# Nuralamsiddik16/Ultrafnd_git

Hardware: AMD Instinct MI355X
Metric: train-step samples/sec (FakeSV batch, seq128+224^2) (higher is better)
Workload: dtype bf16

## Files before the change

### include/ultrafnd_hip.h

```cpp
#ifndef ULTRAFND_HIP_H
#define ULTRAFND_HIP_H

#include <stddef.h>
#include <stdint.h>

#ifdef __cplusplus
extern "C" {
#endif

#define UFND_OK 0
#define UFND_ERR_INVALID 1
#define UFND_ERR_LAUNCH 2

#define UFND_ABI_VERSION 5

const char* ufnd_last_error(void);
int ufnd_abi_version(void);

typedef struct ufnd_step_state {
  uint64_t step;
  uint64_t seed;
  float lr;
  float weight_decay;
  float beta1, beta2, eps;
  float max_norm;
  float grad_scale;
  float loss;
  float grad_norm;
  float clip_coef;
  float bc1, bc2_sqrt;
  float reserved[3];
} ufnd_step_state;

typedef struct ufnd_dims {
  int hidden;
  int text_dim;
  int audio_dim;
  int visual_dim;
  int temporal_dim;
  int gnn_dim;
  int aux_dim;
  int trees;
  int depth;
  int classes;
  float fusion_dropout;
  float clf_dropout;
  float node_dropout;
} ufnd_dims;

typedef struct ufnd_fusion_params {
  float *text_w, *text_b;
  float *audio_w, *audio_b;
  float *visual_w, *visual_b;
  float *temporal_w, *temporal_b;
  float *gnn_w, *gnn_b;
  float *qkv_w, *qkv_b;
  float *ev0_w[3], *ev0_b[3];
  float *ev2_w[3], *ev2_b[3];
  float *fuse0_w, *fuse0_b;
  float *fuse3_w, *fuse3_b;
  float *cls_w, *cls_b;
} ufnd_fusion_params;

typedef struct ufnd_clf_params {
  float *pre0_w, *pre0_b;
  float *pre3_w, *pre3_b;
  float *gates, *thresh;
  float *leaf, *tau;
  float *bypass_w, *bypass_b;
  float *temperature;
} ufnd_clf_params;

size_t ufnd_fusion_workspace_floats(const ufnd_dims* d, int B);
size_t ufnd_clf_workspace_floats(const ufnd_dims* d, int B);

int ufnd_fusion_forward(const ufnd_dims* d, const ufnd_fusion_params* p, const float* text, const float* audio,
                        const float* visual, const float* temporal, const float* gnn, int B, int train,
                        float* workspace, float* fused, int ld_fused, float* logits, float* forensic,
                        const ufnd_step_state* state, void* stream);

int ufnd_fusion_backward(const ufnd_dims* d, const ufnd_fusion_params* p, const ufnd_fusion_params* g,
                         const float* text, const float* audio, const float* visual, const float* temporal,
                         const float* gnn, int B, int train, float* workspace, const float* d_fused,
                         int ld_dfused, const float* d_logits, const ufnd_step_state* state, void* stream,
                         void* side_stream, int join);

#define UFND_BWD_ALL 0
#define UFND_BWD_FUSE_MLP 1
#define UFND_BWD_REST 2
#define UFND_BWD_NO_LINEAR_GRADS 16
int ufnd_fusion_backward_phase(const ufnd_dims* d, const ufnd_fusion_params* p, const ufnd_fusion_params* g,
                               const float* text, const float* audio, const float* visual, const float* temporal,
                               const float* gnn, int B, int train, float* workspace, const float* d_fused,
                               int ld_dfused, const float* d_logits, const ufnd_step_state* state, void* stream,
                               void* side_stream, int join, int phase);

float* ufnd_clf_input_panel(const ufnd_dims* d, float* clf_workspace, int B, int* ld);
int ufnd_classifier_forward(const ufnd_dims* d, const ufnd_clf_params* p, const float* fused, int ld_fused,
                            const float* aux, int B, int train, float* workspace, float* logits, float* probs,
                            const ufnd_step_state* state, void* stream);
int ufnd_classifier_backward(const ufnd_dims* d, const ufnd_clf_params* p, const ufnd_clf_params* g, int B,
                             int train, float* workspace, const float* d_logits, float* d_fused, int ld_dfused,
                             const ufnd_step_state* state, void* stream, void* side_stream, int join);

int ufnd_classifier_backward_ex(const ufnd_dims* d, const ufnd_clf_params* p, const ufnd_clf_params* g, int B,
                                int train, float* workspace, const float* d_logits, float* d_fused, int ld_dfused,
                                const ufnd_step_state* state, void* stream, void* side_stream, int join, int flags);

size_t ufnd_head_factor_floats(const ufnd_dims* d, int B);
int ufnd_head_pack_factors(const ufnd_dims* d, const float* text, const float* audio, const float* visual, const float* temporal,
                           const float* gnn, int B, float* fusion_workspace, float* clf_workspace, float* pack, void* stream);
int ufnd_head_linear_grads_from_factors(const ufnd_dims* d, const ufnd_fusion_params* fusion_grads, const ufnd_clf_params* clf_grads,
                                        const float* packs, size_t rank_stride, int ranks, int B, void* stream);

typedef struct ufnd_head_io {
  const float *text, *audio, *visual, *temporal, *gnn, *aux;
  const int64_t* labels;
  float *fusion_workspace, *clf_workspace;
  float *logits, *probs, *forensic;
  float* d_logits;
} ufnd_head_io;
int ufnd_head_forward_loss(const ufnd_dims* d, const ufnd_fusion_params* fusion, const ufnd_clf_params* clf, const ufnd_head_io* io, int B,
                           int train, ufnd_step_state* state, void* stream);
int ufnd_head_backward(const ufnd_dims* d, const ufnd_fusion_params* fusion, const ufnd_fusion_params* fusion_grads, const ufnd_clf_params* clf,
                       const ufnd_clf_params* clf_grads, const ufnd_head_io* io, int B, int train, ufnd_step_state* state, void* stream,
                       void* side_stream, int join, int phase);

int ufnd_softmax_ce(const float* logits, const int64_t* labels, int B, float* loss_rows, float* d_logits,
                    ufnd_step_state* state, void* stream);

int ufnd_softmax_ce_weighted(const float* logits, const int64_t* labels, int B, float w0, float w1, float label_smoothing,
                             float* loss_rows, float* d_logits, ufnd_step_state* state, void* stream);

int ufnd_grad_norm(const float* grad, size_t n, float* partials, ufnd_step_state* state, void* stream);
int ufnd_adamw_step(float* param, const float* grad, float* exp_avg, float* exp_avg_sq, size_t n,
                    const ufnd_step_state* state, void* stream);
int ufnd_step_advance(ufnd_step_state* state, void* stream);
int ufnd_clip_adamw_step(float* param, const float* grad, float* exp_avg, float* exp_avg_sq, size_t n, float* partials,
                         ufnd_step_state* state, void* stream);

#define UFND_ACT_NONE 0
#define UFND_ACT_GELU 1
#define UFND_ACT_QUICK_GELU 2
#define UFND_ACT_GELU_BWD 3
#define UFND_ACT_QUICK_GELU_BWD 4

int ufnd_cast_bf16(const float* src, void* dst_bf16, size_t n, void* stream);

int ufnd_gemm_bf16(const void* A, const void* W, const float* bias, const float* residual, void* out_bf16,
                   float* out_f32, int M, int N, int K, int lda, int ldw, int ldr, int ldo, int ldf, int act,
                   void* stream);

#define UFND_GEMM_TILE_PERSISTENT 64
int ufnd_gemm_bf16_ex(const void* A, const void* W, const float* bias, const float* residual, void* out_bf16,
                      float* out_f32, int M, int N, int K, int lda, int ldw, int ldr, int ldo, int ldf, int act,
                      int tile_cfg, void* stream);

typedef struct ufnd_gemm_ln {
  const float* a_stats;
  const float* colsum;
  const float* r_stats;
  const float* r_gamma;
  const float* r_beta;
  float* out_stats;
  int a_parts, r_parts;
  float a_eps, r_eps;
  int width;
  int tile_cfg;
  const void* residual_bf16;
  int ldrb;
  float* guard;
} ufnd_gemm_ln;
#define UFND_FOLD_GUARD_SLOTS 1024
int ufnd_gemm_bf16_ln(const void* A, const void* W, const float* bias, const float* residual, void* out_bf16,
                      float* out_f32, int M, int N, int K, int lda, int ldw, int ldr, int ldo, int ldf, int act,
                      const ufnd_gemm_ln* ln, void* stream);
int ufnd_gemm_bf16_stat_parts(int M, int N, int K);

int ufnd_ln_fold_guard(const float* stats, int M, int parts, int width, float eps, float* guard, void* stream);
int ufnd_ln_fold_guard_multi(const float* stats, int M, int parts, int nbuf, size_t buf_stride, int width, float eps, float* guard,
                             void* stream);

int ufnd_gemm_bf16_tile_count(void);
int ufnd_gemm_bf16_tile_info(int tile_cfg, int* bm, int* bn, int* ln_aware);

int ufnd_layernorm(const float* x, int ldx, const float* gamma, const float* beta, void* out_bf16, float* out_f32,
                   int M, int H, float eps, void* stream);

int ufnd_attention_bf16(const void* qkv, const int32_t* key_mask, void* ctx, int B, int L, int heads,
                        void* stream);

int ufnd_qkv_attention_bf16(const void* X, const void* Wqkv, const float* bqkv, const int32_t* key_mask, void* ctx, int B, int L,
                            int heads, int ldx, int ldw, const ufnd_gemm_ln* ln, void* stream);

int ufnd_bert_embed_packed(const int64_t* ids, const int32_t* pos_ids, const float* word, const float* pos, const float* type0,
                           const float* gamma, const float* beta, void* x_bf16, float* x_f32, int T, int max_pos, int H,
                           int vocab, float eps, void* stream);
int ufnd_attention_bf16_varlen(const void* qkv, const int32_t* cu_seqlens, void* ctx, int B, int max_len, int heads, void* stream);
int ufnd_meanpool_l2_packed(const float* hidden, const int32_t* cu_seqlens, const int32_t* pos_ids, float* out, int B, int H,
                            void* stream);

int ufnd_text_pack(const int32_t* mask, int B, int L, int32_t* cu_seqlens, int32_t* row_src, void* stream);
int ufnd_bert_embed_live(const int64_t* ids, const int32_t* row_src, const int* m_live, const float* word, const float* pos,
                         const float* type0, const float* gamma, const float* beta, void* x_bf16, float* x_f32, int capacity, int L,
                         int H, int vocab, float eps, void* stream);
int ufnd_gemm_bf16_live(const void* A, const void* W, const float* bias, const float* residual, void* out_bf16, float* out_f32,
                        int M, int N, int K, int lda, int ldw, int ldr, int ldo, int ldf, int act, int tile_cfg, const int* m_live,
                        void* stream);
int ufnd_gemm_bf16_ln_live(const void* A, const void* W, const float* bias, const float* residual, void* out_bf16, float* out_f32,
                           int M, int N, int K, int lda, int ldw, int ldr, int ldo, int ldf, int act, const ufnd_gemm_ln* ln,
                           const int* m_live, void* stream);
int ufnd_qkv_attention_bf16_packed(const void* X, const void* Wqkv, const float* bqkv, const int32_t* key_mask, const int32_t* cu_seqlens,
                                   void* ctx, int B, int L, int heads, int ldx, int ldw, const ufnd_gemm_ln* ln, void* stream);
int ufnd_attention_bf16_varlen_masked(const void* qkv, const int32_t* cu_seqlens, const int32_t* key_mask, void* ctx, int B, int max_len,
                                      int heads, void* stream);
int ufnd_layernorm_live(const float* x, int ldx, const float* gamma, const float* beta, void* out_bf16, float* out_f32, int capacity,
                        int H, float eps, const int* m_live, void* stream);
int ufnd_masked_meanpool_l2_live(const float* hidden, const int32_t* mask, const int32_t* cu_seqlens, float* out, int B, int L, int H,
                                 void* stream);

int ufnd_bert_embed(const int64_t* ids, const float* word, const float* pos, const float* type0, const float* gamma,
                    const float* beta, void* x_bf16, float* x_f32, int B, int L, int H, int vocab, float eps,
                    void* stream);

int ufnd_masked_meanpool_l2(const float* hidden, const int32_t* mask, float* out, int B, int L, int H,
                            void* stream);

int ufnd_field_mean_l2(const float* parts, const int32_t* valid, float* out, int N, int M, int D, void* stream);

int ufnd_vit_patchify(const float* frames, void* patches_bf16, int N, int image, int patch, void* stream);

int ufnd_vit_assemble(const float* patch_emb, const float* cls, const float* pos, const float* gamma,
                      const float* beta, float* x_f32, void* x_bf16, float* stats, int N, int P, int H, float eps,
                      void* stream);

int ufnd_l2norm_frames(const float* e, float* out, int B, int F, int D, void* stream);

#define UFND_GATHER_MAX_ITEMS 8
typedef struct ufnd_gather_item {
  const void* src;
  void* dst;
  int row_bytes;
  int64_t src_rows;
} ufnd_gather_item;
int ufnd_gather_rows(const int64_t* idx, int B, const ufnd_gather_item* items, int n_items, void* stream);

int ufnd_temporal_weight_ld(int in_dim);
size_t ufnd_temporal_workspace_floats(int B, int in_dim, int hidden);
int ufnd_temporal_align(const float* text, const float* visual, const float* w0, const float* b0, const float* w3,
                        const float* b3, float* workspace, float* out, int B, int in_dim, int vis_dim, int hidden,
                        int out_dim, float dropout_p, const ufnd_step_state* state, void* stream);

typedef struct ufnd_tcn_layer {
  const float *w, *b;
  const float *gamma, *beta;
  float *running_mean, *running_var;
} ufnd_tcn_layer;
int ufnd_tcn_weight_ld(int in_ch, int kernel);
size_t ufnd_tcn_workspace_floats(int B, int T, int in_ch, int hid, int kernel);
int ufnd_tcn_forward(const float* text_seq, int text_dim, const float* vis_seq, int vis_dim, int B, int T,
                     const ufnd_tcn_layer* layers, int n_layers, int kernel, int hid, const float* head_w,
                     const float* head_b, int out_dim, int train, float dropout_p, float momentum, float eps,
                     const ufnd_step_state* state, float* workspace, float* out, void* stream);


int ufnd_ocr_adjacency(const int32_t* offsets, const int32_t* tokens, int N, double thresh, float* adj, int ld, void* stream);

typedef struct ufnd_gcn_params {
  const float* w1;
  const float* b1;
  const float* w2;
  const float* b2;
} ufnd_gcn_params;

size_t ufnd_gcn_workspace_floats(int N, int in_dim, int hid, int out_dim, int train);

int ufnd_gcn_forward(const float* x, const float* adj, int ld_adj, const ufnd_gcn_params* p, float* z, float* workspace, int N,
                     int in_dim, int hid, int out_dim, float dropout_p, const ufnd_step_state* state, void* stream);

int ufnd_gcn_pretrain_step(const float* x, const float* adj, int ld_adj, const ufnd_gcn_params* p, float* exp_avg,
                           float* exp_avg_sq, const float* head_w, const float* head_b, float* z, float* workspace, int N,
                           int in_dim, int hid, int out_dim, float dropout_p, float lr, float weight_decay, int step,
                           const ufnd_step_state* state, float* loss, void* stream);


int ufnd_ocr_adjacency_weighted(const int32_t* offsets, const int32_t* tokens, int N, double thresh, float* adj, int ld, void* stream);

int ufnd_node_features(const float* text, int ld_text, const float* audio, int ld_audio, const float* visual, int ld_visual,
                       const float* temporal, int ld_temporal, int n_text, int n_audio, int n_visual, int n_temporal, int B,
                       float* out, void* stream);

size_t ufnd_gnn_workspace_floats(int N, int in_dim, int hid, int out_dim);
int ufnd_gnn_forward(const float* x, const float* adj, int ld_adj, const ufnd_gcn_params* p, float* z, float* workspace, int N,
                     int in_dim, int hid, int out_dim, float dropout_p, const ufnd_step_state* state, void* stream);
int ufnd_gnn_backward(const float* x, const ufnd_gcn_params* p, float* g_w1, float* g_b1, float* g_w2, float* g_b2, const float* d_z,
                      float* workspace, int N, int in_dim, int hid, int out_dim, float dropout_p, const ufnd_step_state* state,
                      void* stream);
int ufnd_fusion_feature_grads(const ufnd_dims* d, const ufnd_fusion_params* p, float* workspace, int B, float* d_text, float* d_visual,
                              const ufnd_step_state* state, void* stream);

int ufnd_fusion_gnn_input_grad(const ufnd_dims* d, const ufnd_fusion_params* p, float* workspace, int B, float* d_gnn,
                               const ufnd_step_state* state, void* stream);

int ufnd_stream_create_cu_mask(const uint32_t* mask_words, int n_words, void** stream_out);
int ufnd_stream_destroy(void* stream);
int ufnd_device_cu_count(void);


int ufnd_gemm_bf16_dgrad(const void* dY, const void* Wt, const float* residual, const void* aux, void* out_bf16, float* out_f32,
                         int M, int N, int K, int lda, int ldw, int ldr, int ldaux, int ldo, int ldf, int act, void* stream);

size_t ufnd_gemm_bf16_wgrad_workspace_floats(int n_out, int k_in, int tokens);
int ufnd_gemm_bf16_wgrad(const void* dYt, const void* Xt, float* dW, int n_out, int k_in, int tokens, int lda, int ldb, int ldw,
                         float* workspace, int accumulate, void* stream);

typedef struct ufnd_partials_job {
  const float* part;
  int nblk, H;
  float *out0, *out1;
} ufnd_partials_job;
#define UFND_PARTIALS_DEFER 2

#define UFND_WGRAD_ALL 0
#define UFND_WGRAD_TRANSPOSE 1
#define UFND_WGRAD_PRODUCT 2
int ufnd_linear_wgrad(const void* dY, int lddy, const void* X, int ldx, int M, int N, int K, float* dW, float* db, void* dYt, void* Xt, int ldt,
                      float* slab_workspace, float* colsum_workspace, const ufnd_partials_job* extra, int part, void* stream);

typedef struct ufnd_refresh_item {
  const void* master;
  void* w;
  void* wt;
  int rows, cols, ld_master, ld_w, ld_wt, tile0;
} ufnd_refresh_item;
int ufnd_refresh_operands(const ufnd_refresh_item* items_device, int n_items, int total_tiles, void* stream);

size_t ufnd_transpose_colsum_workspace_floats(int rows_pad, int cols);
int ufnd_transpose_bf16(const void* src, int src_is_f32, int rows, int cols, int lds, void* dst, int ldd, int rows_pad, float* colsum,
                        float* colsum_ws, int colsum_accumulate, void* stream);

int ufnd_attention_bf16_lse(const void* qkv, const int32_t* key_mask, void* ctx, float* lse, int B, int L, int heads, void* stream);
size_t ufnd_attention_bwd_workspace_floats(int B, int L, int heads);
int ufnd_attention_bf16_bwd(const void* qkv, const void* ctx, const void* dctx, const float* lse, const int32_t* key_mask, void* dqkv,
                            float* workspace, int B, int L, int heads, void* stream);

size_t ufnd_layernorm_bwd_workspace_floats(int M, int H);
int ufnd_layernorm_bwd_blocks(int M);
int ufnd_row_partials_finish(const ufnd_partials_job* job, int accumulate, void* stream);
int ufnd_layernorm_bwd(const float* x, int ldx, const float* gamma, const float* dy, int lddy, const float* add, int ldadd, float* dx_f32,
                       void* dx_bf16, int lddx, float* dgamma, float* dbeta, float* workspace, int accumulate, int M, int H, float eps,
                       void* stream);

int ufnd_act_bf16(const void* x, void* out, size_t n, int act, void* stream);

int ufnd_masked_meanpool_l2_bwd(const float* hidden, const int32_t* mask, const float* dfeat, float* dhidden, int B, int L, int H, void* stream);
int ufnd_l2norm_frames_bwd(const float* e, const float* dfeat, float* de, int B, int F, int D, void* stream);
int ufnd_bert_embed_bwd(const int64_t* ids, const float* ds, float* dword, float* dpos, float* dtype, int B, int L, int H, int vocab,
                        int max_pos, int type_vocab, void* stream);
int ufnd_vit_assemble_bwd(const float* ds, float* dcls, float* dpos, void* dpe_bf16, int N, int P, int H, void* stream);

typedef struct ufnd_dropout {
  const ufnd_step_state* state;
  float p;
  uint32_t tag;
} ufnd_dropout;

#define UFND_LN_BWD_DROP_DXB 1
#define UFND_LN_BWD_DROP_DY 2

int ufnd_attention_bf16_lse_dropout(const void* qkv, const int32_t* key_mask, void* ctx, float* lse, int B, int L, int heads,
                                    const ufnd_dropout* drop, void* stream);
int ufnd_attention_bf16_bwd_dropout(const void* qkv, const void* ctx, const void* dctx, const float* lse, const int32_t* key_mask,
                                    void* dqkv, float* workspace, int B, int L, int heads, const ufnd_dropout* drop, void* stream);
int ufnd_dropout_residual_layernorm(const float* x, int ldx, const float* d, int ldd, const float* gamma, const float* beta, float* y,
                                    void* out_bf16, float* out_f32, int M, int H, float eps, const ufnd_dropout* drop, void* stream);
int ufnd_layernorm_dropout(const float* x, int ldx, const float* gamma, const float* beta, void* out_bf16, float* out_f32, int M, int H,
                           float eps, const ufnd_dropout* drop, void* stream);
int ufnd_layernorm_bwd_dropout(const float* x, int ldx, const float* gamma, const float* dy, int lddy, const float* add, int ldadd,
                               float* dx_f32, void* dx_bf16, int lddx, float* dgamma, float* dbeta, float* workspace, int accumulate,
                               int M, int H, float eps, const ufnd_dropout* drop, int where, void* stream);

#ifdef __cplusplus
}
#endif
#endif
```

### ultrafnd_git_amd/_lib.py

```python
from __future__ import annotations

import ctypes as C
from pathlib import Path
from typing import Optional

import torch

_PKG = Path(__file__).resolve().parent
LIB_PATH = _PKG / "libultrafnd_hip.so"


class UltrafndHipError(RuntimeError):
    pass


class StepState(C.Structure):
    _fields_ = [("step", C.c_uint64), ("seed", C.c_uint64), ("lr", C.c_float), ("weight_decay", C.c_float),
                ("beta1", C.c_float), ("beta2", C.c_float), ("eps", C.c_float), ("max_norm", C.c_float),
                ("grad_scale", C.c_float), ("loss", C.c_float), ("grad_norm", C.c_float), ("clip_coef", C.c_float),
                ("bc1", C.c_float), ("bc2_sqrt", C.c_float), ("reserved", C.c_float * 3)]


class Dims(C.Structure):
    _fields_ = [("hidden", C.c_int), ("text_dim", C.c_int), ("audio_dim", C.c_int), ("visual_dim", C.c_int),
                ("temporal_dim", C.c_int), ("gnn_dim", C.c_int), ("aux_dim", C.c_int), ("trees", C.c_int),
                ("depth", C.c_int), ("classes", C.c_int), ("fusion_dropout", C.c_float), ("clf_dropout", C.c_float),
                ("node_dropout", C.c_float)]


_FP = C.c_void_p


class FusionParams(C.Structure):
    _fields_ = [(n, _FP) for n in ("text_w", "text_b", "audio_w", "audio_b", "visual_w", "visual_b", "temporal_w",
                                   "temporal_b", "gnn_w", "gnn_b", "qkv_w", "qkv_b")] + \
               [("ev0_w", _FP * 3), ("ev0_b", _FP * 3), ("ev2_w", _FP * 3), ("ev2_b", _FP * 3)] + \
               [(n, _FP) for n in ("fuse0_w", "fuse0_b", "fuse3_w", "fuse3_b", "cls_w", "cls_b")]


class ClfParams(C.Structure):
    _fields_ = [(n, _FP) for n in ("pre0_w", "pre0_b", "pre3_w", "pre3_b", "gates", "thresh", "leaf", "tau",
                                   "bypass_w", "bypass_b", "temperature")]


class GcnParams(C.Structure):
    _fields_ = [(n, _FP) for n in ("w1", "b1", "w2", "b2")]


class GatherItem(C.Structure):
    _fields_ = [("src", _FP), ("dst", _FP), ("row_bytes", C.c_int), ("src_rows", C.c_int64)]


class TcnLayer(C.Structure):
    _fields_ = [(n, _FP) for n in ("w", "b", "gamma", "beta", "running_mean", "running_var")]


class HeadIO(C.Structure):
    _fields_ = [(n, C.c_void_p) for n in ("text", "audio", "visual", "temporal", "gnn", "aux", "labels", "fusion_workspace", "clf_workspace",
                                           "logits", "probs", "forensic", "d_logits")]


class PartialsJob(C.Structure):
    _fields_ = [("part", C.c_void_p), ("nblk", C.c_int), ("H", C.c_int), ("out0", C.c_void_p), ("out1", C.c_void_p)]


class RefreshItem(C.Structure):
    _fields_ = [("master", C.c_void_p), ("w", C.c_void_p), ("wt", C.c_void_p), ("rows", C.c_int), ("cols", C.c_int), ("ld_master", C.c_int),
                ("ld_w", C.c_int), ("ld_wt", C.c_int), ("tile0", C.c_int)]


class Dropout(C.Structure):
    _fields_ = [("state", C.c_void_p), ("p", C.c_float), ("tag", C.c_uint32)]


PARTIALS_DEFER = 2
LN_BWD_DROP_DXB, LN_BWD_DROP_DY = 1, 2
WGRAD_ALL, WGRAD_TRANSPOSE, WGRAD_PRODUCT = 0, 1, 2


class GemmLn(C.Structure):
    _fields_ = [("a_stats", _FP), ("colsum", _FP), ("r_stats", _FP), ("r_gamma", _FP), ("r_beta", _FP), ("out_stats", _FP),
                ("a_parts", C.c_int), ("r_parts", C.c_int), ("a_eps", C.c_float), ("r_eps", C.c_float), ("width", C.c_int),
                ("tile_cfg", C.c_int), ("residual_bf16", _FP), ("ldrb", C.c_int), ("guard", _FP)]

    def __init__(self, *a, **kw):
        super().__init__(*a, **kw)
        if "tile_cfg" not in kw:
            self.tile_cfg = -1


STEP_STATE_BYTES = C.sizeof(StepState)
BWD_ALL, BWD_FUSE_MLP, BWD_REST = 0, 1, 2
BWD_NO_LINEAR_GRADS = 16
ABI_VERSION = 5
FOLD_GUARD_SLOTS = 1024

_lib: Optional[C.CDLL] = None


def _declare(lib: C.CDLL) -> None:
    P, I, S = C.c_void_p, C.c_int, C.c_size_t
    lib.ufnd_last_error.restype = C.c_char_p
    lib.ufnd_abi_version.restype = I
    lib.ufnd_fusion_workspace_floats.restype = S
    lib.ufnd_fusion_workspace_floats.argtypes = [C.POINTER(Dims), I]
    lib.ufnd_clf_workspace_floats.restype = S
    lib.ufnd_clf_workspace_floats.argtypes = [C.POINTER(Dims), I]
    lib.ufnd_clf_input_panel.restype = P
    lib.ufnd_clf_input_panel.argtypes = [C.POINTER(Dims), P, I, C.POINTER(I)]
    lib.ufnd_fusion_forward.argtypes = [C.POINTER(Dims), C.POINTER(FusionParams), P, P, P, P, P, I, I, P, P, I, P, P, P, P]
    lib.ufnd_fusion_backward.argtypes = [C.POINTER(Dims), C.POINTER(FusionParams), C.POINTER(FusionParams),
                                         P, P, P, P, P, I, I, P, P, I, P, P, P, P, I]
    lib.ufnd_fusion_backward_phase.argtypes = [C.POINTER(Dims), C.POINTER(FusionParams), C.POINTER(FusionParams),
                                               P, P, P, P, P, I, I, P, P, I, P, P, P, P, I, I]
    lib.ufnd_fusion_backward_phase.restype = I
    lib.ufnd_classifier_forward.argtypes = [C.POINTER(Dims), C.POINTER(ClfParams), P, I, P, I, I, P, P, P, P, P]
    lib.ufnd_classifier_backward.argtypes = [C.POINTER(Dims), C.POINTER(ClfParams), C.POINTER(ClfParams), I, I, P, P, P,
                                             I, P, P, P, I]
    lib.ufnd_classifier_backward_ex.argtypes = [C.POINTER(Dims), C.POINTER(ClfParams), C.POINTER(ClfParams), I, I, P, P, P,
                                                I, P, P, P, I, I]
    lib.ufnd_classifier_backward_ex.restype = I
    lib.ufnd_head_factor_floats.argtypes = [C.POINTER(Dims), I]
    lib.ufnd_head_factor_floats.restype = S
    lib.ufnd_head_pack_factors.argtypes = [C.POINTER(Dims), P, P, P, P, P, I, P, P, P, P]
    lib.ufnd_head_pack_factors.restype = I
    lib.ufnd_head_linear_grads_from_factors.argtypes = [C.POINTER(Dims), C.POINTER(FusionParams), C.POINTER(ClfParams), P, S, I, I, P]
    lib.ufnd_head_linear_grads_from_factors.restype = I
    lib.ufnd_head_forward_loss.argtypes = [C.POINTER(Dims), C.POINTER(FusionParams), C.POINTER(ClfParams), C.POINTER(HeadIO), I, I, P, P]
    lib.ufnd_head_forward_loss.restype = I
    lib.ufnd_head_backward.argtypes = [C.POINTER(Dims), C.POINTER(FusionParams), C.POINTER(FusionParams), C.POINTER(ClfParams), C.POINTER(ClfParams),
                                       C.POINTER(HeadIO), I, I, P, P, P, I, I]
    lib.ufnd_head_backward.restype = I
    lib.ufnd_softmax_ce.argtypes = [P, P, I, P, P, P, P]
    lib.ufnd_softmax_ce_weighted.argtypes = [P, P, I, C.c_float, C.c_float, C.c_float, P, P, P, P]
    lib.ufnd_softmax_ce_weighted.restype = I
    lib.ufnd_grad_norm.argtypes = [P, S, P, P, P]
    lib.ufnd_adamw_step.argtypes = [P, P, P, P, S, P, P]
    lib.ufnd_step_advance.argtypes = [P, P]
    lib.ufnd_clip_adamw_step.argtypes = [P, P, P, P, S, P, P, P]
    lib.ufnd_clip_adamw_step.restype = I
    for name in ("ufnd_fusion_forward", "ufnd_fusion_backward", "ufnd_classifier_forward", "ufnd_classifier_backward",
                 "ufnd_softmax_ce", "ufnd_grad_norm", "ufnd_adamw_step", "ufnd_step_advance"):
        getattr(lib, name).restype = I
    _declare_encoders(lib)


def _declare_encoders(lib: C.CDLL) -> None:
    P, I, S, F = C.c_void_p, C.c_int, C.c_size_t, C.c_float
    sigs = {
        "ufnd_cast_bf16": [P, P, S, P],
        "ufnd_gemm_bf16": [P] * 6 + [I] * 9 + [P],
        "ufnd_gemm_bf16_ex": [P] * 6 + [I] * 10 + [P],
        "ufnd_layernorm": [P, I, P, P, P, P, I, I, F, P],
        "ufnd_attention_bf16": [P, P, P, I, I, I, P],
        "ufnd_qkv_attention_bf16": [P, P, P, P, P, I, I, I, I, I, C.POINTER(GemmLn), P],
        "ufnd_bert_embed": [P] * 8 + [I, I, I, I, F, P],
        "ufnd_masked_meanpool_l2": [P, P, P, I, I, I, P],
        "ufnd_bert_embed_packed": [P] * 9 + [I, I, I, I, F, P],
        "ufnd_attention_bf16_varlen": [P, P, P, I, I, I, P],
        "ufnd_meanpool_l2_packed": [P, P, P, P, I, I, P],
        "ufnd_text_pack": [P, I, I, P, P, P],
        "ufnd_bert_embed_live": [P] * 10 + [I, I, I, I, F, P],
        "ufnd_gemm_bf16_live": [P] * 6 + [I] * 10 + [P, P],
        "ufnd_gemm_bf16_ln_live": [P] * 6 + [I] * 9 + [C.POINTER(GemmLn), P, P],
        "ufnd_qkv_attention_bf16_packed": [P, P, P, P, P, P, I, I, I, I, I, C.POINTER(GemmLn), P],
        "ufnd_attention_bf16_varlen_masked": [P, P, P, P, I, I, I, P],
        "ufnd_layernorm_live": [P, I, P, P, P, P, I, I, F, P, P],
        "ufnd_masked_meanpool_l2_live": [P, P, P, P, I, I, I, P],
        "ufnd_vit_patchify": [P, P, I, I, I, P],
        "ufnd_vit_assemble": [P] * 8 + [I, I, I, F, P],
        "ufnd_gemm_bf16_ln": [P] * 6 + [I] * 9 + [C.POINTER(GemmLn), P],
        "ufnd_gemm_bf16_stat_parts": [I, I, I],
        "ufnd_ln_fold_guard": [P, I, I, I, F, P, P],
        "ufnd_ln_fold_guard_multi": [P, I, I, I, S, I, F, P, P],
        "ufnd_gemm_bf16_tile_count": [],
        "ufnd_gemm_bf16_tile_info": [I, C.POINTER(I), C.POINTER(I), C.POINTER(I)],
        "ufnd_stream_create_cu_mask": [C.POINTER(C.c_uint32), I, C.POINTER(P)],
        "ufnd_stream_destroy": [P],
        "ufnd_device_cu_count": [],
        "ufnd_l2norm_frames": [P, P, I, I, I, P],
        "ufnd_field_mean_l2": [P, P, P, I, I, I, P],
        "ufnd_temporal_align": [P] * 8 + [I] * 5 + [F, P, P],
    }
    sigs.update({
        "ufnd_gemm_bf16_dgrad": [P] * 6 + [I] * 10 + [P],
        "ufnd_gemm_bf16_wgrad": [P, P, P, I, I, I, I, I, I, P, I, P],
        "ufnd_transpose_bf16": [P, I, I, I, I, P, I, I, P, P, I, P],
        "ufnd_linear_wgrad": [P, I, P, I, I, I, I, P, P, P, P, I, P, P, C.POINTER(PartialsJob), I, P],
        "ufnd_refresh_operands": [P, I, I, P],
        "ufnd_layernorm_bwd_blocks": [I],
        "ufnd_row_partials_finish": [C.POINTER(PartialsJob), I, P],
        "ufnd_attention_bf16_lse": [P, P, P, P, I, I, I, P],
        "ufnd_attention_bf16_bwd": [P, P, P, P, P, P, P, I, I, I, P],
        "ufnd_layernorm_bwd": [P, I, P, P, I, P, I, P, P, I, P, P, P, I, I, I, F, P],
        "ufnd_masked_meanpool_l2_bwd": [P, P, P, P, I, I, I, P],
        "ufnd_l2norm_frames_bwd": [P, P, P, I, I, I, P],
        "ufnd_bert_embed_bwd": [P, P, P, P, P, I, I, I, I, I, I, P],
        "ufnd_vit_assemble_bwd": [P, P, P, P, I, I, I, P],
        "ufnd_act_bf16": [P, P, S, I, P],
        "ufnd_attention_bf16_lse_dropout": [P, P, P, P, I, I, I, C.POINTER(Dropout), P],
        "ufnd_attention_bf16_bwd_dropout": [P, P, P, P, P, P, P, I, I, I, C.POINTER(Dropout), P],
        "ufnd_dropout_residual_layernorm": [P, I, P, I, P, P, P, P, P, I, I, F, C.POINTER(Dropout), P],
        "ufnd_layernorm_dropout": [P, I, P, P, P, P, I, I, F, C.POINTER(Dropout), P],
        "ufnd_layernorm_bwd_dropout": [P, I, P, P, I, P, I, P, P, I, P, P, P, I, I, I, F, C.POINTER(Dropout), I, P],
    })
    for name, argtypes in sigs.items():
        fn = getattr(lib, name)
        fn.argtypes = argtypes
        fn.restype = I
    for name, argtypes in (("ufnd_gemm_bf16_wgrad_workspace_floats", [I, I, I]), ("ufnd_transpose_colsum_workspace_floats", [I, I]),
                           ("ufnd_attention_bwd_workspace_floats", [I, I, I]), ("ufnd_layernorm_bwd_workspace_floats", [I, I])):
        fn = getattr(lib, name)
        fn.argtypes = argtypes
        fn.restype = S
    D = C.c_double
    lib.ufnd_ocr_adjacency.argtypes = [P, P, I, D, P, I, P]
    lib.ufnd_ocr_adjacency.restype = I
    lib.ufnd_gcn_workspace_floats.argtypes = [I, I, I, I, I]
    lib.ufnd_gcn_workspace_floats.restype = S
    lib.ufnd_gcn_forward.argtypes = [P, P, I, C.POINTER(GcnParams), P, P, I, I, I, I, F, P, P]
    lib.ufnd_gcn_forward.restype = I
    lib.ufnd_gcn_pretrain_step.argtypes = [P, P, I, C.POINTER(GcnParams), P, P, P, P, P, P, I, I, I, I, F, F, F, I, P, P, P]
    lib.ufnd_gcn_pretrain_step.restype = I
    lib.ufnd_ocr_adjacency_weighted.argtypes = [P, P, I, D, P, I, P]
    lib.ufnd_ocr_adjacency_weighted.restype = I
    lib.ufnd_node_features.argtypes = [P, I, P, I, P, I, P, I, I, I, I, I, I, P, P]
    lib.ufnd_node_features.restype = I
    lib.ufnd_gnn_workspace_floats.argtypes = [I, I, I, I]
    lib.ufnd_gnn_workspace_floats.restype = S
    lib.ufnd_gnn_forward.argtypes = [P, P, I, C.POINTER(GcnParams), P, P, I, I, I, I, F, P, P]
    lib.ufnd_gnn_forward.restype = I
    lib.ufnd_gnn_backward.argtypes = [P, C.POINTER(GcnParams), P, P, P, P, P, P, I, I, I, I, F, P, P]
    lib.ufnd_gnn_backward.restype = I
    lib.ufnd_fusion_gnn_input_grad.argtypes = [C.POINTER(Dims), C.POINTER(FusionParams), P, I, P, P, P]
    lib.ufnd_fusion_gnn_input_grad.restype = I
    lib.ufnd_fusion_feature_grads.argtypes = [C.POINTER(Dims), C.POINTER(FusionParams), P, I, P, P, P, P]
    lib.ufnd_fusion_feature_grads.restype = I
    lib.ufnd_gather_rows.argtypes = [P, I, C.POINTER(GatherItem), I, P]
    lib.ufnd_gather_rows.restype = I
    lib.ufnd_tcn_weight_ld.argtypes = [I, I]
    lib.ufnd_tcn_weight_ld.restype = I
    lib.ufnd_tcn_workspace_floats.argtypes = [I, I, I, I, I]
    lib.ufnd_tcn_workspace_floats.restype = S
    lib.ufnd_tcn_forward.argtypes = [P, I, P, I, I, I, C.POINTER(TcnLayer), I, I, I, P, P, I, I, F, F, F, P, P, P, P]
    lib.ufnd_tcn_forward.restype = I
    lib.ufnd_temporal_weight_ld.argtypes = [I]
    lib.ufnd_temporal_weight_ld.restype = I
    lib.ufnd_temporal_workspace_floats.argtypes = [I, I, I]
    lib.ufnd_temporal_workspace_floats.restype = S


def lib() -> C.CDLL:
    global _lib
    if _lib is None:
        if not LIB_PATH.exists():
            raise UltrafndHipError(
                f"{LIB_PATH} is missing: run `python -m ultrafnd_git_amd.build` (hipcc, gfx950). "
                "This package has no CPU fallback.")
        l = C.CDLL(str(LIB_PATH))
        _declare(l)
        if l.ufnd_abi_version() != ABI_VERSION:
            raise UltrafndHipError("libultrafnd_hip.so ABI version mismatch; rebuild")
        _lib = l
    return _lib


def check(rc: int, what: str) -> None:
    if rc != 0:
        raise UltrafndHipError(f"{what} failed (code {rc}): {lib().ufnd_last_error().decode()}")


def ptr(t: Optional[torch.Tensor]) -> Optional[int]:
    return None if t is None else t.data_ptr()


def require_hip(*tensors: Optional[torch.Tensor]) -> torch.device:
    dev = None
    for t in tensors:
        if t is None:
            continue
        if t.device.type != "cuda":
            raise UltrafndHipError(
                f"tensor on {t.device}: the fusion hot path runs on a HIP device only (no CPU fallback); "
                "move the module and its inputs to 'cuda'")
        dev = dev or t.device
        if t.device != dev:
            raise UltrafndHipError("all tensors of one call must live on the same device")
    return dev


def stream_ptr(device: torch.device) -> int:
    return torch.cuda.current_stream(device).cuda_stream


def f32c(t: torch.Tensor) -> torch.Tensor:
    if t.dtype != torch.float32:
        t = t.float()
    return t if t.is_contiguous() else t.contiguous()
```

### ultrafnd_git_amd/csrc/encoders.hip

```cpp
#include "common.hpp"

namespace {

__device__ __forceinline__ f32x4 ld4(const float* p) { return *reinterpret_cast<const f32x4*>(p); }

template <int NI>
__device__ __forceinline__ void ln_row(f32x4 (&v)[NI], int H, float eps, const float* gamma, const float* beta, int lane) {
  float s = 0.0f;
#pragma unroll
  for (int i = 0; i < NI; ++i) s += v[i][0] + v[i][1] + v[i][2] + v[i][3];
  const float mean = wave_sum(s) / (float)H;
  float q = 0.0f;
#pragma unroll
  for (int i = 0; i < NI; ++i)
#pragma unroll
    for (int k = 0; k < 4; ++k) {
      const float d = v[i][k] - mean;
      q += d * d;
    }
  const float rstd = rsqrtf(wave_sum(q) / (float)H + eps);
#pragma unroll
  for (int i = 0; i < NI; ++i) {
    const int col = 4 * lane + 256 * i;
    const f32x4 gm = ld4(gamma + col), bt = ld4(beta + col);
#pragma unroll
    for (int k = 0; k < 4; ++k) v[i][k] = (v[i][k] - mean) * rstd * gm[k] + bt[k];
  }
}

template <int NI>
__device__ __forceinline__ void store_row(const f32x4 (&v)[NI], __bf16* ob, float* of, size_t row, int H, int lane) {
#pragma unroll
  for (int i = 0; i < NI; ++i) {
    const int col = 4 * lane + 256 * i;
    if (of) *reinterpret_cast<f32x4*>(of + row * H + col) = v[i];
    if (ob) {
      bf16x4 o = {(__bf16)v[i][0], (__bf16)v[i][1], (__bf16)v[i][2], (__bf16)v[i][3]};
      *reinterpret_cast<bf16x4*>(ob + row * H + col) = o;
    }
  }
}

template <int NI>
__device__ __forceinline__ void row_stats(const f32x4 (&v)[NI], float* stats, size_t row, int lane) {
  float s = 0.0f, q = 0.0f;
#pragma unroll
  for (int i = 0; i < NI; ++i)
#pragma unroll
    for (int k = 0; k < 4; ++k) { s += v[i][k]; q += v[i][k] * v[i][k]; }
  s = wave_sum(s);
  q = wave_sum(q);
  if (lane == 0) *reinterpret_cast<f32x4*>(stats + row * 4) = f32x4{s, q, 0.0f, 0.0f};
}

template <int NI>
__global__ __launch_bounds__(256) void layernorm_kernel(const float* x, int ldx, const float* gamma, const float* beta,
                                                        __bf16* ob, float* of, int M, int H, float eps, const int* m_live) {
  const int lane = threadIdx.x & 63;
  const int row = blockIdx.x * 4 + (threadIdx.x >> 6);
  if (row >= M || (m_live && row >= *m_live)) return;
  f32x4 v[NI];
#pragma unroll
  for (int i = 0; i < NI; ++i) v[i] = ld4(x + (size_t)row * ldx + 4 * lane + 256 * i);
  ln_row<NI>(v, H, eps, gamma, beta, lane);
  store_row<NI>(v, ob, of, row, H, lane);
}

template <int NI, bool RESID>
__global__ __launch_bounds__(256) void dropout_layernorm_kernel(const float* x, int ldx, const float* d, int ldd, const float* gamma,
                                                                const float* beta, float* y, __bf16* ob, float* of, int M, int H, float eps,
                                                                ufnd_dropout dr) {
  const int lane = threadIdx.x & 63;
  const int row = blockIdx.x * 4 + (threadIdx.x >> 6);
  if (row >= M) return;
  const uint64_t seed = dr.state->seed, step = dr.state->step;
  f32x4 v[NI], m[NI];
#pragma unroll
  for (int i = 0; i < NI; ++i) {
    const int col = 4 * lane + 256 * i;
    float m4[4];
    dropout_mul4_ctr(seed, step, dr.p, dr.tag, (uint32_t)(((size_t)row * H + col) >> 2), m4);
    m[i] = f32x4{m4[0], m4[1], m4[2], m4[3]};
    v[i] = ld4(x + (size_t)row * ldx + col);
    if constexpr (RESID) {
      v[i] += m[i] * ld4(d + (size_t)row * ldd + col);
      *reinterpret_cast<f32x4*>(y + (size_t)row * H + col) = v[i];
    }
  }
  ln_row<NI>(v, H, eps, gamma, beta, lane);
  if constexpr (!RESID) {
#pragma unroll
    for (int i = 0; i < NI; ++i) v[i] *= m[i];
  }
  store_row<NI>(v, ob, of, row, H, lane);
}

template <int NI>
__global__ __launch_bounds__(256) void bert_embed_kernel(const int64_t* ids, const float* word, const float* pos,
                                                         const float* type0, const float* gamma, const float* beta,
                                                         __bf16* ob, float* of, int M, int L, int H, int vocab,
                                                         float eps, const int32_t* pos_ids, const int32_t* row_src,
                                                         const int* m_live) {
  const int lane = threadIdx.x & 63;
  const int row = blockIdx.x * 4 + (threadIdx.x >> 6);
  if (row >= M || (m_live && row >= *m_live)) return;
  const int src = row_src ? row_src[row] : row;
  long long id = ids[src];
  id = id < 0 ? 0 : (id >= vocab ? vocab - 1 : id);
  int l = pos_ids ? pos_ids[row] : src % L;
  l = l < 0 ? 0 : (l >= L ? L - 1 : l);
  f32x4 v[NI];
#pragma unroll
  for (int i = 0; i < NI; ++i) {
    const int col = 4 * lane + 256 * i;
    v[i] = ld4(word + (size_t)id * H + col) + ld4(pos + (size_t)l * H + col) + ld4(type0 + col);
  }
  if (gamma) ln_row<NI>(v, H, eps, gamma, beta, lane);
  store_row<NI>(v, ob, of, row, H, lane);
}

template <bool PACKED>
__global__ __launch_bounds__(256) void meanpool_kernel(const float* hidden, const int32_t* mask, float* out, int L, int H, const int32_t* cu) {
  __shared__ f32x4 part[4][64];
  __shared__ float cnts[4];
  const int b = blockIdx.y, col = blockIdx.x * 256 + 4 * (threadIdx.x & 63), grp = threadIdx.x >> 6, lane = threadIdx.x & 63;
  f32x4 acc = {0.f, 0.f, 0.f, 0.f};
  float cnt = 0.0f;
  const size_t r0 = PACKED ? (size_t)cu[b] : (size_t)b * L;
  const int n = PACKED ? cu[b + 1] - cu[b] : L;
  for (int l0 = grp; l0 < n; l0 += 32) {
    int mk[8];
    f32x4 x[8];
#pragma unroll
    for (int u = 0; u < 8; ++u) {
      const int l = l0 + 4 * u;
      mk[u] = l < n ? mask[(size_t)b * L + l] : 0;
    }
#pragma unroll
    for (int u = 0; u < 8; ++u) {
      const int l = l0 + 4 * u < n ? l0 + 4 * u : n - 1;
      x[u] = ld4(hidden + (r0 + l) * H + col);
    }
#pragma unroll
    for (int u = 0; u < 8; ++u) {
      if (mk[u] != 0) {
        acc += x[u];
        cnt += 1.0f;
      }
    }
  }
  part[grp][lane] = acc;
  if (lane == 0) cnts[grp] = cnt;
  __syncthreads();
  if (grp == 0) {
    const f32x4 s = (part[0][lane] + part[1][lane]) + (part[2][lane] + part[3][lane]);
    const float denom = fmaxf((cnts[0] + cnts[1]) + (cnts[2] + cnts[3]), 1e-6f);
    *reinterpret_cast<f32x4*>(out + (size_t)b * H + col) = s / denom;
  }
}
__global__ __launch_bounds__(256) void meanpool_packed_kernel(const float* hidden, const int32_t* cu, const int32_t* pos_ids, float* out,
                                                              int H) {
  __shared__ f32x4 part[4][64];
  __shared__ float cnts[4];
  const int b = blockIdx.y, col = blockIdx.x * 256 + 4 * (threadIdx.x & 63), grp = threadIdx.x >> 6, lane = threadIdx.x & 63;
  const int r0 = cu[b], r1 = cu[b + 1];
  f32x4 acc = {0.f, 0.f, 0.f, 0.f};
  float cnt = 0.0f;
  for (int r = r0; r < r1; ++r) {
    if ((pos_ids[r] & 3) == grp) {
      acc += ld4(hidden + (size_t)r * H + col);
      cnt += 1.0f;
    }
  }
  part[grp][lane] = acc;
  if (lane == 0) cnts[grp] = cnt;
  __syncthreads();
  if (grp == 0) {
    const f32x4 s = (part[0][lane] + part[1][lane]) + (part[2][lane] + part[3][lane]);
    const float denom = fmaxf((cnts[0] + cnts[1]) + (cnts[2] + cnts[3]), 1e-6f);
    *reinterpret_cast<f32x4*>(out + (size_t)b * H + col) = s / denom;
  }
}
constexpr int PACK_THREADS = 1024, PACK_MAX_B = 16384;
__global__ __launch_bounds__(PACK_THREADS) void text_pack_kernel(const int32_t* mask, int B, int L, int32_t* cu, int32_t* row_src) {
  __shared__ int lens[PACK_MAX_B];
  __shared__ int wsum[PACK_THREADS / 64];
  __shared__ int total;
  const int tid = threadIdx.x, wave = tid >> 6, lane = tid & 63;
  for (int b = wave; b < B; b += PACK_THREADS / 64) {
    int last = 0;
    for (int l = lane; l < L; l += 64) last = mask[(size_t)b * L + l] != 0 ? l + 1 : last;
#pragma unroll
    for (int o = 32; o >= 1; o >>= 1) last = max(last, __shfl_xor(last, o, 64));
    if (lane == 0) lens[b] = last;
  }
  __syncthreads();
  const int per = (B + PACK_THREADS - 1) / PACK_THREADS, b0 = tid * per, b1 = min(b0 + per, B);
  int own = 0;
  for (int b = b0; b < b1; ++b) own += lens[b];
  int inc = own;
#pragma unroll
  for (int o = 1; o < 64; o <<= 1) {
    const int y = __shfl_up(inc, o, 64);
    if (lane >= o) inc += y;
  }
  if (lane == 63) wsum[wave] = inc;
  __syncthreads();
  int base = 0;
  for (int w = 0; w < wave; ++w) base += wsum[w];
  int run = base + inc - own;
  for (int b = b0; b < b1; ++b) {
    const int n = lens[b];
    lens[b] = run;
    cu[b] = run;
    run += n;
  }
  if (tid == PACK_THREADS - 1) {
    cu[B] = run;
    total = run;
  }
  __syncthreads();
  for (int b = wave; b < B; b += PACK_THREADS / 64) {
    const int r0 = lens[b], n = (b + 1 < B ? lens[b + 1] : total) - r0;
    for (int l = lane; l < n; l += 64) row_src[r0 + l] = b * L + l;
  }
}

__global__ __launch_bounds__(256) void l2norm_rows_kernel(float* x, int H) {
  __shared__ float sh[4];
  float* row = x + (size_t)blockIdx.x * H;
  float sq = 0.0f;
  for (int c = threadIdx.x; c < H; c += 256) sq += row[c] * row[c];
  sq = wave_sum(sq);
  if ((threadIdx.x & 63) == 0) sh[threadIdx.x >> 6] = sq;
  __syncthreads();
  const float nrm = sqrtf((sh[0] + sh[1]) + (sh[2] + sh[3])) + 1e-9f;
  for (int c = threadIdx.x; c < H; c += 256) row[c] = row[c] / nrm;
}

template <int PT, int GT>
__global__ __launch_bounds__(256) void patchify_kernel(const float* frames, __bf16* patches, int S_, int P_) {
  const int P = PT ? PT : P_, G = GT ? GT : S_ / P_, S = P * G;
  const int n = blockIdx.x / G, py = blockIdx.x - n * G;
  const int K = 3 * P * P, CPR = P / 8;
  const int chunks = 3 * P * G * CPR;
  const float* src = frames + ((size_t)n * 3 * S + (size_t)py * P) * S;
  __bf16* dst = patches + ((size_t)n * G * G + (size_t)py * G) * K;
  for (int q = threadIdx.x; q < chunks; q += 256) {
    const int x8 = q % (G * CPR), r = q / (G * CPR);
    const int ky = r % P, c = r / P;
    const int px = x8 / CPR, kx = (x8 - px * CPR) * 8;
    const float* sp = src + ((size_t)c * S + ky) * S + x8 * 8;
    const f32x4 v0 = ld4(sp), v1 = ld4(sp + 4);
    bf16x8 o = {(__bf16)v0[0], (__bf16)v0[1], (__bf16)v0[2], (__bf16)v0[3], (__bf16)v1[0], (__bf16)v1[1], (__bf16)v1[2], (__bf16)v1[3]};
    *reinterpret_cast<bf16x8*>(dst + (size_t)px * K + c * P * P + ky * P + kx) = o;
  }
}

template <int NI>
__global__ __launch_bounds__(256) void vit_assemble_kernel(const float* pe, const float* cls, const float* pos,
                                                           const float* gamma, const float* beta, float* of, __bf16* ob,
                                                           float* stats, int M, int P, int H, float eps) {
  const int lane = threadIdx.x & 63;
  const int row = blockIdx.x * 4 + (threadIdx.x >> 6);
  if (row >= M) return;
  const int n = row / (P + 1), t = row % (P + 1);
  f32x4 v[NI];
#pragma unroll
  for (int i = 0; i < NI; ++i) {
    const int col = 4 * lane + 256 * i;
    const f32x4 base = (t == 0) ? ld4(cls + col) : ld4(pe + ((size_t)n * P + (t - 1)) * H + col);
    v[i] = base + ld4(pos + (size_t)t * H + col);
  }
  if (gamma) ln_row<NI>(v, H, eps, gamma, beta, lane);
  store_row<NI>(v, ob, of, row, H, lane);
  if (stats) row_stats<NI>(v, stats, row, lane);
}

__global__ __launch_bounds__(256) void l2norm_frames_kernel(const float* e, float* out, int F, int D) {
  __shared__ float sh[4];
  const int b = blockIdx.x;
  float acc[4] = {0, 0, 0, 0};
  for (int f = 0; f < F; ++f) {
    const float* row = e + ((size_t)b * F + f) * D;
    float sq = 0.0f;
    for (int c = threadIdx.x; c < D; c += 256) sq += row[c] * row[c];
    sq = wave_sum(sq);
    __syncthreads();
    if ((threadIdx.x & 63) == 0) sh[threadIdx.x >> 6] = sq;
    __syncthreads();
    const float nrm = sqrtf((sh[0] + sh[1]) + (sh[2] + sh[3])) + 1e-9f;
    int n = 0;
    for (int c = threadIdx.x; c < D; c += 256, ++n) acc[n] += row[c] / nrm;
  }
  if (F == 1) {
    int n = 0;
    for (int c = threadIdx.x; c < D; c += 256, ++n) out[(size_t)b * D + c] = acc[n];
    return;
  }
  float sq = 0.0f;
  int n = 0;
  for (int c = threadIdx.x; c < D; c += 256, ++n) {
    acc[n] /= (float)F;
    sq += acc[n] * acc[n];
  }
  sq = wave_sum(sq);
  __syncthreads();
  if ((threadIdx.x & 63) == 0) sh[threadIdx.x >> 6] = sq;
  __syncthreads();
  const float nrm = sqrtf((sh[0] + sh[1]) + (sh[2] + sh[3])) + 1e-9f;
  n = 0;
  for (int c = threadIdx.x; c < D; c += 256, ++n) out[(size_t)b * D + c] = acc[n] / nrm;
}

__global__ __launch_bounds__(256) void field_mean_l2_kernel(const float* parts, const int32_t* valid, float* out, int Mx,
                                                            int D) {
  __shared__ float sh[4];
  const int n = blockIdx.x;
  float acc[4] = {0, 0, 0, 0};
  int cnt = 0;
  for (int m = 0; m < Mx; ++m) {
    if (valid[(size_t)n * Mx + m] == 0) continue;
    ++cnt;
    const float* row = parts + ((size_t)n * Mx + m) * D;
    int k = 0;
    for (int c = threadIdx.x; c < D; c += 256, ++k) acc[k] += row[c];
  }
  float sq = 0.0f;
  int k = 0;
  for (int c = threadIdx.x; c < D; c += 256, ++k) {
    acc[k] = cnt ? acc[k] / (float)cnt : 0.0f;
    sq += acc[k] * acc[k];
  }
  sq = wave_sum(sq);
  if ((threadIdx.x & 63) == 0) sh[threadIdx.x >> 6] = sq;
  __syncthreads();
  const float nrm = sqrtf((sh[0] + sh[1]) + (sh[2] + sh[3])) + 1e-9f;
  k = 0;
  for (int c = threadIdx.x; c < D; c += 256, ++k) out[(size_t)n * D + c] = cnt ? acc[k] / nrm : 0.0f;
}

#define NI_LAUNCH(H, KERNEL, GRID, STREAM, ...)                                                       \
  do {                                                                                                \
    if ((H) == 256) hipLaunchKernelGGL((KERNEL<1>), GRID, dim3(256), 0, STREAM, __VA_ARGS__);         \
    else if ((H) == 512) hipLaunchKernelGGL((KERNEL<2>), GRID, dim3(256), 0, STREAM, __VA_ARGS__);    \
    else if ((H) == 768) hipLaunchKernelGGL((KERNEL<3>), GRID, dim3(256), 0, STREAM, __VA_ARGS__);    \
    else hipLaunchKernelGGL((KERNEL<4>), GRID, dim3(256), 0, STREAM, __VA_ARGS__);                    \
  } while (0)

#define NI_LAUNCH_T(H, KERNEL, T, GRID, STREAM, ...)                                                       \
  do {                                                                                                     \
    if ((H) == 256) hipLaunchKernelGGL((KERNEL<1, T>), GRID, dim3(256), 0, STREAM, __VA_ARGS__);           \
    else if ((H) == 512) hipLaunchKernelGGL((KERNEL<2, T>), GRID, dim3(256), 0, STREAM, __VA_ARGS__);      \
    else if ((H) == 768) hipLaunchKernelGGL((KERNEL<3, T>), GRID, dim3(256), 0, STREAM, __VA_ARGS__);      \
    else hipLaunchKernelGGL((KERNEL<4, T>), GRID, dim3(256), 0, STREAM, __VA_ARGS__);                      \
  } while (0)

inline bool h_ok(int H) { return H == 256 || H == 512 || H == 768 || H == 1024; }

}

extern "C" int ufnd_layernorm(const float* x, int ldx, const float* gamma, const float* beta, void* out_bf16,
                              float* out_f32, int M, int H, float eps, void* stream_) {
  UFND_REQUIRE(x && gamma && beta && (out_bf16 || out_f32) && M >= 1, "layernorm: null argument");
  UFND_REQUIRE(h_ok(H), "layernorm: H=%d (supported 256/512/768/1024)", H);
  UFND_REQUIRE(ldx % 4 == 0 && ldx >= H && ufnd_aligned(x, 16) && ufnd_aligned(gamma, 16) && ufnd_aligned(beta, 16),
               "layernorm: alignment");
  NI_LAUNCH(H, layernorm_kernel, dim3(ufnd_cdiv(M, 4)), (hipStream_t)stream_, x, ldx, gamma, beta, (__bf16*)out_bf16,
            out_f32, M, H, eps, (const int*)nullptr);
  UFND_CHECK_LAUNCH();
  return UFND_OK;
}

extern "C" int ufnd_dropout_residual_layernorm(const float* x, int ldx, const float* d, int ldd, const float* gamma, const float* beta, float* y,
                                               void* out_bf16, float* out_f32, int M, int H, float eps, const ufnd_dropout* drop, void* stream_) {
  UFND_REQUIRE(x && d && gamma && beta && y && (out_bf16 || out_f32) && M >= 1 && drop && drop->state, "dropout_residual_layernorm: null argument");
  UFND_REQUIRE(drop->p > 0.0f && drop->p < 1.0f, "dropout_residual_layernorm: p=%g (0 < p < 1)", (double)drop->p);
  UFND_REQUIRE(h_ok(H), "dropout_residual_layernorm: H=%d (supported 256/512/768/1024)", H);
  UFND_REQUIRE(ldx % 4 == 0 && ldx >= H && ldd % 4 == 0 && ldd >= H && ufnd_aligned(x, 16) && ufnd_aligned(d, 16) && ufnd_aligned(y, 16) &&
                   ufnd_aligned(gamma, 16) && ufnd_aligned(beta, 16) && (!out_f32 || ufnd_aligned(out_f32, 16)) && (!out_bf16 || ufnd_aligned(out_bf16, 8)),
               "dropout_residual_layernorm: alignment");
  UFND_REQUIRE((long long)M * H / 4 <= (1ll << 32), "dropout_residual_layernorm: M=%d H=%d overflows the 32-bit dropout counter", M, H);
  NI_LAUNCH_T(H, dropout_layernorm_kernel, true, dim3(ufnd_cdiv(M, 4)), (hipStream_t)stream_, x, ldx, d, ldd, gamma, beta, y, (__bf16*)out_bf16,
            out_f32, M, H, eps, *drop);
  UFND_CHECK_LAUNCH();
  return UFND_OK;
}

extern "C" int ufnd_layernorm_dropout(const float* x, int ldx, const float* gamma, const float* beta, void* out_bf16, float* out_f32, int M, int H,
                                      float eps, const ufnd_dropout* drop, void* stream_) {
  UFND_REQUIRE(x && gamma && beta && (out_bf16 || out_f32) && M >= 1 && drop && drop->state, "layernorm_dropout: null argument");
  UFND_REQUIRE(drop->p > 0.0f && drop->p < 1.0f, "layernorm_dropout: p=%g (0 < p < 1)", (double)drop->p);
  UFND_REQUIRE(h_ok(H), "layernorm_dropout: H=%d (supported 256/512/768/1024)", H);
  UFND_REQUIRE(ldx % 4 == 0 && ldx >= H && ufnd_aligned(x, 16) && ufnd_aligned(gamma, 16) && ufnd_aligned(beta, 16) &&
                   (!out_f32 || ufnd_aligned(out_f32, 16)) && (!out_bf16 || ufnd_aligned(out_bf16, 8)), "layernorm_dropout: alignment");
  UFND_REQUIRE((long long)M * H / 4 <= (1ll << 32), "layernorm_dropout: M=%d H=%d overflows the 32-bit dropout counter", M, H);
  NI_LAUNCH_T(H, dropout_layernorm_kernel, false, dim3(ufnd_cdiv(M, 4)), (hipStream_t)stream_, x, ldx, (const float*)nullptr, 0, gamma, beta,
            (float*)nullptr, (__bf16*)out_bf16, out_f32, M, H, eps, *drop);
  UFND_CHECK_LAUNCH();
  return UFND_OK;
}

extern "C" int ufnd_bert_embed(const int64_t* ids, const float* word, const float* pos, const float* type0,
                               const float* gamma, const float* beta, void* x_bf16, float* x_f32, int B, int L, int H,
                               int vocab, float eps, void* stream_) {
  UFND_REQUIRE(ids && word && pos && type0 && ((gamma && beta) || (!gamma && !beta)) && (x_bf16 || x_f32), "bert_embed: null argument");
  UFND_REQUIRE(h_ok(H) && B >= 1 && L >= 1 && vocab >= 1, "bert_embed: B=%d L=%d H=%d vocab=%d", B, L, H, vocab);
  UFND_REQUIRE(ufnd_aligned(word, 16) && ufnd_aligned(pos, 16) && ufnd_aligned(type0, 16), "bert_embed: alignment");
  const int M = B * L;
  NI_LAUNCH(H, bert_embed_kernel, dim3(ufnd_cdiv(M, 4)), (hipStream_t)stream_, ids, word, pos, type0, gamma, beta,
            (__bf16*)x_bf16, x_f32, M, L, H, vocab, eps, (const int32_t*)nullptr, (const int32_t*)nullptr,
            (const int*)nullptr);
  UFND_CHECK_LAUNCH();
  return UFND_OK;
}

extern "C" int ufnd_bert_embed_packed(const int64_t* ids, const int32_t* pos_ids, const float* word, const float* pos,
                                      const float* type0, const float* gamma, const float* beta, void* x_bf16, float* x_f32,
                                      int T, int max_pos, int H, int vocab, float eps, void* stream_) {
  UFND_REQUIRE(ids && pos_ids && word && pos && type0 && gamma && beta && (x_bf16 || x_f32), "bert_embed_packed: null argument");
  UFND_REQUIRE(h_ok(H) && T >= 1 && max_pos >= 1 && vocab >= 1, "bert_embed_packed: T=%d H=%d vocab=%d", T, H, vocab);
  UFND_REQUIRE(ufnd_aligned(word, 16) && ufnd_aligned(pos, 16) && ufnd_aligned(type0, 16), "bert_embed_packed: alignment");
  NI_LAUNCH(H, bert_embed_kernel, dim3(ufnd_cdiv(T, 4)), (hipStream_t)stream_, ids, word, pos, type0, gamma, beta,
            (__bf16*)x_bf16, x_f32, T, max_pos, H, vocab, eps, pos_ids, (const int32_t*)nullptr, (const int*)nullptr);
  UFND_CHECK_LAUNCH();
  return UFND_OK;
}

extern "C" int ufnd_masked_meanpool_l2(const float* hidden, const int32_t* mask, float* out, int B, int L, int H,
                                       void* stream_) {
  UFND_REQUIRE(hidden && mask && out && B >= 1 && L >= 1, "meanpool: null argument");
  UFND_REQUIRE(H >= 256 && H % 256 == 0 && ufnd_aligned(hidden, 16) && ufnd_aligned(out, 16), "meanpool: H=%d (multiple of 256)", H);
  hipLaunchKernelGGL(meanpool_kernel<false>, dim3(H / 256, B), dim3(256), 0, (hipStream_t)stream_, hidden, mask, out, L, H,
                     (const int32_t*)nullptr);
  UFND_CHECK_LAUNCH();
  hipLaunchKernelGGL(l2norm_rows_kernel, dim3(B), dim3(256), 0, (hipStream_t)stream_, out, H);
  UFND_CHECK_LAUNCH();
  return UFND_OK;
}

extern "C" int ufnd_meanpool_l2_packed(const float* hidden, const int32_t* cu_seqlens, const int32_t* pos_ids, float* out, int B, int H,
                                       void* stream_) {
  UFND_REQUIRE(hidden && cu_seqlens && pos_ids && out && B >= 1, "meanpool_packed: null argument");
  UFND_REQUIRE(H >= 256 && H % 256 == 0 && ufnd_aligned(hidden, 16) && ufnd_aligned(out, 16), "meanpool_packed: H=%d (multiple of 256)", H);
  hipLaunchKernelGGL(meanpool_packed_kernel, dim3(H / 256, B), dim3(256), 0, (hipStream_t)stream_, hidden, cu_seqlens, pos_ids, out, H);
  UFND_CHECK_LAUNCH();
  hipLaunchKernelGGL(l2norm_rows_kernel, dim3(B), dim3(256), 0, (hipStream_t)stream_, out, H);
  UFND_CHECK_LAUNCH();
  return UFND_OK;
}

extern "C" int ufnd_text_pack(const int32_t* mask, int B, int L, int32_t* cu_seqlens, int32_t* row_src, void* stream_) {
  UFND_REQUIRE(mask && cu_seqlens && row_src, "text_pack: null argument");
  UFND_REQUIRE(B >= 1 && B <= PACK_MAX_B && L >= 1 && (long long)B * L < (1ll << 31), "text_pack: B=%d L=%d (B <= %d)", B, L, PACK_MAX_B);
  hipLaunchKernelGGL(text_pack_kernel, dim3(1), dim3(PACK_THREADS), 0, (hipStream_t)stream_, mask, B, L, cu_seqlens, row_src);
  UFND_CHECK_LAUNCH();
  return UFND_OK;
}

extern "C" int ufnd_bert_embed_live(const int64_t* ids, const int32_t* row_src, const int* m_live, const float* word, const float* pos,
                                    const float* type0, const float* gamma, const float* beta, void* x_bf16, float* x_f32, int capacity,
                                    int L, int H, int vocab, float eps, void* stream_) {
  UFND_REQUIRE(ids && row_src && m_live && word && pos && type0 && gamma && beta && (x_bf16 || x_f32), "bert_embed_live: null argument");
  UFND_REQUIRE(h_ok(H) && capacity >= 1 && L >= 1 && vocab >= 1, "bert_embed_live: capacity=%d L=%d H=%d vocab=%d", capacity, L, H, vocab);
  UFND_REQUIRE(ufnd_aligned(word, 16) && ufnd_aligned(pos, 16) && ufnd_aligned(type0, 16), "bert_embed_live: alignment");
  NI_LAUNCH(H, bert_embed_kernel, dim3(ufnd_cdiv(capacity, 4)), (hipStream_t)stream_, ids, word, pos, type0, gamma, beta,
            (__bf16*)x_bf16, x_f32, capacity, L, H, vocab, eps, (const int32_t*)nullptr, row_src, m_live);
  UFND_CHECK_LAUNCH();
  return UFND_OK;
}

extern "C" int ufnd_layernorm_live(const float* x, int ldx, const float* gamma, const float* beta, void* out_bf16, float* out_f32,
                                   int capacity, int H, float eps, const int* m_live, void* stream_) {
  UFND_REQUIRE(x && gamma && beta && (out_bf16 || out_f32) && m_live && capacity >= 1, "layernorm_live: null argument");
  UFND_REQUIRE(h_ok(H), "layernorm_live: H=%d (supported 256/512/768/1024)", H);
  UFND_REQUIRE(ldx % 4 == 0 && ldx >= H && ufnd_aligned(x, 16) && ufnd_aligned(gamma, 16) && ufnd_aligned(beta, 16),
               "layernorm_live: alignment");
  NI_LAUNCH(H, layernorm_kernel, dim3(ufnd_cdiv(capacity, 4)), (hipStream_t)stream_, x, ldx, gamma, beta, (__bf16*)out_bf16,
            out_f32, capacity, H, eps, m_live);
  UFND_CHECK_LAUNCH();
  return UFND_OK;
}

extern "C" int ufnd_masked_meanpool_l2_live(const float* hidden, const int32_t* mask, const int32_t* cu_seqlens, float* out, int B, int L,
                                            int H, void* stream_) {
  UFND_REQUIRE(hidden && mask && cu_seqlens && out && B >= 1 && L >= 1, "meanpool_live: null argument");
  UFND_REQUIRE(H >= 256 && H % 256 == 0 && ufnd_aligned(hidden, 16) && ufnd_aligned(out, 16), "meanpool_live: H=%d (multiple of 256)", H);
  hipLaunchKernelGGL(meanpool_kernel<true>, dim3(H / 256, B), dim3(256), 0, (hipStream_t)stream_, hidden, mask, out, L, H, cu_seqlens);
  UFND_CHECK_LAUNCH();
  hipLaunchKernelGGL(l2norm_rows_kernel, dim3(B), dim3(256), 0, (hipStream_t)stream_, out, H);
  UFND_CHECK_LAUNCH();
  return UFND_OK;
}

extern "C" int ufnd_vit_patchify(const float* frames, void* patches, int N, int image, int patch, void* stream_) {
  UFND_REQUIRE(frames && patches && N >= 1, "patchify: null argument");
  UFND_REQUIRE(patch % 8 == 0 && image % patch == 0 && ufnd_aligned(frames, 16) && ufnd_aligned(patches, 16),
               "patchify: image=%d patch=%d (patch a multiple of 8, 16-B aligned buffers)", image, patch);
  const int G = image / patch;
  if (patch == 32 && G == 7) hipLaunchKernelGGL((patchify_kernel<32, 7>), dim3(N * G), dim3(256), 0, (hipStream_t)stream_, frames, (__bf16*)patches, image, patch);
  else hipLaunchKernelGGL((patchify_kernel<0, 0>), dim3(N * G), dim3(256), 0, (hipStream_t)stream_, frames, (__bf16*)patches, image, patch);
  UFND_CHECK_LAUNCH();
  return UFND_OK;
}

extern "C" int ufnd_vit_assemble(const float* patch_emb, const float* cls, const float* pos, const float* gamma,
                                 const float* beta, float* x_f32, void* x_bf16, float* stats, int N, int P, int H, float eps,
                                 void* stream_) {
  UFND_REQUIRE(patch_emb && cls && pos && ((gamma && beta) || (!gamma && !beta)) && (x_f32 || x_bf16) && N >= 1 && P >= 1, "vit_assemble: null argument");
  UFND_REQUIRE(h_ok(H), "vit_assemble: H=%d", H);
  const int M = N * (P + 1);
  UFND_REQUIRE(!stats || ufnd_aligned(stats, 16), "vit_assemble: stats alignment");
  NI_LAUNCH(H, vit_assemble_kernel, dim3(ufnd_cdiv(M, 4)), (hipStream_t)stream_, patch_emb, cls, pos, gamma, beta, x_f32,
            (__bf16*)x_bf16, stats, M, P, H, eps);
  UFND_CHECK_LAUNCH();
  return UFND_OK;
}

extern "C" int ufnd_l2norm_frames(const float* e, float* out, int B, int F, int D, void* stream_) {
  UFND_REQUIRE(e && out && B >= 1 && F >= 1 && D >= 1 && D <= 1024, "l2norm_frames: B=%d F=%d D=%d", B, F, D);
  hipLaunchKernelGGL(l2norm_frames_kernel, dim3(B), dim3(256), 0, (hipStream_t)stream_, e, out, F, D);
  UFND_CHECK_LAUNCH();
  return UFND_OK;
}

extern "C" int ufnd_field_mean_l2(const float* parts, const int32_t* valid, float* out, int N, int Mx, int D, void* stream_) {
  UFND_REQUIRE(parts && valid && out && N >= 1 && Mx >= 1 && D >= 1 && D <= 1024, "field_mean_l2: N=%d M=%d D=%d", N, Mx, D);
  hipLaunchKernelGGL(field_mean_l2_kernel, dim3(N), dim3(256), 0, (hipStream_t)stream_, parts, valid, out, Mx, D);
  UFND_CHECK_LAUNCH();
  return UFND_OK;
}

namespace {
__global__ __launch_bounds__(256) void ln_fold_guard_kernel(const float* stats, int M, int parts, int nbuf, size_t buf_stride, float inv_h,
                                                            float eps, float* guard) {
  __shared__ float sh[4];
  float worst = 0.0f;
  const int nq = parts >> 1, sub = threadIdx.x & 3;
  const long long total = (long long)M * nbuf;
  const long long step = (long long)gridDim.x * 64;
  for (long long r = (long long)blockIdx.x * 64 + (threadIdx.x >> 2); r < total; r += 2 * step) {
    f32x4 v[2][3];
    bool live[2];
#pragma unroll
    for (int k = 0; k < 2; ++k) {
      const long long rk = r + k * step;
      live[k] = rk < total;
      const long long rc = live[k] ? rk : r;
      const int bi = (int)(rc / M), row = (int)(rc - (long long)bi * M);
      const f32x4* p = reinterpret_cast<const f32x4*>(stats + bi * buf_stride + (size_t)row * parts * 2);
#pragma unroll
      for (int u = 0; u < 3; ++u) {
        const int c = sub + 4 * u;
        v[k][u] = p[c < nq ? c : sub];
      }
    }
#pragma unroll
    for (int k = 0; k < 2; ++k) {
      float sm = 0.0f, sq = 0.0f;
#pragma unroll
      for (int u = 0; u < 3; ++u) {
        if (sub + 4 * u < nq) {
          sm += v[k][u][0] + v[k][u][2];
          sq += v[k][u][1] + v[k][u][3];
        }
      }
      sm += quad_xor1(sm); sq += quad_xor1(sq);
      sm += quad_xor2(sm); sq += quad_xor2(sq);
      const float mean = sm * inv_h;
      const float var = fmaxf(sq * inv_h - mean * mean, 0.0f);
      if (live[k]) {
        float ratio = fabsf(mean) * rsqrtf(var + eps);
        ratio = ratio == ratio ? ratio : INFINITY;
        worst = fmaxf(worst, ratio);
      }
    }
  }
  worst = wave_max(worst);
  if ((threadIdx.x & 63) == 0) sh[threadIdx.x >> 6] = worst;
  __syncthreads();
  if (threadIdx.x == 0)
    atomicMax(reinterpret_cast<int*>(guard), __float_as_int(fmaxf(fmaxf(sh[0], sh[1]), fmaxf(sh[2], sh[3]))));
}
}

extern "C" int ufnd_ln_fold_guard_multi(const float* stats, int M, int parts, int nbuf, size_t buf_stride, int width, float eps, float* guard,
                                        void* stream_) {
  UFND_REQUIRE(stats && guard && M >= 1 && parts >= 2 && parts <= 24 && parts % 2 == 0 && nbuf >= 1 && width >= 1 && ufnd_aligned(stats, 16) &&
               (nbuf == 1 || (buf_stride % 4 == 0 && buf_stride >= (size_t)M * parts * 2)),
               "ln_fold_guard: M=%d parts=%d (even) nbuf=%d stride=%zu", M, parts, nbuf, buf_stride);
  const long long rows = (long long)M * nbuf;
  const long long want = (rows + 63) / 64;
  const int blocks = (int)(want < 2048 ? want : 2048);
  hipLaunchKernelGGL(ln_fold_guard_kernel, dim3(blocks), dim3(256), 0, (hipStream_t)stream_, stats, M, parts, nbuf, buf_stride,
                     1.0f / (float)width, eps, guard);
  UFND_CHECK_LAUNCH();
  return UFND_OK;
}

extern "C" int ufnd_ln_fold_guard(const float* stats, int M, int parts, int width, float eps, float* guard, void* stream_) {
  return ufnd_ln_fold_guard_multi(stats, M, parts, 1, 0, width, eps, guard, stream_);
}
```

### ultrafnd_git_amd/csrc/gemm_bf16.hip

```cpp
#include "gemm_bf16_kernel.hpp"

#define UFND_GEMM_TILE_PP UFND_GEMM_TILE_PERSISTENT
int ufnd_pp_pick(const void* gemm_args);
int ufnd_pp_launch(void* gemm_args, void* stream);
int ufnd_pp_stat_parts(int N);

namespace {
__global__ __launch_bounds__(256) void cast_bf16_kernel(const float* src, __bf16* dst, size_t n) {
  for (size_t i = (blockIdx.x * (size_t)256 + threadIdx.x) * 4; i < n; i += (size_t)gridDim.x * 256 * 4) {
    if (i + 4 <= n) {
      const f32x4 v = *reinterpret_cast<const f32x4*>(src + i);
      bf16x4 o = {(__bf16)v[0], (__bf16)v[1], (__bf16)v[2], (__bf16)v[3]};
      *reinterpret_cast<bf16x4*>(dst + i) = o;
    } else {
      for (size_t j = i; j < n; ++j) dst[j] = (__bf16)src[j];
    }
  }
}

}

extern "C" int ufnd_gemm_bf16_live(const void* A, const void* W, const float* bias, const float* residual, void* out_bf16,
                                   float* out_f32, int M, int N, int K, int lda, int ldw, int ldr, int ldo, int ldf, int act,
                                   int tile_cfg, const int* m_live, void* stream_) {
  UFND_REQUIRE(A && W && (out_bf16 || out_f32), "gemm_bf16: null operand");
  UFND_REQUIRE(M >= 1 && N >= 64 && K >= 64 && N % 64 == 0 && K % 64 == 0, "gemm_bf16: M=%d N=%d K=%d (need N%%64==0, K%%64==0)", M, N, K);
  UFND_REQUIRE(lda % 8 == 0 && ldw % 8 == 0 && lda >= K && ldw >= K && ufnd_aligned(A, 16) && ufnd_aligned(W, 16),
               "gemm_bf16: A/W strides must be multiples of 8 and pointers 16-B aligned");
  UFND_REQUIRE(!residual || (ldr % 4 == 0 && ldr >= N && ufnd_aligned(residual, 16)), "gemm_bf16: residual alignment");
  UFND_REQUIRE(!out_f32 || (ldf % 4 == 0 && ldf >= N && ufnd_aligned(out_f32, 16)), "gemm_bf16: out_f32 alignment");
  UFND_REQUIRE(!out_bf16 || (ldo % 8 == 0 && ldo >= N && ufnd_aligned(out_bf16, 16)), "gemm_bf16: out_bf16 alignment");
  UFND_REQUIRE(!bias || ufnd_aligned(bias, 4), "gemm_bf16: bias alignment");
  UFND_REQUIRE(act >= 0 && act <= 2, "gemm_bf16: act=%d", act);
  GemmArgs a{(const __bf16*)A, (const __bf16*)W, bias, residual, (__bf16*)out_bf16, out_f32, M, N, K, lda, ldw, ldr, ldo, ldf, act, 0, 0, nullptr};
  a.m_live = m_live;
  if (tile_cfg == UFND_GEMM_TILE_PP || (tile_cfg < 0 && ufnd_pp_pick(&a))) return ufnd_pp_launch(&a, stream_);
  const int cfg = tile_cfg < 0 ? auto_cfg(M, N, K) : tile_cfg;
  UFND_REQUIRE(cfg < kNumTiles && kTiles[cfg].built, "gemm_bf16: tile config %d is not part of this library (ufnd_gemm_bf16_tile_info)", cfg);
  UFND_REQUIRE(N % kTiles[cfg].bn == 0, "gemm_bf16: tile config %d needs N %% %d == 0", cfg, kTiles[cfg].bn);
  int rc = launch_cfg(cfg, 0, a, (hipStream_t)stream_);
  if (rc != UFND_OK) return rc;
  UFND_CHECK_LAUNCH();
  return UFND_OK;
}

extern "C" int ufnd_gemm_bf16_ex(const void* A, const void* W, const float* bias, const float* residual, void* out_bf16,
                                 float* out_f32, int M, int N, int K, int lda, int ldw, int ldr, int ldo, int ldf, int act,
                                 int tile_cfg, void* stream_) {
  return ufnd_gemm_bf16_live(A, W, bias, residual, out_bf16, out_f32, M, N, K, lda, ldw, ldr, ldo, ldf, act, tile_cfg, nullptr, stream_);
}

extern "C" int ufnd_gemm_bf16_tile_info(int tile_cfg, int* bm, int* bn, int* ln_aware) {
  if (tile_cfg < 0 || tile_cfg >= kNumTiles || !kTiles[tile_cfg].built) return 0;
  if (bm) *bm = kTiles[tile_cfg].bm;
  if (bn) *bn = kTiles[tile_cfg].bn;
  if (ln_aware) *ln_aware = kTiles[tile_cfg].lnx;
  return 1;
}
extern "C" int ufnd_gemm_bf16_tile_count(void) { return kNumTiles; }

static int stat_parts_for(int cfg, int N) {
  const TileCfg& t = kTiles[cfg];
  const int tn = t.bn / t.wn;
  if (!t.built || !t.lnx || N % t.bn != 0 || tn % 32 != 0 || (N / 32) % 2 != 0 || N / 32 > 24) return 0;
  return N / 32;
}
extern "C" int ufnd_gemm_bf16_stat_parts(int M, int N, int K) {
  static const __bf16 probe[8] = {};
  GemmArgs a{};
  a.A = a.W = probe;
  a.out_bf16 = const_cast<__bf16*>(probe);
  a.residual_b = probe;
  a.out_stats = reinterpret_cast<float*>(const_cast<__bf16*>(probe));
  a.M = M; a.N = N; a.K = K; a.lda = a.ldw = K; a.ldo = a.ldrb = N;
  if (ufnd_pp_pick(&a)) return ufnd_pp_stat_parts(N);
  return stat_parts_for(auto_cfg(M, N, K), N);
}

extern "C" int ufnd_gemm_bf16_ln_live(const void* A, const void* W, const float* bias, const float* residual, void* out_bf16,
                                      float* out_f32, int M, int N, int K, int lda, int ldw, int ldr, int ldo, int ldf, int act,
                                      const ufnd_gemm_ln* ln, const int* m_live, void* stream_);
extern "C" int ufnd_gemm_bf16_ln(const void* A, const void* W, const float* bias, const float* residual, void* out_bf16,
                                 float* out_f32, int M, int N, int K, int lda, int ldw, int ldr, int ldo, int ldf, int act,
                                 const ufnd_gemm_ln* ln, void* stream_) {
  return ufnd_gemm_bf16_ln_live(A, W, bias, residual, out_bf16, out_f32, M, N, K, lda, ldw, ldr, ldo, ldf, act, ln, nullptr, stream_);
}

extern "C" int ufnd_gemm_bf16_ln_live(const void* A, const void* W, const float* bias, const float* residual, void* out_bf16,
                                      float* out_f32, int M, int N, int K, int lda, int ldw, int ldr, int ldo, int ldf, int act,
                                      const ufnd_gemm_ln* ln, const int* m_live, void* stream_) {
  UFND_REQUIRE(A && W && ln && (out_bf16 || out_f32), "gemm_bf16_ln: null operand");
  UFND_REQUIRE(M >= 1 && N >= 64 && K >= 64 && N % 64 == 0 && K % 64 == 0, "gemm_bf16_ln: M=%d N=%d K=%d (need N%%64==0, K%%64==0)", M, N, K);
  UFND_REQUIRE(lda % 8 == 0 && ldw % 8 == 0 && lda >= K && ldw >= K && ufnd_aligned(A, 16) && ufnd_aligned(W, 16),
               "gemm_bf16_ln: A/W strides must be multiples of 8 and pointers 16-B aligned");
  UFND_REQUIRE(!residual || (ldr % 4 == 0 && ldr >= N && ufnd_aligned(residual, 16)), "gemm_bf16_ln: residual alignment");
  UFND_REQUIRE(!out_f32 || (ldf % 4 == 0 && ldf >= N && ufnd_aligned(out_f32, 16)), "gemm_bf16_ln: out_f32 alignment");
  UFND_REQUIRE(!out_bf16 || (ldo % 8 == 0 && ldo >= N && ufnd_aligned(out_bf16, 16)), "gemm_bf16_ln: out_bf16 alignment");
  UFND_REQUIRE(!bias || ufnd_aligned(bias, 16), "gemm_bf16_ln: bias must be 16-B aligned");
  UFND_REQUIRE(act >= 0 && act <= 2, "gemm_bf16_ln: act=%d", act);
  UFND_REQUIRE(!(ln->a_stats && ln->r_stats), "gemm_bf16_ln: a_stats and r_stats are mutually exclusive");
  UFND_REQUIRE(!(residual && ln->residual_bf16), "gemm_bf16_ln: residual (fp32) and residual_bf16 are mutually exclusive");
  UFND_REQUIRE(!ln->residual_bf16 || (ln->ldrb % 8 == 0 && ln->ldrb >= N && ufnd_aligned(ln->residual_bf16, 16)), "gemm_bf16_ln: residual_bf16 alignment");
  UFND_REQUIRE(ln->a_stats || act == UFND_ACT_NONE, "gemm_bf16_ln: an activation is only fused together with a folded LayerNorm (a_stats)");
  UFND_REQUIRE(ln->width > 0, "gemm_bf16_ln: width (the LayerNorm dimension) must be positive");
  if (ln->a_stats) {
    UFND_REQUIRE(!residual && !ln->residual_bf16 && !ln->out_stats,
                 "gemm_bf16_ln: a folded LayerNorm (a_stats) takes no residual and writes no out_stats (that epilogue is compiled without them)");
    UFND_REQUIRE(ln->colsum && ufnd_aligned(ln->colsum, 16) && ufnd_aligned(ln->a_stats, 16), "gemm_bf16_ln: colsum / a_stats alignment");
    UFND_REQUIRE(ln->a_parts >= 2 && ln->a_parts <= 24 && ln->a_parts % 2 == 0, "gemm_bf16_ln: a_parts=%d (even, 2..24)", ln->a_parts);
  }
  if (ln->r_stats) {
    UFND_REQUIRE((residual || ln->residual_bf16) && ln->r_gamma && ln->r_beta && ufnd_aligned(ln->r_gamma, 16) && ufnd_aligned(ln->r_beta, 16) &&
                     ufnd_aligned(ln->r_stats, 16), "gemm_bf16_ln: r_stats needs residual, r_gamma, r_beta (16-B aligned)");
    UFND_REQUIRE(ln->r_parts >= 2 && ln->r_parts <= 24 && ln->r_parts % 2 == 0, "gemm_bf16_ln: r_parts=%d (even, 2..24)", ln->r_parts);
  }
  GemmArgs a{(const __bf16*)A, (const __bf16*)W, bias, residual, (__bf16*)out_bf16, out_f32, M, N, K, lda, ldw, ldr, ldo, ldf, act, 0, 0, nullptr};
  a.a_stats = ln->a_stats; a.colsum = ln->colsum; a.r_stats = ln->r_stats; a.r_gamma = ln->r_gamma; a.r_beta = ln->r_beta;
  a.out_stats = ln->out_stats; a.a_parts = ln->a_parts; a.r_parts = ln->r_parts; a.a_eps = ln->a_eps; a.r_eps = ln->r_eps;
  a.inv_h = 1.0f / (float)ln->width;
  a.residual_b = (const __bf16*)ln->residual_bf16;
  a.ldrb = ln->ldrb;
  a.guard = ln->a_stats ? ln->guard : nullptr;
  a.m_live = m_live;
  if (ln->tile_cfg == UFND_GEMM_TILE_PP || (ln->tile_cfg < 0 && ufnd_pp_pick(&a))) return ufnd_pp_launch(&a, stream_);
  const int cfg = ln->tile_cfg < 0 ? auto_cfg(M, N, K) : ln->tile_cfg;
  UFND_REQUIRE(cfg < kNumTiles && kTiles[cfg].built && kTiles[cfg].lnx && N % kTiles[cfg].bn == 0,
               "gemm_bf16_ln: no LayerNorm-aware kernel for M=%d N=%d K=%d (tile %d)", M, N, K, cfg);
  if (ln->out_stats) {
    UFND_REQUIRE(stat_parts_for(cfg, N) > 0 && ufnd_aligned(ln->out_stats, 16), "gemm_bf16_ln: out_stats unsupported for this shape / tile");
  }
  int rc = launch_cfg(cfg, 4, a, (hipStream_t)stream_);
  if (rc != UFND_OK) return rc;
  UFND_CHECK_LAUNCH();
  return UFND_OK;
}

extern "C" int ufnd_qkv_attention_bf16_packed(const void* X, const void* Wqkv, const float* bqkv, const int32_t* key_mask,
                                              const int32_t* cu_seqlens, void* ctx, int B, int L, int heads, int ldx, int ldw,
                                              const ufnd_gemm_ln* ln, void* stream_);
extern "C" int ufnd_qkv_attention_bf16(const void* X, const void* Wqkv, const float* bqkv, const int32_t* key_mask, void* ctx,
                                       int B, int L, int heads, int ldx, int ldw, const ufnd_gemm_ln* ln, void* stream_) {
  return ufnd_qkv_attention_bf16_packed(X, Wqkv, bqkv, key_mask, nullptr, ctx, B, L, heads, ldx, ldw, ln, stream_);
}

extern "C" int ufnd_qkv_attention_bf16_packed(const void* X, const void* Wqkv, const float* bqkv, const int32_t* key_mask,
                                              const int32_t* cu_seqlens, void* ctx, int B, int L, int heads, int ldx, int ldw,
                                              const ufnd_gemm_ln* ln, void* stream_) {
  UFND_REQUIRE(X && Wqkv && ctx, "qkv_attention: null operand");
  UFND_REQUIRE(L == 128 && heads >= 2 && heads % 2 == 0 && heads <= 64 && B >= 1 && B <= 16384,
               "qkv_attention: B=%d L=%d heads=%d (this kernel is built for 128-token samples and an even head count; "
               "use ufnd_gemm_bf16[_ln] + ufnd_attention_bf16 otherwise)", B, L, heads);
  const int H = heads * 64;
  UFND_REQUIRE(ldx % 8 == 0 && ldw % 8 == 0 && ldx >= H && ldw >= H && ufnd_aligned(X, 16) && ufnd_aligned(Wqkv, 16) && ufnd_aligned(ctx, 16),
               "qkv_attention: strides must be multiples of 8 and pointers 16-B aligned");
  UFND_REQUIRE(!bqkv || ufnd_aligned(bqkv, 16), "qkv_attention: bias alignment");
  GemmArgs a{(const __bf16*)X, (const __bf16*)Wqkv, bqkv, nullptr, nullptr, nullptr, B * L, 3 * H, H, ldx, ldw, 0, 0, 0, UFND_ACT_NONE, 0, 0, nullptr};
  if (ln && ln->a_stats) {
    UFND_REQUIRE(ln->colsum && ufnd_aligned(ln->colsum, 16) && ufnd_aligned(ln->a_stats, 16), "qkv_attention: colsum / a_stats alignment");
    UFND_REQUIRE(ln->a_parts >= 2 && ln->a_parts <= 24 && ln->a_parts % 2 == 0 && ln->width > 0, "qkv_attention: a_parts=%d width=%d", ln->a_parts, ln->width);
    a.a_stats = ln->a_stats; a.colsum = ln->colsum; a.a_parts = ln->a_parts; a.a_eps = ln->a_eps;
    a.inv_h = 1.0f / (float)ln->width;
    a.guard = ln->guard;
  }
  a.att_mask = key_mask;
  a.att_cu = cu_seqlens;
  a.m_live = cu_seqlens ? cu_seqlens + B : nullptr;
  a.att_ctx = (__bf16*)ctx;
  a.att_h = H;
  a.att_scale_log2e = 0.125f * 1.44269504088896340736f;
  a.m_tiles = B;
  a.n_tiles = heads / 2;
  a.xcd_cols = (a.n_tiles % 2 == 0 && a.m_tiles >= 4) ? 2 : 1;
  hipLaunchKernelGGL((gemm_bf16_kernel<128, 384, 2, 4, 3, 2, 16, 0, 0, 1, 1>), dim3(a.m_tiles * a.n_tiles), dim3(512), 0, (hipStream_t)stream_, a);
  UFND_CHECK_LAUNCH();
  return UFND_OK;
}

extern "C" int ufnd_gemm_bf16(const void* A, const void* W, const float* bias, const float* residual, void* out_bf16,
                              float* out_f32, int M, int N, int K, int lda, int ldw, int ldr, int ldo, int ldf, int act,
                              void* stream_) {
  return ufnd_gemm_bf16_ex(A, W, bias, residual, out_bf16, out_f32, M, N, K, lda, ldw, ldr, ldo, ldf, act, -1, stream_);
}

extern "C" int ufnd_cast_bf16(const float* src, void* dst, size_t n, void* stream_) {
  UFND_REQUIRE(src && dst && n > 0, "cast_bf16: null argument");
  UFND_REQUIRE(ufnd_aligned(src, 16) && ufnd_aligned(dst, 8), "cast_bf16: alignment");
  size_t want = (n / 4 + 255) / 256;
  const int blocks = (int)(want < 1 ? 1 : (want > 4096 ? 4096 : want));
  hipLaunchKernelGGL(cast_bf16_kernel, dim3(blocks), dim3(256), 0, (hipStream_t)stream_, src, (__bf16*)dst, n);
  UFND_CHECK_LAUNCH();
  return UFND_OK;
}
```

### ultrafnd_git_amd/csrc/gemm_bf16_kernel.hpp

```cpp
#pragma once
#ifndef UFND_GEMM_OUT_NT
#define UFND_GEMM_OUT_NT 0
#endif

#include <type_traits>

#include "common.hpp"
#include "attn_softmax.hpp"

#pragma clang fp contract(off)

#ifndef UFND_GEMM_ILV
#define UFND_GEMM_ILV 1
#endif

namespace {

constexpr int BK = 64;

struct GemmArgs {
  const __bf16* A;
  const __bf16* W;
  const float* bias;
  const float* residual;
  __bf16* out_bf16;
  float* out_f32;
  int M, N, K, lda, ldw, ldr, ldo, ldf, act;
  int m_tiles, n_tiles;
  unsigned long long* stamps;
  const float* a_stats;
  const float* colsum;
  const float* r_stats;
  const float* r_gamma;
  const float* r_beta;
  float* out_stats;
  int a_parts, r_parts;
  float a_eps, r_eps, inv_h;
  const int32_t* att_mask;
  __bf16* att_ctx;
  int att_h;
  int xcd_cols;
  float att_scale_log2e;
  const __bf16* residual_b;
  int ldrb;
  int ksplit;
  size_t slab_stride;
  const __bf16* aux;
  int ldaux;
  float* guard;
  int pp_rows;
  const int* m_live;
  const int32_t* att_cu;
};

__device__ __forceinline__ void dma16(const void* gsrc, void* lds_dst) {
  __builtin_amdgcn_global_load_lds((const void __attribute__((address_space(1)))*)gsrc,
                                   (void __attribute__((address_space(3)))*)lds_dst, 16, 0, 0);
}

__device__ __forceinline__ float opaque_f(float x) {
  asm volatile("" : "+v"(x));
  return x;
}
__device__ __forceinline__ f32x2 opaque_f2(f32x2 x) {
  asm volatile("" : "+v"(x));
  return x;
}

__device__ __forceinline__ bf16x8 lds_frag(const char* tile, int row, int chunk) {
  return *reinterpret_cast<const bf16x8*>(tile + row * 128 + ((chunk ^ ((row >> 1) & 7)) << 4));
}

template <int N>
__device__ __forceinline__ void wait_vmcnt() {
  static_assert(N >= 0 && N <= 63, "vmcnt range");
  asm volatile("s_waitcnt vmcnt(%0)" ::"n"(N) : "memory");
}

template <int V> struct IntC { static constexpr int value = V; };

constexpr int gemm_waves_per_simd(int BM, int BN, int WM, int WN, int STA, int STB, int MI, int LNX, int ATT) {
  const int ring = (STA * BM + STB * BN) * 128, cbytes = WM * WN * MI * (BN / WN + 4) * 4;
  const int smem = (ring > cbytes ? ring : cbytes) + (LNX ? BM * 8 + 64 : 0);
  return (!ATT && smem <= 80 * 1024 ? 2 : 1) * WM * WN / 4;
}
template <int BM, int BN, int WM, int WN, int STA, int STB, int MI, int ABL = 0, int DBG = 0, int LNX = 0, int ATT = 0, int BWD = 0>
__global__ __launch_bounds__(WM * WN * 64) __attribute__((amdgpu_waves_per_eu(gemm_waves_per_simd(BM, BN, WM, WN, STA, STB, MI, LNX, ATT))))
void gemm_bf16_kernel(const GemmArgs a) {
  static_assert(!BWD || (!LNX && !ATT && !ABL && !DBG), "backward forms are plain kernels");
  static_assert(MI == 16 || MI == 32, "MFMA shape");
  static_assert(!ATT || (BM == 128 && BN == 384 && MI == 16 && WM * WN == 8 && LNX == 1), "fused attention tile");
  using acc_t = typename std::conditional<MI == 16, f32x4, f32x16>::type;
  constexpr int AR = MI * MI / 64;
  constexpr int KQ = MI == 16 ? 1 : 2;
  constexpr int NW = WM * WN;
  constexpr int TM = BM / WM, TN = BN / WN;
  constexpr int MT = TM / MI, NT = TN / MI;
  constexpr int ASLOT = BM * 128, BSLOT = BN * 128;
  constexpr int DA = STA - 1, DB = STB - 1;
  constexpr int APIECES = BM / 8, BPIECES = BN / 8;
  constexpr int PWA = APIECES / NW, PWB = (BPIECES + NW - 1) / NW;
  constexpr int WAITN = PWA * (DA - 1 > 0 ? DA - 1 : 0) + PWB * (DB - 1 > 0 ? DB - 1 : 0);
  constexpr int CP = TN + 4;
  constexpr int CBYTES = NW * MI * CP * 4;
  constexpr int RING = STA * ASLOT + STB * BSLOT;
  constexpr int ATT_OFF = (CBYTES + 1023) & ~1023;
  constexpr int ATT_END = ATT ? ATT_OFF + 6 * 16384 + 512 : 0;
  constexpr int STAT_OFF0 = (RING > CBYTES) ? RING : CBYTES;
  constexpr int STAT_OFF = STAT_OFF0 > ATT_END ? STAT_OFF0 : ATT_END;
  constexpr int SMEM = STAT_OFF + (LNX ? BM * 8 + 64 : 0);
  static_assert(SMEM <= 160 * 1024, "LDS budget");
  static_assert(APIECES % NW == 0 && TM % MI == 0 && TN % MI == 0, "tile split");
  static_assert(STB >= 2 && (STA == STB || STA == STB + 1), "ring depths");
  static_assert(WAITN <= 63, "vmcnt range");
  __shared__ __attribute__((aligned(16))) char smem[SMEM];

  unsigned long long stamp[10];
  if constexpr (DBG) {
    stamp[0] = __builtin_amdgcn_s_memtime();
    stamp[1] = __builtin_amdgcn_s_memrealtime();
  }

  int mlive = a.M, m_tiles = a.m_tiles;
  if constexpr (!BWD && !ATT) {
    if (a.m_live) {
      const int v = __builtin_amdgcn_readfirstlane(*a.m_live);
      mlive = v < a.M ? (v > 0 ? v : 0) : a.M;
      m_tiles = (mlive + BM - 1) / BM;
      if ((int)blockIdx.x >= m_tiles * a.n_tiles) return;
    }
  }
  const int nblk = m_tiles * a.n_tiles;
  int bid, kslice = 0;
  {
    const int ngrid = BWD ? nblk * (a.ksplit > 1 ? a.ksplit : 1) : nblk;
    const int q = ngrid >> 3, r = ngrid & 7, xcd = blockIdx.x & 7, idx = blockIdx.x >> 3;
    bid = (xcd < r ? xcd * (q + 1) : r * (q + 1) + (xcd - r) * q) + idx;
    if constexpr (BWD) {
      kslice = bid / nblk;
      bid -= kslice * nblk;
    }
  }
  int tm = bid / a.n_tiles, tn = bid % a.n_tiles;
  if (a.xcd_cols == 2) {
    const int nh = a.n_tiles >> 1, per_half = m_tiles * nh;
    const int half = bid / per_half, rem = bid - half * per_half;
    tm = rem / nh;
    tn = half * nh + (rem - tm * nh);
  }
  const int m0 = tm * BM, n0 = tn * BN;
  int arow0 = m0, alen = BM;
  if constexpr (ATT) {
    if (a.att_cu) {
      mlive = __builtin_amdgcn_readfirstlane(*a.m_live);
      arow0 = __builtin_amdgcn_readfirstlane(a.att_cu[tm]);
      alen = __builtin_amdgcn_readfirstlane(a.att_cu[tm + 1]) - arow0;
      if (alen <= 0) return;
    }
  } else {
    alen = mlive - m0;
  }
  const int wave = __builtin_amdgcn_readfirstlane(threadIdx.x >> 6), lane = threadIdx.x & 63;
  const int wm = wave / WN, wn = wave % WN, fr = lane & (MI - 1), g = lane / MI;

  acc_t acc[MT][NT];
#pragma unroll
  for (int i = 0; i < MT; ++i)
#pragma unroll
    for (int j = 0; j < NT; ++j)
#pragma unroll
      for (int r = 0; r < AR; ++r) acc[i][j][r] = 0.f;

  int nk = a.K / BK, kbase = 0;
  if constexpr (BWD) {
    if (a.ksplit > 1) {
      const int per = (nk + a.ksplit - 1) / a.ksplit;
      kbase = kslice * per * BK;
      nk = nk - kslice * per < per ? nk - kslice * per : per;
    }
  }
  const int prow = lane >> 3, ppos = lane & 7;
  auto issueA = [&](int t) {
    char* buf = smem + (t % STA) * ASLOT;
    const int k0 = kbase + t * BK;
#pragma unroll
    for (int ii = 0; ii < PWA; ++ii) {
      const int p = wave + NW * ii;
      const int r = 8 * p + prow;
      const int c = ppos ^ ((r >> 1) & 7);
      int gr = arow0 + r;
      gr = gr < mlive ? gr : mlive - 1;
      dma16(a.A + (size_t)gr * a.lda + k0 + c * 8, buf + p * 1024);
    }
  };
  auto issueB = [&](int t) {
    char* buf = smem + STA * ASLOT + (t % STB) * BSLOT;
    const int k0 = kbase + t * BK;
#pragma unroll
    for (int ii = 0; ii < PWB; ++ii) {
      int p = wave + NW * ii;
      if constexpr (BPIECES % NW != 0) p = p < BPIECES ? p : p - BPIECES;
      const int r = 8 * p + prow;
      const int c = ppos ^ ((r >> 1) & 7);
      int gr = n0 + r;
      gr = gr < a.N ? gr : a.N - 1;
      if constexpr (ATT) gr = (r >> 7) * a.att_h + tn * 128 + (r & 127);
      dma16(a.W + (size_t)gr * a.ldw + k0 + c * 8, buf + p * 1024);
    }
  };
  constexpr int TPR = NW * 64 / BM;
  static_assert(!LNX || TPR == 2 || TPR == 4, "threads per tile row");
  constexpr int GPT = 4 / (TPR < 4 ? TPR : 4);
  f32x4 sv[GPT][3];
  f32x2* st_lds = reinterpret_cast<f32x2*>(smem + STAT_OFF);
  const float* sp = nullptr;
  if constexpr (LNX) {
    sp = a.a_stats ? a.a_stats : a.r_stats;
    if (sp) {
      const int parts = a.a_stats ? a.a_parts : a.r_parts;
      int row = arow0 + (int)threadIdx.x / TPR;
      row = row < mlive ? row : mlive - 1;
      const f32x4* base = reinterpret_cast<const f32x4*>(sp + (size_t)row * parts * 2);
      const int nq = parts >> 1, sub = threadIdx.x % TPR;
#pragma unroll
      for (int gi = 0; gi < GPT; ++gi)
#pragma unroll
        for (int u = 0; u < 3; ++u) {
          const int q = (sub + gi * TPR) + 4 * u;
          asm volatile("global_load_dwordx4 %0, %1, off" : "=v"(sv[gi][u]) : "v"(base + (q < nq ? q : 0)) : "memory");
        }
    }
  }
  int att_mk = 1;
  if constexpr (ATT) {
    if (a.att_mask && threadIdx.x < BM) att_mk = a.att_mask[m0 + threadIdx.x];
  }
#pragma unroll
  for (int s = 0; s < STA; ++s) {
    if (s < STB && s < nk) issueB(s);
    if (s < nk) issueA(s);
  }

  if constexpr (LNX) {
    if (sp) {
      constexpr int NPRO = STA * PWA + STB * PWB;
      static_assert(NPRO <= 63, "vmcnt range");
      if (STA <= nk) {
        if constexpr (GPT == 1)
          asm volatile("s_waitcnt vmcnt(%3)" : "+v"(sv[0][0]), "+v"(sv[0][1]), "+v"(sv[0][2]) : "n"(NPRO) : "memory");
        else
          asm volatile("s_waitcnt vmcnt(%6)" : "+v"(sv[0][0]), "+v"(sv[0][1]), "+v"(sv[0][2]), "+v"(sv[GPT - 1][0]), "+v"(sv[GPT - 1][1]),
                       "+v"(sv[GPT - 1][2]) : "n"(NPRO) : "memory");
      } else {
        if constexpr (GPT == 1)
          asm volatile("s_waitcnt vmcnt(0)" : "+v"(sv[0][0]), "+v"(sv[0][1]), "+v"(sv[0][2]) : : "memory");
        else
          asm volatile("s_waitcnt vmcnt(0)" : "+v"(sv[0][0]), "+v"(sv[0][1]), "+v"(sv[0][2]), "+v"(sv[GPT - 1][0]), "+v"(sv[GPT - 1][1]),
                       "+v"(sv[GPT - 1][2]) : : "memory");
      }
      const int nq_ = (a.a_stats ? a.a_parts : a.r_parts) >> 1, sub_ = threadIdx.x % TPR;
      float gs[GPT], gq[GPT];
#pragma unroll
      for (int gi = 0; gi < GPT; ++gi) {
#pragma unroll
        for (int u = 0; u < 3; ++u) {
          if ((sub_ + gi * TPR) + 4 * u >= nq_) sv[gi][u] = f32x4{0.f, 0.f, 0.f, 0.f};
        }
        gs[gi] = sv[gi][0][0] + sv[gi][0][2];
        gq[gi] = sv[gi][0][1] + sv[gi][0][3];
#pragma unroll
        for (int u = 1; u < 3; ++u) { gs[gi] += sv[gi][u][0] + sv[gi][u][2]; gq[gi] += sv[gi][u][1] + sv[gi][u][3]; }
      }
      float sm, sq;
      if constexpr (TPR == 4) {
        sm = gs[0] + quad_xor1(gs[0]);
        sq = gq[0] + quad_xor1(gq[0]);
        sm += quad_xor2(sm);
        sq += quad_xor2(sq);
      } else {
        const float s01 = gs[0] + quad_xor1(gs[0]), s23 = gs[1] + quad_xor1(gs[1]);
        const float q01 = gq[0] + quad_xor1(gq[0]), q23 = gq[1] + quad_xor1(gq[1]);
        sm = s01 + s23;
        sq = q01 + q23;
      }
      const float mean = __fmul_rn(sm, a.inv_h);
      const float var = fmaxf(__fmaf_rn(-mean, mean, __fmul_rn(sq, a.inv_h)), 0.f);
      const float rstd = __builtin_amdgcn_rsqf(__fadd_rn(var, a.a_stats ? a.a_eps : a.r_eps));
      if (threadIdx.x % TPR == 0) st_lds[threadIdx.x / TPR] = f32x2{mean, rstd};
      if (a.guard && a.a_stats) {
        float ratio = __fmul_rn(fabsf(mean), rstd);
        ratio = ratio == ratio ? ratio : INFINITY;
        const float worst = wave_max(threadIdx.x % TPR == 0 && (int)threadIdx.x / TPR < alen ? ratio : 0.0f);
        if (lane == 0) reinterpret_cast<float*>(smem + STAT_OFF + BM * 8)[wave] = worst;
      }
      asm volatile("s_waitcnt lgkmcnt(0)" ::: "memory");
    }
  }

  bf16x8 af0[KQ][MT], bf0[KQ][NT], af1[KQ][MT], bf1[KQ][NT];
  auto read_half = [&](int t, auto kk_, bf16x8 (&af)[KQ][MT], bf16x8 (&bfr)[KQ][NT]) {
    constexpr int kk = decltype(kk_)::value;
    const char* At = smem + (t % STA) * ASLOT;
    const char* Bt = smem + STA * ASLOT + (t % STB) * BSLOT;
#pragma unroll
    for (int q = 0; q < KQ; ++q) {
      const int chunk = MI == 16 ? g + 4 * kk : g + 2 * q + 4 * kk;
#pragma unroll
      for (int i = 0; i < MT; ++i) af[q][i] = lds_frag(At, wm * TM + i * MI + fr, chunk);
#pragma unroll
      for (int j = 0; j < NT; ++j) bfr[q][j] = lds_frag(Bt, wn * TN + j * MI + fr, chunk);
    }
  };
  auto mma_half = [&](const bf16x8 (&af)[KQ][MT], const bf16x8 (&bfr)[KQ][NT]) {
#pragma unroll
    for (int q = 0; q < KQ; ++q)
#pragma unroll
      for (int i = 0; i < MT; ++i)
#pragma unroll
        for (int j = 0; j < NT; ++j) {
          if constexpr (MI == 16) acc[i][j] = __builtin_amdgcn_mfma_f32_16x16x32_bf16(af[q][i], bfr[q][j], acc[i][j], 0, 0, 0);
          else acc[i][j] = __builtin_amdgcn_mfma_f32_32x32x16_bf16(af[q][i], bfr[q][j], acc[i][j], 0, 0, 0);
        }
  };
  constexpr int NMF = KQ * MT * NT, NRD = KQ * (MT + NT);
  constexpr bool ILV = UFND_GEMM_ILV != 0;
  auto body = [&](int t, auto ia_, auto ib_, auto next_) {
    constexpr bool IA = decltype(ia_)::value != 0, IB = decltype(ib_)::value != 0, NEXT = decltype(next_)::value != 0;
    if constexpr (ABL != 1) {
      read_half(t, IntC<1>{}, af1, bf1);
      mma_half(af0, bf0);
      if constexpr (ILV) {
#pragma unroll
        for (int q = 0; q < (NRD < NMF ? NRD : NMF - 1); ++q) {
          __builtin_amdgcn_sched_group_barrier(0x008, 1, 0);
          __builtin_amdgcn_sched_group_barrier(0x100, 1, 0);
        }
        __builtin_amdgcn_sched_group_barrier(0x100, NRD - (NRD < NMF ? NRD : NMF - 1), 0);
        __builtin_amdgcn_sched_group_barrier(0x008, NMF - (NRD < NMF ? NRD : NMF - 1), 0);
      } else {
        __builtin_amdgcn_sched_group_barrier(0x008, 1, 0);
        __builtin_amdgcn_sched_group_barrier(0x100, NRD, 0);
        __builtin_amdgcn_sched_group_barrier(0x008, NMF - 1, 0);
      }
    }
    if constexpr (NEXT) {
      __builtin_amdgcn_sched_barrier(0);
      if (t + STA - 1 < nk) wait_vmcnt<WAITN>();
      else wait_vmcnt<0>();
      asm volatile("s_waitcnt lgkmcnt(0)" ::: "memory");
      __builtin_amdgcn_s_barrier();
      __builtin_amdgcn_sched_barrier(0);
      if constexpr (ABL != 1) read_half(t + 1, IntC<0>{}, af0, bf0);
      if constexpr (ABL != 2) {
        if constexpr (IB) issueB(t + STB);
        if constexpr (IA) issueA(t + STA);
      }
    }
    if constexpr (ABL != 1) {
      mma_half(af1, bf1);
      constexpr int PW = (ABL == 2 || !NEXT) ? 0 : (IA ? PWA : 0) + (IB ? PWB : 0);
      constexpr int GRP = (NMF - 1) / (PW + 1) > 0 ? (NMF - 1) / (PW + 1) : 1;
      if constexpr (ILV && NEXT && NRD + PW < NMF) {
#pragma unroll
        for (int q = 0; q < NRD; ++q) {
          __builtin_amdgcn_sched_group_barrier(0x008, 1, 0);
          __builtin_amdgcn_sched_group_barrier(0x100, 1, 0);
        }
        constexpr int REST = NMF - NRD, G2 = REST / (PW + 1) > 0 ? REST / (PW + 1) : 1;
#pragma unroll
        for (int q = 0; q < PW; ++q) {
          __builtin_amdgcn_sched_group_barrier(0x008, G2, 0);
          __builtin_amdgcn_sched_group_barrier(0x020, 1, 0);
        }
        __builtin_amdgcn_sched_group_barrier(0x008, REST - G2 * PW > 0 ? REST - G2 * PW : 0, 0);
      } else {
        __builtin_amdgcn_sched_group_barrier(0x008, 1, 0);
        if constexpr (NEXT) __builtin_amdgcn_sched_group_barrier(0x100, NRD, 0);
#pragma unroll
        for (int q = 0; q < PW; ++q) {
          __builtin_amdgcn_sched_group_barrier(0x008, GRP, 0);
          __builtin_amdgcn_sched_group_barrier(0x020, 1, 0);
        }
        __builtin_amdgcn_sched_group_barrier(0x008, NMF - 1 - GRP * PW > 0 ? NMF - 1 - GRP * PW : 0, 0);
      }
    }
  };

  if (STA <= nk) wait_vmcnt<PWA * (STA - 1) + PWB * (STB - 1)>();
  else wait_vmcnt<0>();
  __builtin_amdgcn_sched_barrier(0);
  __builtin_amdgcn_s_barrier();
  __builtin_amdgcn_sched_barrier(0);
  if constexpr (DBG) {
    stamp[2] = __builtin_amdgcn_s_memtime();
    stamp[3] = __builtin_amdgcn_s_memrealtime();
  }
  if constexpr (ABL != 1) read_half(0, IntC<0>{}, af0, bf0);
  int t = 0;
  for (; t + STA < nk; ++t) body(t, IntC<1>{}, IntC<1>{}, IntC<1>{});
  for (; t + STB < nk; ++t) body(t, IntC<0>{}, IntC<1>{}, IntC<1>{});
  for (; t + 1 < nk; ++t) body(t, IntC<0>{}, IntC<0>{}, IntC<1>{});
  body(t, IntC<0>{}, IntC<0>{}, IntC<0>{});
  __builtin_amdgcn_sched_barrier(0);
  __builtin_amdgcn_s_barrier();
  __builtin_amdgcn_sched_barrier(0);
  if constexpr (DBG) {
    stamp[4] = __builtin_amdgcn_s_memtime();
    stamp[5] = __builtin_amdgcn_s_memrealtime();
  }

  float bj[NT], csj[NT];
#pragma unroll
  for (int j = 0; j < NT; ++j) { bj[j] = 0.f; csj[j] = 0.f; }
  auto gcol = [&](int c) { return ATT ? (c >> 7) * a.att_h + tn * 128 + (c & 127) : n0 + c; };
  if (a.bias) {
#pragma unroll
    for (int j = 0; j < NT; ++j) bj[j] = a.bias[gcol(wn * TN + j * MI + fr)];
  }
  bool fold = false, rln = false;
  if constexpr (LNX) {
    fold = a.a_stats != nullptr;
    rln = a.r_stats != nullptr;
    if (fold) {
#pragma unroll
      for (int j = 0; j < NT; ++j) csj[j] = a.colsum[gcol(wn * TN + j * MI + fr)];
    }
  }
  float* cst = reinterpret_cast<float*>(smem) + wave * MI * CP;
  float* const outf = (BWD && a.out_f32) ? a.out_f32 + (size_t)kslice * a.slab_stride : a.out_f32;
  constexpr int CPR = TN / 8;
  constexpr int CHUNKS = MI * CPR;
  constexpr int NIT = (CHUNKS + 63) / 64;
  constexpr bool FIXCOL = (64 % CPR) == 0;
  auto ld8 = [&](const float* ptr, float (&o)[8]) {
    const f32x4 x0 = *reinterpret_cast<const f32x4*>(ptr), x1 = *reinterpret_cast<const f32x4*>(ptr + 4);
#pragma unroll
    for (int q = 0; q < 4; ++q) { o[q] = x0[q]; o[4 + q] = x1[q]; }
  };
  float g8[8], b8[8];
  if constexpr (LNX && FIXCOL) {
    if (rln) {
      const int col = n0 + wn * TN + (lane % CPR) * 8;
      ld8(a.r_gamma + col, g8);
      ld8(a.r_beta + col, b8);
    }
  }
  auto epilogue = [&](auto act_, auto mode_) {
    constexpr int ACT = decltype(act_)::value;
    constexpr bool FOLD = LNX && decltype(mode_)::value == 1, RLN = LNX && decltype(mode_)::value == 2;
    constexpr bool RES = !FOLD;
#pragma unroll
    for (int i = 0; i < MT; ++i) {
      float rr8[RES ? NIT : 1][8];
      if constexpr (RES) if (a.residual && !(BWD && a.aux)) {
#pragma unroll
        for (int it = 0; it < NIT; ++it) {
          const int id = lane + 64 * it;
          if (id < CHUNKS) {
            int row = m0 + wm * TM + i * MI + id / CPR;
            row = row < a.M ? row : a.M - 1;
            ld8(a.residual + (size_t)row * a.ldr + n0 + wn * TN + (id % CPR) * 8, rr8[it]);
          }
        }
      }
      if constexpr (BWD) {
        if (a.aux) {
#pragma unroll
          for (int it = 0; it < NIT; ++it) {
            const int id = lane + 64 * it;
            if (id < CHUNKS) {
              int row = m0 + wm * TM + i * MI + id / CPR;
              row = row < a.M ? row : a.M - 1;
              const bf16x8 xb = *reinterpret_cast<const bf16x8*>(a.aux + (size_t)row * a.ldaux + n0 + wn * TN + (id % CPR) * 8);
#pragma unroll
              for (int q = 0; q < 8; ++q) rr8[it][q] = (float)xb[q];
            }
          }
        }
      }
      if constexpr (LNX && RES) {
        if (a.residual_b) {
#pragma unroll
          for (int it = 0; it < NIT; ++it) {
            const int id = lane + 64 * it;
            if (id < CHUNKS) {
              int row = m0 + wm * TM + i * MI + id / CPR;
              row = row < a.M ? row : a.M - 1;
              const bf16x8 rb = *reinterpret_cast<const bf16x8*>(a.residual_b + (size_t)row * a.ldrb + n0 + wn * TN + (id % CPR) * 8);
#pragma unroll
              for (int q = 0; q < 8; ++q) rr8[it][q] = (float)rb[q];
            }
          }
        }
      }
#pragma unroll
      for (int r = 0; r < AR; r += 2) {
        const int prow_ = MI == 16 ? 4 * g + r : 8 * (r >> 2) + 4 * g + (r & 3);
        f32x2 mean2 = {0.f, 0.f}, rstd2 = {1.f, 1.f};
        if constexpr (FOLD) {
          const f32x2 a0 = st_lds[wm * TM + i * MI + prow_], a1 = st_lds[wm * TM + i * MI + prow_ + 1];
          mean2 = f32x2{a0[0], a1[0]};
          rstd2 = f32x2{a0[1], a1[1]};
        }
#pragma unroll
        for (int j = 0; j < NT; ++j) {
          f32x2 v = {acc[i][j][r], acc[i][j][r + 1]};
          if constexpr (FOLD) v = opaque_f2(rstd2 * __builtin_elementwise_fma(-mean2, f32x2{csj[j], csj[j]}, v));
          v = v + f32x2{bj[j], bj[j]};
          if constexpr (ACT == UFND_ACT_GELU) v = gelu_fast_f2(v);
          else if constexpr (ACT == UFND_ACT_QUICK_GELU) v = quick_gelu_fast_f2(v);
          cst[prow_ * CP + j * MI + fr] = v.x;
          cst[(prow_ + 1) * CP + j * MI + fr] = v.y;
        }
      }
      asm volatile("s_waitcnt lgkmcnt(0)" ::: "memory");
#pragma unroll
      for (int it = 0; it < NIT; ++it) {
        const int id = lane + 64 * it;
        if (id >= CHUNKS) break;
        const int rr = id / CPR, cl = (id % CPR) * 8;
        const int row = m0 + wm * TM + i * MI + rr;
        const int col = n0 + wn * TN + cl;
        const bool live = row < mlive;
        const f32x4 v0 = *reinterpret_cast<const f32x4*>(cst + rr * CP + cl);
        const f32x4 v1 = *reinterpret_cast<const f32x4*>(cst + rr * CP + cl + 4);
        float v[8] = {v0[0], v0[1], v0[2], v0[3], v1[0], v1[1], v1[2], v1[3]};
        if constexpr (BWD) {
          if (a.aux) {
            if (a.act == UFND_ACT_GELU_BWD) {
#pragma unroll
              for (int q = 0; q < 8; ++q) v[q] = v[q] * gelu_grad_f(rr8[it][q]);
            } else {
#pragma unroll
              for (int q = 0; q < 8; ++q) v[q] = v[q] * quick_gelu_grad_f(rr8[it][q]);
            }
          }
        }
        if constexpr (RES) if ((a.residual && !(BWD && a.aux)) || (LNX && a.residual_b)) {
          if constexpr (RLN) {
            const f32x2 ms = st_lds[wm * TM + i * MI + rr];
            if constexpr (!FIXCOL) {
              ld8(a.r_gamma + col, g8);
              ld8(a.r_beta + col, b8);
            }
#pragma unroll
            for (int q = 0; q < 8; ++q) rr8[it][q] = __fmaf_rn(__fmul_rn(__fsub_rn(rr8[it][q], ms[0]), ms[1]), g8[q], b8[q]);
          }
#pragma unroll
          for (int q = 0; q < 8; ++q) v[q] = __fadd_rn(v[q], rr8[it][q]);
        }
        if constexpr (LNX && RES) {
          if (a.out_stats) {
            if constexpr (CPR % 4 == 0) {
              float sm = 0.f, sq = 0.f;
#pragma unroll
              for (int q = 0; q < 8; ++q) { sm = __fadd_rn(sm, v[q]); sq = __fmaf_rn(v[q], v[q], sq); }
              sm += quad_xor1(sm);
              sq += quad_xor1(sq);
              sm += quad_xor2(sm);
              sq += quad_xor2(sq);
              if (live && (id & 3) == 0)
                *reinterpret_cast<f32x2*>(a.out_stats + ((size_t)row * (a.N >> 5) + (col >> 5)) * 2) = f32x2{sm, sq};
            }
          }
        }
        if constexpr (ATT) {
          const int ct = wn * TN + cl;
          const int trow = wm * TM + i * MI + rr, img = ct >> 6, ch = (ct & 63) >> 3;
          bf16x8 o;
#pragma unroll
          for (int q = 0; q < 8; ++q) o[q] = (__bf16)v[q];
          const int sw = img >= 4 ? (ch ^ (((trow >> 1) & 3) << 1)) : (ch ^ ((trow >> 1) & 7));
          *reinterpret_cast<bf16x8*>(smem + ATT_OFF + img * 16384 + trow * 128 + (sw << 4)) = o;
          continue;
        }
        if (!live) continue;
        if (a.out_f32) {
          float* op = outf + (size_t)row * a.ldf + col;
          *reinterpret_cast<f32x4*>(op) = f32x4{v[0], v[1], v[2], v[3]};
          *reinterpret_cast<f32x4*>(op + 4) = f32x4{v[4], v[5], v[6], v[7]};
        }
        if (a.out_bf16) {
          bf16x8 o;
#pragma unroll
          for (int q = 0; q < 8; ++q) o[q] = (__bf16)v[q];
          if constexpr (UFND_GEMM_OUT_NT && !BWD) __builtin_nontemporal_store(o, reinterpret_cast<bf16x8*>(a.out_bf16 + (size_t)row * a.ldo + col));
          else *reinterpret_cast<bf16x8*>(a.out_bf16 + (size_t)row * a.ldo + col) = o;
        }
      }
      asm volatile("s_waitcnt lgkmcnt(0)" ::: "memory");
    }
  };
  if constexpr (LNX) {
    if (fold) {
      if (a.act == UFND_ACT_GELU) epilogue(IntC<UFND_ACT_GELU>{}, IntC<1>{});
      else if (a.act == UFND_ACT_QUICK_GELU) epilogue(IntC<UFND_ACT_QUICK_GELU>{}, IntC<1>{});
      else epilogue(IntC<UFND_ACT_NONE>{}, IntC<1>{});
    } else if (rln) {
      epilogue(IntC<UFND_ACT_NONE>{}, IntC<2>{});
    } else {
      epilogue(IntC<UFND_ACT_NONE>{}, IntC<0>{});
    }
  } else {
    if (a.act == UFND_ACT_GELU) epilogue(IntC<UFND_ACT_GELU>{}, IntC<0>{});
    else if (a.act == UFND_ACT_QUICK_GELU) epilogue(IntC<UFND_ACT_QUICK_GELU>{}, IntC<0>{});
    else epilogue(IntC<UFND_ACT_NONE>{}, IntC<0>{});
  }
  if constexpr (ATT && DBG) {
    stamp[8] = __builtin_amdgcn_s_memtime();
    stamp[9] = __builtin_amdgcn_s_memrealtime();
  }
  if constexpr (ATT) {
    constexpr float NEG_MASK = -3.0e38f;
    float* kbias = reinterpret_cast<float*>(smem + ATT_OFF + 6 * 16384);
    if (threadIdx.x < BM) kbias[threadIdx.x] = att_mk != 0 ? 0.0f : NEG_MASK;
    __syncthreads();
    const int hh = wave >> 2, wq = wave & 3, g4 = lane >> 4, f16 = lane & 15;
    const char* qimg = smem + ATT_OFF + hh * 16384;
    const char* kimg = smem + ATT_OFF + (2 + hh) * 16384;
    const char* vimg = smem + ATT_OFF + (4 + hh) * 16384;
    bf16x8 qf[2][2];
#pragma unroll
    for (int qt = 0; qt < 2; ++qt) {
      const int q = wq * 32 + qt * 16 + f16;
      qf[qt][0] = lds_frag(qimg, q, g4);
      qf[qt][1] = lds_frag(qimg, q, g4 + 4);
    }
    f32x4 o[4][2];
#pragma unroll
    for (int dt = 0; dt < 4; ++dt)
#pragma unroll
      for (int qt = 0; qt < 2; ++qt) o[dt][qt] = f32x4{0.f, 0.f, 0.f, 0.f};
    float m_run[2] = {-INFINITY, -INFINITY}, l_run[2] = {0.f, 0.f};
    constexpr int KB = 64, KT = KB / 16;
    if (wq * 32 < alen) {
#pragma unroll
    for (int kb0 = 0; kb0 < BM; kb0 += KB) {
      const char* ks = kimg + kb0 * 128;
      const char* vs = vimg + kb0 * 128;
      if (masked_block_is_noop(kbias + kb0, lane, m_run)) continue;
      f32x4 sc[KT][2];
#pragma unroll
      for (int kt = 0; kt < KT; ++kt)
#pragma unroll
        for (int qt = 0; qt < 2; ++qt) sc[kt][qt] = f32x4{0.f, 0.f, 0.f, 0.f};
#pragma unroll
      for (int kk = 0; kk < 2; ++kk)
#pragma unroll
        for (int kt = 0; kt < KT; ++kt) {
          const bf16x8 kf = lds_frag(ks, kt * 16 + f16, g4 + 4 * kk);
#pragma unroll
          for (int qt = 0; qt < 2; ++qt) sc[kt][qt] = __builtin_amdgcn_mfma_f32_16x16x32_bf16(kf, qf[qt][kk], sc[kt][qt], 0, 0, 0);
        }
      const bool any_masked = __any(kbias[kb0 + lane] != 0.0f);
      bf16x8 pf[KT / 2][2];
#pragma unroll
      for (int qt = 0; qt < 2; ++qt) {
        const float alpha = online_softmax_block<KT>(sc, qt, kbias + kb0, any_masked, g4, a.att_scale_log2e, m_run[qt], l_run[qt], pf);
        if (!__all(alpha == 1.0f)) {
#pragma unroll
          for (int dt = 0; dt < 4; ++dt) o[dt][qt] *= alpha;
        }
      }
#pragma unroll
      for (int ksd = 0; ksd < KT / 2; ++ksd) {
#pragma unroll
        for (int dt = 0; dt < 4; ++dt) {
          const int qq = f16 >> 2, pp = f16 & 3;
          const int key0 = 32 * ksd + 4 * g4 + qq;
          const int ch = 2 * dt + (pp >> 1);
          const int off0 = key0 * 128 + ((ch ^ (((key0 >> 1) & 3) << 1)) << 4) + 8 * (pp & 1);
          const int key1 = key0 + 16;
          const int off1 = key1 * 128 + ((ch ^ (((key1 >> 1) & 3) << 1)) << 4) + 8 * (pp & 1);
          const s16x4 t0 = __builtin_amdgcn_ds_read_tr16_b64_v4i16((s16x4 __attribute__((address_space(3)))*)(vs + off0));
          const s16x4 t1 = __builtin_amdgcn_ds_read_tr16_b64_v4i16((s16x4 __attribute__((address_space(3)))*)(vs + off1));
          union { s16x4 s2[2]; bf16x8 v; } u;
          u.s2[0] = t0;
          u.s2[1] = t1;
#pragma unroll
          for (int qt = 0; qt < 2; ++qt) o[dt][qt] = __builtin_amdgcn_mfma_f32_16x16x32_bf16(u.v, pf[ksd][qt], o[dt][qt], 0, 0, 0);
        }
      }
    }
    }
#pragma unroll
    for (int qt = 0; qt < 2; ++qt) {
      float l = l_run[qt];
      l += __shfl_xor(l, 16, 64);
      l += __shfl_xor(l, 32, 64);
      const float inv = 1.0f / l;
      const int q = wq * 32 + qt * 16 + f16;
      if (q >= alen) continue;
      __bf16* dst = a.att_ctx + (size_t)(arow0 + q) * a.att_h + (tn * 2 + hh) * 64 + 4 * g4;
#pragma unroll
      for (int dt = 0; dt < 4; ++dt) {
        bf16x4 ov = {(__bf16)(o[dt][qt][0] * inv), (__bf16)(o[dt][qt][1] * inv), (__bf16)(o[dt][qt][2] * inv), (__bf16)(o[dt][qt][3] * inv)};
        *reinterpret_cast<bf16x4*>(dst + dt * 16) = ov;
      }
    }
  }
  if constexpr (LNX) {
    if (a.guard && a.a_stats && threadIdx.x == 0) {
      const float* gw = reinterpret_cast<const float*>(smem + STAT_OFF + BM * 8);
      float worst = gw[0];
#pragma unroll
      for (int w = 1; w < NW; ++w) worst = fmaxf(worst, gw[w]);
      atomicMax(reinterpret_cast<int*>(a.guard + (blockIdx.x & 1023)), __float_as_int(worst));
    }
  }
  if constexpr (DBG) {
    asm volatile("s_waitcnt vmcnt(0)" ::: "memory");
    stamp[6] = __builtin_amdgcn_s_memtime();
    stamp[7] = __builtin_amdgcn_s_memrealtime();
    if (threadIdx.x == 0) {
      constexpr int NS = ATT ? 10 : 8;
#pragma unroll
      for (int i = 0; i < NS; ++i) a.stamps[(size_t)blockIdx.x * NS + i] = stamp[i];
    }
  }
}

}

#define UFND_GEMM_TILES(X)                                                                             \
  X(0, 128, 128, 2, 2, 3, 3, 16, 0, 0)                                                              \
  X(1, 128, 64, 2, 2, 3, 3, 16, 0, 0)                                                 \
  X(2, 256, 128, 4, 2, 3, 3, 16, 1, 1)                                                              \
  X(3, 128, 128, 2, 2, 2, 2, 16, 1, 0)                                                \
  X(4, 128, 64, 2, 2, 4, 4, 16, 0, 0)                                                               \
  X(5, 256, 64, 4, 2, 3, 3, 16, 0, 0)                                                               \
  X(6, 128, 288, 2, 2, 3, 3, 16, 0, 0)                                   \
  X(7, 128, 96, 2, 2, 3, 3, 16, 0, 0)                                     \
  X(8, 256, 192, 4, 2, 2, 2, 16, 1, 1)                                  \
  X(9, 128, 384, 2, 2, 2, 2, 16, 0, 0)                                                              \
  X(10, 128, 192, 2, 2, 3, 3, 16, 0, 0)                                                             \
  X(11, 128, 96, 2, 2, 4, 4, 16, 0, 0)                                                              \
  X(12, 64, 96, 1, 2, 4, 4, 16, 0, 0)                     \
  X(13, 64, 192, 1, 2, 3, 3, 16, 0, 0)                                                              \
  X(14, 128, 256, 2, 2, 2, 2, 16, 0, 0)                                                             \
  X(15, 256, 256, 4, 2, 2, 2, 16, 1, 1)                                                             \
  X(16, 128, 128, 4, 2, 3, 3, 16, 1, 1)                                  \
  X(17, 128, 192, 4, 2, 3, 3, 16, 1, 1)                                  \
  X(18, 256, 64, 4, 2, 4, 4, 16, 0, 0)                                                              \
  X(19, 64, 64, 1, 2, 4, 4, 16, 0, 0)                                                 \
  X(20, 128, 64, 4, 2, 4, 4, 16, 1, 1)                                   \
  X(21, 256, 192, 2, 4, 2, 2, 16, 0, 0)                                          \
  X(22, 256, 192, 4, 2, 3, 2, 16, 1, 1)                                 \
  X(23, 256, 256, 4, 2, 3, 2, 16, 0, 0)                                                             \
  X(24, 128, 192, 4, 2, 4, 4, 16, 0, 0)                                                             \
  X(25, 128, 256, 4, 2, 3, 3, 16, 0, 0)                                 \
  X(26, 256, 192, 4, 2, 2, 2, 32, 0, 0)   \
  X(27, 128, 128, 4, 2, 3, 3, 32, 0, 0)                                                                    \
  X(28, 256, 144, 8, 1, 2, 2, 16, 1, 1)   \
  X(29, 128, 128, 4, 2, 2, 2, 16, 1, 0)

#ifdef UFND_DIAG
#define UFND_TILE_BUILT(PROD_) 1
#else
#define UFND_TILE_BUILT(PROD_) (PROD_)
#endif

struct TileCfg { int bm, bn, threads, wn, lnx, built; };
static const TileCfg kTiles[] = {
#define X(id, BM_, BN_, WM_, WN_, SA_, SB_, MI_, LN_, PROD_) {BM_, BN_, WM_ * WN_ * 64, WN_, LN_, UFND_TILE_BUILT(PROD_)},
    UFND_GEMM_TILES(X)
#undef X
};
constexpr int kNumTiles = sizeof(kTiles) / sizeof(kTiles[0]);

static int xcd_cols_for(int M, int N, int K, int m_tiles, int n_tiles) {
#ifdef UFND_DIAG
  static const int forced = [] { const char* e = getenv("UFND_GEMM_XCD_COLS"); return e ? atoi(e) : 0; }();
  if (forced == 1) return 1;
  if (forced == 2) return (n_tiles % 2 == 0) ? 2 : 1;
#endif
  (void)K;
  return (4LL * N > (long long)M && n_tiles % 2 == 0 && m_tiles >= 4) ? 2 : 1;
}

static int launch_cfg(int cfg, int mode, GemmArgs& a, hipStream_t stream) {
  if (cfg < 0 || cfg >= kNumTiles || !kTiles[cfg].built) {
    ufnd_set_error("gemm_bf16: tile config %d is not part of this library", cfg);
    return UFND_ERR_INVALID;
  }
  const TileCfg& t = kTiles[cfg];
  a.m_tiles = ufnd_cdiv(a.M, t.bm);
  a.n_tiles = a.N / t.bn;
  a.xcd_cols = xcd_cols_for(a.M, a.N, a.K, a.m_tiles, a.n_tiles);
  const dim3 grid(a.m_tiles * a.n_tiles * (mode == 6 && a.ksplit > 1 ? a.ksplit : 1)), block(t.threads);
#ifdef UFND_GEMM_ONLY_BWD
#define X(id, BM_, BN_, WM_, WN_, SA_, SB_, MI_, LN_, PROD_)                                                                      \
  case id:                                                                                                                        \
    if constexpr (id == 15 || id == 16 || id == 17 || id == 20 || id == 22) {                                                     \
      hipLaunchKernelGGL((gemm_bf16_kernel<BM_, BN_, WM_, WN_, SA_, SB_, MI_, 0, 0, 0, 0, 1>), grid, block, 0, stream, a);        \
    } else {                                                                                                                      \
      ufnd_set_error("gemm_bf16 backward: tile %d has no backward kernel", id);                                                   \
      return UFND_ERR_INVALID;                                                                                                    \
    }                                                                                                                             \
    break;
  (void)mode;
  switch (cfg) {
    UFND_GEMM_TILES(X)
    default: ufnd_set_error("gemm_bf16: unknown tile config %d", cfg); return UFND_ERR_INVALID;
  }
#undef X
  return UFND_OK;
#else
#ifdef UFND_DIAG
#define UFND_DIAG_LAUNCH(BM_, BN_, WM_, WN_, SA_, SB_, MI_)                                                                             \
  else if (mode == 5) hipLaunchKernelGGL((gemm_bf16_kernel<BM_, BN_, WM_, WN_, SA_, SB_, MI_, 0, 1, 1>), grid, block, 0, stream, a);   \
  else if (mode == 1) hipLaunchKernelGGL((gemm_bf16_kernel<BM_, BN_, WM_, WN_, SA_, SB_, MI_, 1, 0>), grid, block, 0, stream, a);      \
  else if (mode == 2) hipLaunchKernelGGL((gemm_bf16_kernel<BM_, BN_, WM_, WN_, SA_, SB_, MI_, 2, 0>), grid, block, 0, stream, a);      \
  else if (mode == 3) hipLaunchKernelGGL((gemm_bf16_kernel<BM_, BN_, WM_, WN_, SA_, SB_, MI_, 0, 1>), grid, block, 0, stream, a);
#else
#define UFND_DIAG_LAUNCH(BM_, BN_, WM_, WN_, SA_, SB_, MI_)
#endif
#define X(id, BM_, BN_, WM_, WN_, SA_, SB_, MI_, LN_, PROD_)                                                        \
  case id:                                                                                                          \
    if constexpr (UFND_TILE_BUILT(PROD_) != 0) {                                                                    \
      if (mode == 0) {                                                                                              \
        hipLaunchKernelGGL((gemm_bf16_kernel<BM_, BN_, WM_, WN_, SA_, SB_, MI_, 0, 0>), grid, block, 0, stream, a); \
      } else if constexpr (LN_ != 0) {    \
        if (mode == 4) hipLaunchKernelGGL((gemm_bf16_kernel<BM_, BN_, WM_, WN_, SA_, SB_, MI_, 0, 0, 1>), grid, block, 0, stream, a); \
        UFND_DIAG_LAUNCH(BM_, BN_, WM_, WN_, SA_, SB_, MI_)                                                         \
        else {                                                                                                      \
          ufnd_set_error("gemm_bf16: tile %d has no kernel for mode %d in this library", id, mode);                 \
          return UFND_ERR_INVALID;                                                                                  \
        }                                                                                                           \
      } else {                                                                                                      \
        ufnd_set_error("gemm_bf16: tile %d has no diagnostics / LayerNorm-aware build", id);                        \
        return UFND_ERR_INVALID;                                                                                    \
      }                                                                                                             \
    }                                                                                                               \
    break;
  switch (cfg) {
    UFND_GEMM_TILES(X)
    default: ufnd_set_error("gemm_bf16: unknown tile config %d", cfg); return UFND_ERR_INVALID;
  }
#undef X
#undef UFND_DIAG_LAUNCH
  return UFND_OK;
#endif
}

static int auto_cfg(int M, int N, int K) {
#ifdef UFND_DIAG
  static const int forced = [] { const char* e = getenv("UFND_GEMM_FORCE_CFG"); return e ? atoi(e) : -1; }();
  if (forced >= 0 && forced < kNumTiles && N % kTiles[forced].bn == 0) return forced;
#endif
  auto tiles = [&](int cfg) { return (long long)ufnd_cdiv(M, kTiles[cfg].bm) * (N / kTiles[cfg].bn); };
  if (N % 256 == 0 && N >= 3072 && tiles(15) >= 512) return 15;
  if (N % 256 == 0 && N >= 2048 && tiles(15) >= 190 && tiles(15) <= 256) return 15;
  if (N % 192 == 0 && tiles(22) >= 160) return 22;
  if (N >= 2048) {
    if (N % 192 == 0 && N >= 3072) return 17;
    if (N % 128 == 0) return 16;
  }
  if (N < 2048 && N % 192 == 0 && tiles(17) >= 150 && tiles(17) <= 256) return 17;
  if (N % 128 == 0 && tiles(16) >= 150) return 16;
  return 20;
}
```

### ultrafnd_git_amd/encoders.py

```python
from __future__ import annotations

from collections import OrderedDict
from typing import Dict, Optional, Tuple

import torch
import torch.nn as nn

from . import _lib as L

ACT_NONE, ACT_GELU, ACT_QUICK_GELU = 0, 1, 2


def _bf16(t: torch.Tensor) -> torch.Tensor:
    t = t.contiguous()
    out = torch.empty(t.shape, dtype=torch.bfloat16, device=t.device)
    L.check(L.lib().ufnd_cast_bf16(t.data_ptr(), out.data_ptr(), t.numel(), L.stream_ptr(t.device)), "ufnd_cast_bf16")
    return out


def dropout_prob(name: str, p) -> float:
    p = float(p)
    if not 0.0 <= p < 1.0:
        raise ValueError(f"{name}={p!r}: a dropout probability in [0, 1)")
    return p


class _EncoderBase(nn.Module):

    FOLD_GUARD_MAX = 4.0

    def __init__(self):
        super().__init__()
        self.tiles = {}
        self._guard: Optional[torch.Tensor] = None
        self._w: "OrderedDict[str, torch.Tensor]" = OrderedDict()
        self._packed: Optional[dict] = None
        self._bufs: Dict[Tuple, dict] = {}
        self.weights_version = 0

    def state_dict(self, *args, **kwargs):
        return OrderedDict((k, v.detach().clone()) for k, v in self._w.items())

    def load_state_dict(self, sd, strict: bool = True):
        missing = [k for k in self._w if k not in sd]
        unexpected = [k for k in sd if k not in self._w]
        if strict and missing:
            raise RuntimeError(f"missing keys: {missing[:5]}{'...' if len(missing) > 5 else ''}")
        for k in self._w:
            if k in sd:
                if tuple(sd[k].shape) != tuple(self._w[k].shape):
                    raise RuntimeError(f"shape mismatch for {k}: {tuple(sd[k].shape)} vs {tuple(self._w[k].shape)}")
                self._w[k].copy_(sd[k].to(self._w[k].device, torch.float32))
        self._packed = None
        self.weights_version += 1
        return missing, unexpected

    def _apply(self, fn, recurse=True):
        super()._apply(fn, recurse)
        for k in self._w:
            self._w[k] = fn(self._w[k]).float()
        self._packed = None
        self._bufs.clear()
        self.weights_version += 1
        return self

    @property
    def device(self) -> torch.device:
        return next(iter(self._w.values())).device

    def _require_hip(self):
        if self.device.type != "cuda":
            raise L.UltrafndHipError(f"{type(self).__name__} runs on a HIP device only: call .to('cuda') (no CPU fallback)")

    tiles: Dict[str, int] = {}

    _m_live: Optional[int] = None

    def _gemm(self, A, W, bias, out_bf16=None, out_f32=None, residual=None, act=ACT_NONE, M=None, which=None):
        M = A.shape[0] if M is None else M
        N, K = W.shape
        L.check(L.lib().ufnd_gemm_bf16_live(A.data_ptr(), W.data_ptr(), L.ptr(bias), L.ptr(residual), L.ptr(out_bf16),
                                            L.ptr(out_f32), M, N, K, A.stride(0), W.stride(0),
                                            residual.stride(0) if residual is not None else 0,
                                            out_bf16.stride(0) if out_bf16 is not None else 0,
                                            out_f32.stride(0) if out_f32 is not None else 0, act, self.tiles.get(which, -1),
                                            self._m_live, L.stream_ptr(A.device)), "ufnd_gemm_bf16_live")

    def _gemm_ln(self, A, W, bias, out_bf16=None, out_f32=None, residual=None, act=ACT_NONE, a_stats=None, colsum=None,
                 r_stats=None, r_gamma=None, r_beta=None, out_stats=None, eps=1e-5, which=None, residual_bf16=None):
        M = A.shape[0]
        N, K = W.shape
        ln = L.GemmLn()
        ln.a_stats, ln.colsum = L.ptr(a_stats), L.ptr(colsum)
        ln.r_stats, ln.r_gamma, ln.r_beta = L.ptr(r_stats), L.ptr(r_gamma), L.ptr(r_beta)
        ln.out_stats = L.ptr(out_stats)
        ln.a_parts = a_stats.shape[1] if a_stats is not None else 0
        ln.r_parts = r_stats.shape[1] if r_stats is not None else 0
        ln.a_eps = ln.r_eps = eps
        ln.width = self.hidden
        ln.tile_cfg = self.tiles.get(which, -1)
        if residual_bf16 is not None:
            ln.residual_bf16, ln.ldrb = residual_bf16.data_ptr(), residual_bf16.stride(0)
        if a_stats is not None:
            ln.guard = self._guard_buf(A.device).data_ptr()
        import ctypes
        L.check(L.lib().ufnd_gemm_bf16_ln_live(A.data_ptr(), W.data_ptr(), L.ptr(bias), L.ptr(residual), L.ptr(out_bf16),
                                               L.ptr(out_f32), M, N, K, A.stride(0), W.stride(0),
                                               residual.stride(0) if residual is not None else 0,
                                               out_bf16.stride(0) if out_bf16 is not None else 0,
                                               out_f32.stride(0) if out_f32 is not None else 0, act, ctypes.byref(ln),
                                               self._m_live, L.stream_ptr(A.device)), "ufnd_gemm_bf16_ln_live")

    def _guard_buf(self, dev) -> torch.Tensor:
        if self._guard is None or self._guard.device != dev:
            self._guard = torch.zeros(L.FOLD_GUARD_SLOTS, dtype=torch.float32, device=dev)
        return self._guard

    def fold_ratio(self) -> float:
        return 0.0 if self._guard is None else float(self._guard.max().cpu())

    def check_fold(self, reset: bool = True, ratio: Optional[float] = None) -> bool:
        r = self.fold_ratio() if ratio is None else float(ratio)
        if reset and self._guard is not None:
            self._guard.zero_()
        if self.fold_ln and r > self.FOLD_GUARD_MAX:
            import warnings
            warnings.warn(f"{type(self).__name__}: a residual-stream row with |mean|/std = {r:.1f} (> {self.FOLD_GUARD_MAX}) went through a "
                          "folded LayerNorm; switching to materialised LayerNorms (fold_ln=False)")
            self.fold_ln = False
            self._bufs.clear()
            return True
        return False

    @staticmethod
    def _fold(W, b, gamma, beta):
        Wp = _bf16(W * gamma[None, :])
        return Wp, Wp.float().sum(1).contiguous(), (b + (W * beta[None, :]).sum(1)).contiguous()

    def _ln(self, x, ldx, gamma, beta, out_bf16, out_f32, M, H, eps):
        if self._m_live is not None:
            L.check(L.lib().ufnd_layernorm_live(x.data_ptr(), ldx, gamma.data_ptr(), beta.data_ptr(), L.ptr(out_bf16),
                                                L.ptr(out_f32), M, H, eps, self._m_live, L.stream_ptr(x.device)), "ufnd_layernorm_live")
            return
        L.check(L.lib().ufnd_layernorm(x.data_ptr(), ldx, gamma.data_ptr(), beta.data_ptr(), L.ptr(out_bf16),
                                       L.ptr(out_f32), M, H, eps, L.stream_ptr(x.device)), "ufnd_layernorm")

    def _qkv_attn(self, A, W, bias, mask_i32, ctx, B, Lq, heads, a_stats=None, colsum=None, eps=1e-5, cu=None):
        import ctypes
        ln = None
        if a_stats is not None:
            ln = L.GemmLn()
            ln.a_stats, ln.colsum, ln.a_parts, ln.a_eps, ln.r_eps, ln.width = a_stats.data_ptr(), colsum.data_ptr(), a_stats.shape[1], eps, eps, self.hidden
            ln.guard = self._guard_buf(A.device).data_ptr()
        L.check(L.lib().ufnd_qkv_attention_bf16_packed(A.data_ptr(), W.data_ptr(), L.ptr(bias), L.ptr(mask_i32), L.ptr(cu), ctx.data_ptr(),
                                                       B, Lq, heads, A.stride(0), W.stride(0), ctypes.byref(ln) if ln is not None else None,
                                                       L.stream_ptr(A.device)), "ufnd_qkv_attention_bf16_packed")

    def _attn(self, qkv, mask_i32, ctx, B, Lq, heads):
        L.check(L.lib().ufnd_attention_bf16(qkv.data_ptr(), L.ptr(mask_i32), ctx.data_ptr(), B, Lq, heads,
                                            L.stream_ptr(qkv.device)), "ufnd_attention_bf16")


class BertTextEncoder(_EncoderBase):
    def __init__(self, layers: int = 12, hidden: int = 768, heads: int = 12, intermediate: int = 3072,
                 vocab_size: int = 30522, max_position: int = 512, type_vocab: int = 2, eps: float = 1e-12,
                 fold_ln: bool = True, residual_dtype: str = "bf16", hidden_dropout_prob: float = 0.0,
                 attention_probs_dropout_prob: float = 0.0):
        super().__init__()
        self.fold_ln = fold_ln
        self.hidden_dropout_prob = dropout_prob("hidden_dropout_prob", hidden_dropout_prob)
        self.attention_probs_dropout_prob = dropout_prob("attention_probs_dropout_prob", attention_probs_dropout_prob)
        if residual_dtype not in ("fp32", "bf16"):
            raise ValueError(f"residual_dtype={residual_dtype!r}: 'fp32' or 'bf16'")
        self.residual_dtype = residual_dtype
        self.fuse_qkv_attention = True
        if hidden != heads * 64:
            raise ValueError("head_dim must be 64 (hidden == heads * 64)")
        self.layers, self.hidden, self.heads, self.inter, self.vocab, self.eps = layers, hidden, heads, intermediate, vocab_size, eps
        self.max_position = max_position
        w = self._w
        g = torch.Generator().manual_seed(0)

        def init(shape, std=0.02):
            return torch.randn(shape, generator=g) * std
        w["embeddings.word_embeddings.weight"] = init((vocab_size, hidden))
        w["embeddings.position_embeddings.weight"] = init((max_position, hidden))
        w["embeddings.token_type_embeddings.weight"] = init((type_vocab, hidden))
        w["embeddings.LayerNorm.weight"] = torch.ones(hidden)
        w["embeddings.LayerNorm.bias"] = torch.zeros(hidden)
        for i in range(layers):
            P = f"encoder.layer.{i}."
            for n in ("query", "key", "value"):
                w[P + f"attention.self.{n}.weight"] = init((hidden, hidden))
                w[P + f"attention.self.{n}.bias"] = torch.zeros(hidden)
            w[P + "attention.output.dense.weight"] = init((hidden, hidden))
            w[P + "attention.output.dense.bias"] = torch.zeros(hidden)
            w[P + "attention.output.LayerNorm.weight"] = torch.ones(hidden)
            w[P + "attention.output.LayerNorm.bias"] = torch.zeros(hidden)
            w[P + "intermediate.dense.weight"] = init((intermediate, hidden))
            w[P + "intermediate.dense.bias"] = torch.zeros(intermediate)
            w[P + "output.dense.weight"] = init((hidden, intermediate))
            w[P + "output.dense.bias"] = torch.zeros(hidden)
            w[P + "output.LayerNorm.weight"] = torch.ones(hidden)
            w[P + "output.LayerNorm.bias"] = torch.zeros(hidden)

    def _pack(self):
        if self._packed is None:
            w, layers = self._w, []
            for i in range(self.layers):
                P = f"encoder.layer.{i}."
                layers.append({
                    "wqkv": _bf16(torch.cat([w[P + f"attention.self.{n}.weight"] for n in ("query", "key", "value")], 0)),
                    "bqkv": torch.cat([w[P + f"attention.self.{n}.bias"] for n in ("query", "key", "value")], 0).contiguous(),
                    "wo": _bf16(w[P + "attention.output.dense.weight"]), "bo": w[P + "attention.output.dense.bias"],
                    "g1": w[P + "attention.output.LayerNorm.weight"], "b1": w[P + "attention.output.LayerNorm.bias"],
                    "w1": _bf16(w[P + "intermediate.dense.weight"]), "bi": w[P + "intermediate.dense.bias"],
                    "w2": _bf16(w[P + "output.dense.weight"]), "b2": w[P + "output.dense.bias"],
                    "g2": w[P + "output.LayerNorm.weight"], "b2n": w[P + "output.LayerNorm.bias"]})
                ly = layers[-1]
                ly["w1f"], ly["cs1"], ly["bif"] = self._fold(w[P + "intermediate.dense.weight"], ly["bi"], ly["g1"], ly["b1"])
                if i > 0:
                    prev = layers[-2]
                    wq = torch.cat([w[P + f"attention.self.{n}.weight"] for n in ("query", "key", "value")], 0)
                    ly["wqkvf"], ly["csqkv"], ly["bqkvf"] = self._fold(wq, ly["bqkv"], prev["g2"], prev["b2n"])
            self._packed = {"layers": layers}
        return self._packed

    def _workbufs(self, B: int, Lq: int) -> dict:
        key = (B, Lq)
        if key not in self._bufs:
            dev, M, H = self.device, B * Lq, self.hidden
            bf, f32 = dict(dtype=torch.bfloat16, device=dev), dict(dtype=torch.float32, device=dev)
            self._bufs[key] = {"xb": torch.empty(M, H, **bf), "xf": torch.empty(M, H, **f32), "y": torch.empty(M, H, **f32),
                               "x1b": torch.empty(M, H, **bf), "x1f": torch.empty(M, H, **f32),
                               "qkv": torch.empty(M, 3 * H, **bf), "ctx": torch.empty(M, H, **bf),
                               "h": torch.empty(M, self.inter, **bf), "feat": torch.empty(B, H, **f32),
                               "cu": torch.zeros(B + 1, dtype=torch.int32, device=dev), "row_src": torch.zeros(M, dtype=torch.int32, device=dev)}
            p1 = L.lib().ufnd_gemm_bf16_stat_parts(M, H, H)
            p2 = L.lib().ufnd_gemm_bf16_stat_parts(M, H, self.inter)
            if self.fold_ln and p1 > 0 and p1 == p2 and p1 % 2 == 0:
                self._bufs[key].update({"y2": torch.empty(M, H, **f32), "y1b": torch.empty(M, H, **bf), "y2b": torch.empty(M, H, **bf),
                                        "st": torch.zeros(2 * self.layers, M, p1, 2, **f32)})
                self._guard_buf(dev)
        return self._bufs[key]

    @torch.no_grad()
    def last_hidden_state(self, input_ids: torch.Tensor, attention_mask: torch.Tensor, n_layers: Optional[int] = None) -> torch.Tensor:
        self._require_hip()
        dev = self.device
        B, Lq = input_ids.shape
        if Lq > self.max_position:
            raise RuntimeError(f"sequence length {Lq} exceeds max_position_embeddings {self.max_position}")
        ids = input_ids.to(dev, torch.int64).contiguous()
        mask = attention_mask.to(dev, torch.int32).contiguous()
        self._mask_i32 = mask
        p, b, w = self._pack(), self._workbufs(B, Lq), self._w
        M, H = B * Lq, self.hidden
        L.check(L.lib().ufnd_bert_embed(ids.data_ptr(), w["embeddings.word_embeddings.weight"].data_ptr(),
                                        w["embeddings.position_embeddings.weight"].data_ptr(),
                                        w["embeddings.token_type_embeddings.weight"].data_ptr(),
                                        w["embeddings.LayerNorm.weight"].data_ptr(), w["embeddings.LayerNorm.bias"].data_ptr(),
                                        b["xb"].data_ptr(), None if ("st" in b and self.residual_dtype == "bf16") else b["xf"].data_ptr(),
                                        B, Lq, H, self.vocab, self.eps, L.stream_ptr(dev)), "ufnd_bert_embed")
        fused = (B, Lq, mask) if (self.fuse_qkv_attention and Lq == 128 and self.heads % 2 == 0) else None
        if n_layers is not None:
            p = {"layers": p["layers"][:max(1, int(n_layers))]}
        self._layers(p, b, M, lambda qkv, ctx: self._attn(qkv, mask, ctx, B, Lq, self.heads), fused)
        return b["xf"].view(B, Lq, H)

    def _layers(self, p, b, M, attn, fused=None) -> None:
        H = self.hidden
        v = {k: (x[:M] if torch.is_tensor(x) and x.dim() >= 2 and x.shape[0] >= M and k not in ("feat", "st") else x) for k, x in b.items()}
        cu = fused[3] if fused is not None and len(fused) > 3 else None
        if "st" in b:
            return self._layers_folded(p, v, M, attn, fused)
        for ly in p["layers"]:
            if fused is not None:
                self._qkv_attn(v["xb"], ly["wqkv"], ly["bqkv"], fused[2], v["ctx"], fused[0], fused[1], self.heads, cu=cu)
            else:
                self._gemm(v["xb"], ly["wqkv"], ly["bqkv"], out_bf16=v["qkv"], which="qkv")
                attn(v["qkv"], v["ctx"])
            self._gemm(v["ctx"], ly["wo"], ly["bo"], out_f32=v["y"], residual=v["xf"], which="out")
            self._ln(v["y"], H, ly["g1"], ly["b1"], v["x1b"], v["x1f"], M, H, self.eps)
            self._gemm(v["x1b"], ly["w1"], ly["bi"], out_bf16=v["h"], act=ACT_GELU, which="ffn1")
            self._gemm(v["h"], ly["w2"], ly["b2"], out_f32=v["y"], residual=v["x1f"], which="ffn2")
            self._ln(v["y"], H, ly["g2"], ly["b2n"], v["xb"], v["xf"], M, H, self.eps)

    def _layers_folded(self, p, b, M, attn, fused=None) -> None:
        H, eps = self.hidden, self.eps
        y1, y2 = b["y"], b["y2"]
        st = b["st"]
        cu = fused[3] if fused is not None and len(fused) > 3 else None
        prev = None
        for i, ly in enumerate(p["layers"]):
            st1, st2 = st[2 * i][:M], st[2 * i + 1][:M]
            stp = st[2 * i - 1][:M] if i > 0 else None
            if fused is not None:
                if prev is None:
                    self._qkv_attn(b["xb"], ly["wqkv"], ly["bqkv"], fused[2], b["ctx"], fused[0], fused[1], self.heads, cu=cu)
                else:
                    self._qkv_attn(b["y2b"], ly["wqkvf"], ly["bqkvf"], fused[2], b["ctx"], fused[0], fused[1], self.heads,
                                   a_stats=stp, colsum=ly["csqkv"], eps=eps, cu=cu)
            elif prev is None:
                self._gemm(b["xb"], ly["wqkv"], ly["bqkv"], out_bf16=b["qkv"], which="qkv")
            else:
                self._gemm_ln(b["y2b"], ly["wqkvf"], ly["bqkvf"], out_bf16=b["qkv"], a_stats=stp, colsum=ly["csqkv"], eps=eps, which="qkv")
            if fused is None:
                attn(b["qkv"], b["ctx"])
            rb = self.residual_dtype == "bf16"
            last = i == len(p["layers"]) - 1
            if prev is None:
                self._gemm_ln(b["ctx"], ly["wo"], ly["bo"], out_f32=None if rb else y1, out_bf16=b["y1b"], residual=None if rb else b["xf"],
                              residual_bf16=b["xb"] if rb else None, out_stats=st1, eps=eps, which="out")
            else:
                self._gemm_ln(b["ctx"], ly["wo"], ly["bo"], out_f32=None if rb else y1, out_bf16=b["y1b"], residual=None if rb else y2,
                              residual_bf16=b["y2b"] if rb else None, r_stats=stp, r_gamma=prev["g2"], r_beta=prev["b2n"], out_stats=st1,
                              eps=eps, which="out")
            self._gemm_ln(b["y1b"], ly["w1f"], ly["bif"], out_bf16=b["h"], act=ACT_GELU, a_stats=st1, colsum=ly["cs1"], eps=eps, which="ffn1")
            self._gemm_ln(b["h"], ly["w2"], ly["b2"], out_f32=y2 if (last or not rb) else None, out_bf16=b["y2b"], residual=None if rb else y1,
                          residual_bf16=b["y1b"] if rb else None, r_stats=st1, r_gamma=ly["g1"], r_beta=ly["b1"], out_stats=st2, eps=eps,
                          which="ffn2")
            prev = ly
        self._ln(y2, H, prev["g2"], prev["b2n"], None, b["xf"], M, H, eps)

    @torch.no_grad()
    def forward(self, input_ids: torch.Tensor, attention_mask: torch.Tensor, unpad: bool = True, strict: bool = False) -> torch.Tensor:
        if strict:
            rd, self.residual_dtype = self.residual_dtype, "fp32"
            try:
                if self.fold_ln:
                    out = self.forward(input_ids, attention_mask, unpad=unpad)
                    if not self.check_fold():
                        return out
                return self.forward(input_ids, attention_mask, unpad=unpad)
            finally:
                self.residual_dtype = rd
        if unpad:
            return self._forward_live(input_ids, attention_mask)
        hid = self.last_hidden_state(input_ids, attention_mask)
        B, Lq, H = hid.shape
        feat = self._workbufs(B, Lq)["feat"]
        L.check(L.lib().ufnd_masked_meanpool_l2(hid.data_ptr(), self._mask_i32.data_ptr(), feat.data_ptr(), B, Lq, H,
                                                L.stream_ptr(self.device)), "ufnd_masked_meanpool_l2")
        return feat

    def _forward_live(self, input_ids: torch.Tensor, attention_mask: torch.Tensor) -> torch.Tensor:
        self._require_hip()
        dev = self.device
        B, Lq = input_ids.shape
        if Lq > self.max_position:
            raise RuntimeError(f"sequence length {Lq} exceeds max_position_embeddings {self.max_position}")
        ids = input_ids.to(dev, torch.int64).contiguous()
        mask = attention_mask.to(dev, torch.int32).contiguous()
        p, b, w = self._pack(), self._workbufs(B, Lq), self._w
        M, H, s = B * Lq, self.hidden, L.stream_ptr(dev)
        cu, feat = b["cu"], b["feat"]
        live = cu.data_ptr() + 4 * B
        L.check(L.lib().ufnd_text_pack(mask.data_ptr(), B, Lq, cu.data_ptr(), b["row_src"].data_ptr(), s), "ufnd_text_pack")
        L.check(L.lib().ufnd_bert_embed_live(ids.data_ptr(), b["row_src"].data_ptr(), live, w["embeddings.word_embeddings.weight"].data_ptr(),
                                             w["embeddings.position_embeddings.weight"].data_ptr(),
                                             w["embeddings.token_type_embeddings.weight"].data_ptr(),
                                             w["embeddings.LayerNorm.weight"].data_ptr(), w["embeddings.LayerNorm.bias"].data_ptr(),
                                             b["xb"].data_ptr(), None if ("st" in b and self.residual_dtype == "bf16") else b["xf"].data_ptr(),
                                             M, Lq, H, self.vocab, self.eps, s), "ufnd_bert_embed_live")
        fused = (B, Lq, mask, cu) if (self.fuse_qkv_attention and Lq == 128 and self.heads % 2 == 0) else None

        def attn(qkv, ctx):
            L.check(L.lib().ufnd_attention_bf16_varlen_masked(qkv.data_ptr(), cu.data_ptr(), mask.data_ptr(), ctx.data_ptr(), B, Lq,
                                                              self.heads, s), "ufnd_attention_bf16_varlen_masked")
        self._m_live = live
        try:
            self._layers(p, b, M, attn, fused)
        finally:
            self._m_live = None
        L.check(L.lib().ufnd_masked_meanpool_l2_live(b["xf"].data_ptr(), mask.data_ptr(), cu.data_ptr(), feat.data_ptr(), B, Lq, H, s),
                "ufnd_masked_meanpool_l2_live")
        return feat

    encode_batch = forward

    @torch.no_grad()
    def encode_fields(self, input_ids: torch.Tensor, attention_mask: torch.Tensor, part_valid: torch.Tensor,
                      chunk: int = 1024, unpad: bool = True) -> torch.Tensor:
        self._require_hip()
        dev = self.device
        N, Mx, Lq = input_ids.shape
        valid = part_valid.to(dev, torch.int32).contiguous()
        ids = input_ids.to(dev, torch.int64).reshape(N * Mx, Lq)
        mask = attention_mask.to(dev, torch.int32).reshape(N * Mx, Lq)
        rows = torch.nonzero(valid.reshape(-1), as_tuple=False).flatten()
        parts = torch.zeros(N * Mx, self.hidden, dtype=torch.float32, device=dev)
        for s0 in range(0, rows.numel(), chunk):
            r = rows[s0:s0 + chunk]
            parts[r] = self.forward(ids[r], mask[r], unpad=unpad, strict=True)
        out = torch.empty(N, self.hidden, dtype=torch.float32, device=dev)
        L.check(L.lib().ufnd_field_mean_l2(parts.data_ptr(), valid.data_ptr(), out.data_ptr(), N, Mx, self.hidden,
                                           L.stream_ptr(dev)), "ufnd_field_mean_l2")
        return out


class ClipVisualEncoder(_EncoderBase):
    def __init__(self, layers: int = 12, hidden: int = 768, heads: int = 12, intermediate: int = 3072, patch: int = 32,
                 image: int = 224, projection_dim: int = 512, eps: float = 1e-5, fold_ln: bool = True, residual_dtype: str = "bf16",
                 attention_dropout: float = 0.0):
        super().__init__()
        self.fold_ln = fold_ln
        self.attention_dropout = dropout_prob("attention_dropout", attention_dropout)
        if residual_dtype not in ("fp32", "bf16"):
            raise ValueError(f"residual_dtype={residual_dtype!r}: 'fp32' or 'bf16'")
        self.residual_dtype = residual_dtype
        if hidden != heads * 64:
            raise ValueError("head_dim must be 64 (hidden == heads * 64)")
        self.layers, self.hidden, self.heads, self.inter = layers, hidden, heads, intermediate
        self.patch, self.image, self.proj, self.eps = patch, image, projection_dim, eps
        self.n_patches = (image // patch) ** 2
        w, V = self._w, "vision_model."
        g = torch.Generator().manual_seed(0)

        def init(shape, std=0.02):
            return torch.randn(shape, generator=g) * std
        w[V + "embeddings.class_embedding"] = init((hidden,))
        w[V + "embeddings.patch_embedding.weight"] = init((hidden, 3, patch, patch))
        w[V + "embeddings.position_embedding.weight"] = init((self.n_patches + 1, hidden))
        w[V + "pre_layrnorm.weight"], w[V + "pre_layrnorm.bias"] = torch.ones(hidden), torch.zeros(hidden)
        for i in range(layers):
            P = V + f"encoder.layers.{i}."
            for n in ("k_proj", "v_proj", "q_proj", "out_proj"):
                w[P + f"self_attn.{n}.weight"] = init((hidden, hidden))
                w[P + f"self_attn.{n}.bias"] = torch.zeros(hidden)
            w[P + "layer_norm1.weight"], w[P + "layer_norm1.bias"] = torch.ones(hidden), torch.zeros(hidden)
            w[P + "mlp.fc1.weight"], w[P + "mlp.fc1.bias"] = init((intermediate, hidden)), torch.zeros(intermediate)
            w[P + "mlp.fc2.weight"], w[P + "mlp.fc2.bias"] = init((hidden, intermediate)), torch.zeros(hidden)
            w[P + "layer_norm2.weight"], w[P + "layer_norm2.bias"] = torch.ones(hidden), torch.zeros(hidden)
        w[V + "post_layernorm.weight"], w[V + "post_layernorm.bias"] = torch.ones(hidden), torch.zeros(hidden)
        w["visual_projection.weight"] = init((projection_dim, hidden))

    def _pack(self):
        if self._packed is None:
            w, V, layers = self._w, "vision_model.", []
            for i in range(self.layers):
                P = V + f"encoder.layers.{i}."
                layers.append({
                    "wqkv": _bf16(torch.cat([w[P + f"self_attn.{n}.weight"] for n in ("q_proj", "k_proj", "v_proj")], 0)),
                    "bqkv": torch.cat([w[P + f"self_attn.{n}.bias"] for n in ("q_proj", "k_proj", "v_proj")], 0).contiguous(),
                    "wo": _bf16(w[P + "self_attn.out_proj.weight"]), "bo": w[P + "self_attn.out_proj.bias"],
                    "g1": w[P + "layer_norm1.weight"], "b1": w[P + "layer_norm1.bias"],
                    "w1": _bf16(w[P + "mlp.fc1.weight"]), "bi": w[P + "mlp.fc1.bias"],
                    "w2": _bf16(w[P + "mlp.fc2.weight"]), "b2": w[P + "mlp.fc2.bias"],
                    "g2": w[P + "layer_norm2.weight"], "b2n": w[P + "layer_norm2.bias"]})
                ly = layers[-1]
                wq = torch.cat([w[P + f"self_attn.{n}.weight"] for n in ("q_proj", "k_proj", "v_proj")], 0)
                ly["wqkvf"], ly["csqkv"], ly["bqkvf"] = self._fold(wq, ly["bqkv"], ly["g1"], ly["b1"])
                ly["w1f"], ly["cs1"], ly["bif"] = self._fold(w[P + "mlp.fc1.weight"], ly["bi"], ly["g2"], ly["b2n"])
            self._packed = {"layers": layers,
                            "wpatch": _bf16(w[V + "embeddings.patch_embedding.weight"].reshape(self.hidden, -1)),
                            "wproj": _bf16(w["visual_projection.weight"])}
        return self._packed

    def _workbufs(self, B: int, Fr: int) -> dict:
        key = (B, Fr)
        if key not in self._bufs:
            dev, H, N = self.device, self.hidden, B * Fr
            T = self.n_patches + 1
            M = N * T
            bf, f32 = dict(dtype=torch.bfloat16, device=dev), dict(dtype=torch.float32, device=dev)
            self._bufs[key] = {"patches": torch.empty(N * self.n_patches, 3 * self.patch ** 2, **bf),
                               "pe": torch.empty(N * self.n_patches, H, **f32), "xf": torch.empty(M, H, **f32),
                               "hb": torch.empty(M, H, **bf), "qkv": torch.empty(M, 3 * H, **bf),
                               "ctx": torch.empty(M, H, **bf), "m": torch.empty(M, self.inter, **bf),
                               "pooled": torch.empty(N, H, **bf), "e": torch.empty(N, self.proj, **f32),
                               "feat": torch.empty(B, self.proj, **f32)}
            p1 = L.lib().ufnd_gemm_bf16_stat_parts(M, H, H)
            p2 = L.lib().ufnd_gemm_bf16_stat_parts(M, H, self.inter)
            if self.fold_ln and p1 > 0 and p1 == p2 and p1 % 2 == 0:
                self._bufs[key].update({"st0": torch.zeros(M, 2, 2, **f32), "st": torch.zeros(2 * self.layers, M, p1, 2, **f32)})
                self._guard_buf(dev)
        return self._bufs[key]

    @torch.no_grad()
    def image_embeds(self, frames: torch.Tensor) -> torch.Tensor:
        return self._run(frames[:, None])[0]

    @torch.no_grad()
    def hidden_state(self, frames: torch.Tensor, n_layers: Optional[int] = None) -> torch.Tensor:
        if frames.dim() == 4:
            frames = frames[:, None]
        _, b = self._run(frames, n_layers)
        N = frames.shape[0] * frames.shape[1]
        return b["xf"].view(N, self.n_patches + 1, self.hidden)

    def _run(self, frames5: torch.Tensor, n_layers: Optional[int] = None):
        self._require_hip()
        dev = self.device
        B, Fr = frames5.shape[:2]
        if tuple(frames5.shape[2:]) != (3, self.image, self.image):
            raise RuntimeError(f"frames: expected (B,F,3,{self.image},{self.image}), got {tuple(frames5.shape)}")
        fr = L.f32c(frames5.to(dev)).view(B * Fr, 3, self.image, self.image)
        p, b, w, V = self._pack(), self._workbufs(B, Fr), self._w, "vision_model."
        if n_layers is not None:
            p = dict(p, layers=p["layers"][:max(1, int(n_layers))])
        N, H, T = B * Fr, self.hidden, self.n_patches + 1
        M = N * T
        s = L.stream_ptr(dev)
        L.check(L.lib().ufnd_vit_patchify(fr.data_ptr(), b["patches"].data_ptr(), N, self.image, self.patch, s), "ufnd_vit_patchify")
        self._gemm(b["patches"], p["wpatch"], None, out_f32=b["pe"])
        L.check(L.lib().ufnd_vit_assemble(b["pe"].data_ptr(), w[V + "embeddings.class_embedding"].data_ptr(),
                                          w[V + "embeddings.position_embedding.weight"].data_ptr(),
                                          w[V + "pre_layrnorm.weight"].data_ptr(), w[V + "pre_layrnorm.bias"].data_ptr(),
                                          None if ("st0" in b and self.residual_dtype == "bf16") else b["xf"].data_ptr(),
                                          L.ptr(b["hb"]) if "st0" in b else None, L.ptr(b.get("st0")),
                                          N, self.n_patches, H, self.eps, s), "ufnd_vit_assemble")
        if "st0" in b:
            eps, stA, st = self.eps, b["st0"], b["st"]
            for i, ly in enumerate(p["layers"]):
                st1, st2 = st[2 * i], st[2 * i + 1]
                self._gemm_ln(b["hb"], ly["wqkvf"], ly["bqkvf"], out_bf16=b["qkv"], a_stats=stA, colsum=ly["csqkv"], eps=eps, which="qkv")
                self._attn(b["qkv"], None, b["ctx"], N, T, self.heads)
                rb = self.residual_dtype == "bf16"
                last = i == len(p["layers"]) - 1
                self._gemm_ln(b["ctx"], ly["wo"], ly["bo"], out_f32=None if rb else b["xf"], out_bf16=b["hb"], residual=None if rb else b["xf"],
                              residual_bf16=b["hb"] if rb else None, out_stats=st1, eps=eps, which="out")
                self._gemm_ln(b["hb"], ly["w1f"], ly["bif"], out_bf16=b["m"], act=ACT_QUICK_GELU, a_stats=st1, colsum=ly["cs1"], eps=eps, which="ffn1")
                self._gemm_ln(b["m"], ly["w2"], ly["b2"], out_f32=b["xf"] if (last or not rb) else None, out_bf16=b["hb"],
                              residual=None if rb else b["xf"], residual_bf16=b["hb"] if rb else None, out_stats=st2, eps=eps, which="ffn2")
                stA = st2
            self._ln(b["xf"], T * H, w[V + "post_layernorm.weight"], w[V + "post_layernorm.bias"], b["pooled"], None, N, H, self.eps)
            self._gemm(b["pooled"], p["wproj"], None, out_f32=b["e"])
            return b["e"], b
        for ly in p["layers"]:
            self._ln(b["xf"], H, ly["g1"], ly["b1"], b["hb"], None, M, H, self.eps)
            self._gemm(b["hb"], ly["wqkv"], ly["bqkv"], out_bf16=b["qkv"], which="qkv")
            self._attn(b["qkv"], None, b["ctx"], N, T, self.heads)
            self._gemm(b["ctx"], ly["wo"], ly["bo"], out_f32=b["xf"], residual=b["xf"], which="out")
            self._ln(b["xf"], H, ly["g2"], ly["b2n"], b["hb"], None, M, H, self.eps)
            self._gemm(b["hb"], ly["w1"], ly["bi"], out_bf16=b["m"], act=ACT_QUICK_GELU, which="ffn1")
            self._gemm(b["m"], ly["w2"], ly["b2"], out_f32=b["xf"], residual=b["xf"], which="ffn2")
        self._ln(b["xf"], T * H, w[V + "post_layernorm.weight"], w[V + "post_layernorm.bias"], b["pooled"], None, N, H, self.eps)
        self._gemm(b["pooled"], p["wproj"], None, out_f32=b["e"])
        return b["e"], b

    @torch.no_grad()
    def forward(self, frames: torch.Tensor, strict: bool = False) -> torch.Tensor:
        if frames.dim() == 4:
            frames = frames[:, None]
        if strict:
            rd, self.residual_dtype = self.residual_dtype, "fp32"
            try:
                if self.fold_ln:
                    out = self.forward(frames)
                    if not self.check_fold():
                        return out
                return self.forward(frames)
            finally:
                self.residual_dtype = rd
        B, Fr = frames.shape[:2]
        e, b = self._run(frames)
        L.check(L.lib().ufnd_l2norm_frames(e.data_ptr(), b["feat"].data_ptr(), B, Fr, self.proj, L.stream_ptr(self.device)),
                "ufnd_l2norm_frames")
        return b["feat"]
```

Before: 27670.

## Bin-pack short text sequences into 128-row attention tiles for fused QKV-attention

Extends the text pack kernel to group live sequences into 32-row slots and bin-pack them, e.g. 3+1 or 2+2 or 1+1+1+1, into 128-row tiles. The fused QKV+attention GEMM then launches only nbins tiles and gathers rows per slot, replacing the one-tile-per-sample scheme. The goal is to cut wasted MMA and attention work on padded rows of short sequences. In exchange it adds index and masking complexity, slot-level row gathers, and a packing step in the single-block pack kernel.

```diff
diff --git a/include/ultrafnd_hip.h b/include/ultrafnd_hip.h
--- a/include/ultrafnd_hip.h
+++ b/include/ultrafnd_hip.h
@@ -201,6 +201,8 @@
                             void* stream);
 
 int ufnd_text_pack(const int32_t* mask, int B, int L, int32_t* cu_seqlens, int32_t* row_src, void* stream);
+int ufnd_text_pack_bins(const int32_t* mask, int B, int L, int32_t* cu_seqlens, int32_t* row_src, int32_t* bins, int32_t* nbins,
+                        void* stream);
 int ufnd_bert_embed_live(const int64_t* ids, const int32_t* row_src, const int* m_live, const float* word, const float* pos,
                          const float* type0, const float* gamma, const float* beta, void* x_bf16, float* x_f32, int capacity, int L,
                          int H, int vocab, float eps, void* stream);
@@ -212,6 +214,9 @@
                            const int* m_live, void* stream);
 int ufnd_qkv_attention_bf16_packed(const void* X, const void* Wqkv, const float* bqkv, const int32_t* key_mask, const int32_t* cu_seqlens,
                                    void* ctx, int B, int L, int heads, int ldx, int ldw, const ufnd_gemm_ln* ln, void* stream);
+int ufnd_qkv_attention_bf16_bins(const void* X, const void* Wqkv, const float* bqkv, const int32_t* key_mask, const int32_t* cu_seqlens,
+                                 const int32_t* bins, const int32_t* nbins, void* ctx, int B, int L, int heads, int ldx, int ldw,
+                                 const ufnd_gemm_ln* ln, void* stream);
 int ufnd_attention_bf16_varlen_masked(const void* qkv, const int32_t* cu_seqlens, const int32_t* key_mask, void* ctx, int B, int max_len,
                                       int heads, void* stream);
 int ufnd_layernorm_live(const float* x, int ldx, const float* gamma, const float* beta, void* out_bf16, float* out_f32, int capacity,
diff --git a/ultrafnd_git_amd/_lib.py b/ultrafnd_git_amd/_lib.py
--- a/ultrafnd_git_amd/_lib.py
+++ b/ultrafnd_git_amd/_lib.py
@@ -160,10 +160,12 @@
         "ufnd_attention_bf16_varlen": [P, P, P, I, I, I, P],
         "ufnd_meanpool_l2_packed": [P, P, P, P, I, I, P],
         "ufnd_text_pack": [P, I, I, P, P, P],
+        "ufnd_text_pack_bins": [P, I, I, P, P, P, P, P],
         "ufnd_bert_embed_live": [P] * 10 + [I, I, I, I, F, P],
         "ufnd_gemm_bf16_live": [P] * 6 + [I] * 10 + [P, P],
         "ufnd_gemm_bf16_ln_live": [P] * 6 + [I] * 9 + [C.POINTER(GemmLn), P, P],
         "ufnd_qkv_attention_bf16_packed": [P, P, P, P, P, P, I, I, I, I, I, C.POINTER(GemmLn), P],
+        "ufnd_qkv_attention_bf16_bins": [P] * 8 + [I, I, I, I, I, C.POINTER(GemmLn), P],
         "ufnd_attention_bf16_varlen_masked": [P, P, P, P, I, I, I, P],
         "ufnd_layernorm_live": [P, I, P, P, P, P, I, I, F, P, P],
         "ufnd_masked_meanpool_l2_live": [P, P, P, P, I, I, I, P],
diff --git a/ultrafnd_git_amd/csrc/encoders.hip b/ultrafnd_git_amd/csrc/encoders.hip
--- a/ultrafnd_git_amd/csrc/encoders.hip
+++ b/ultrafnd_git_amd/csrc/encoders.hip
@@ -182,9 +182,11 @@
   }
 }
 constexpr int PACK_THREADS = 1024, PACK_MAX_B = 16384;
-__global__ __launch_bounds__(PACK_THREADS) void text_pack_kernel(const int32_t* mask, int B, int L, int32_t* cu, int32_t* row_src) {
+__global__ __launch_bounds__(PACK_THREADS) void text_pack_kernel(const int32_t* mask, int B, int L, int32_t* cu, int32_t* row_src,
+                                                                 int32_t* bins, int32_t* nbins) {
   __shared__ int lens[PACK_MAX_B];
   __shared__ int wsum[PACK_THREADS / 64];
+  __shared__ long long csum[PACK_THREADS / 64];
   __shared__ int total;
   const int tid = threadIdx.x, wave = tid >> 6, lane = tid & 63;
   for (int b = wave; b < B; b += PACK_THREADS / 64) {
@@ -224,6 +226,68 @@
     const int r0 = lens[b], n = (b + 1 < B ? lens[b + 1] : total) - r0;
     for (int l = lane; l < n; l += 64) row_src[r0 + l] = b * L + l;
   }
+  if (!bins) return;
+  auto nrows = [&](int b) { return (b + 1 < B ? lens[b + 1] : total) - lens[b]; };
+  long long cown = 0;
+  for (int b = b0; b < b1; ++b) {
+    const int c = (nrows(b) + 31) >> 5;
+    if (c > 0) cown += 1ll << (16 * (c - 1));
+  }
+  long long cinc = cown;
+#pragma unroll
+  for (int o = 1; o < 64; o <<= 1) {
+    const long long y = __shfl_up(cinc, o, 64);
+    if (lane >= o) cinc += y;
+  }
+  if (lane == 63) csum[wave] = cinc;
+  __syncthreads();
+  long long cbase = 0, call = 0;
+  for (int w = 0; w < PACK_THREADS / 64; ++w) {
+    if (w < wave) cbase += csum[w];
+    call += csum[w];
+  }
+  auto field = [](long long v, int c) { return (int)((v >> (16 * (c - 1))) & 0xffff); };
+  const int n1 = field(call, 1), n2 = field(call, 2), n3 = field(call, 3), n4 = field(call, 4);
+  const int p = min(n1, n3), r1 = n1 - p, h = n2 >> 1, t = n2 & 1, u = t ? min(2, r1) : 0;
+  const bool odd_full = t && u == 2;
+  const int f1 = (r1 - u) >> 2, rem1 = (r1 - u) & 3;
+  const int b31 = n4, b22 = b31 + p, b211 = b22 + h, b1111 = b211 + (odd_full ? 1 : 0);
+  const int bp3 = b1111 + f1, bp2 = bp3 + (n3 - p), bp1 = bp2 + ((t && !odd_full) ? 1 : 0), nb = bp1 + (rem1 ? 1 : 0);
+  const int bodd = odd_full ? b211 : bp2;
+  long long rank = cbase + cinc - cown;
+  for (int b = b0; b < b1; ++b) {
+    const int n = nrows(b), c = (n + 31) >> 5;
+    if (c == 0) continue;
+    const int k = field(rank, c);
+    rank += 1ll << (16 * (c - 1));
+    int bin, s0;
+    if (c == 4) {
+      bin = k, s0 = 0;
+    } else if (c == 3) {
+      bin = k < p ? b31 + k : bp3 + (k - p), s0 = 0;
+    } else if (c == 2) {
+      bin = k < 2 * h ? b22 + (k >> 1) : bodd, s0 = k < 2 * h ? 2 * (k & 1) : 0;
+    } else if (k < p) {
+      bin = b31 + k, s0 = 3;
+    } else if (k - p < u) {
+      bin = bodd, s0 = 2 + (k - p);
+    } else {
+      const int k1 = k - p - u;
+      bin = (k1 >> 2) < f1 ? b1111 + (k1 >> 2) : bp1, s0 = k1 & 3;
+    }
+    for (int s = 0; s < c; ++s) {
+      bins[(size_t)bin * 8 + 2 * (s0 + s)] = lens[b] + 32 * s;
+      bins[(size_t)bin * 8 + 2 * (s0 + s) + 1] = (b << 10) | (s << 8) | n;
+    }
+  }
+  for (int i = bp3 + tid; i < nb; i += PACK_THREADS) {
+    const int used = i < bp2 ? 3 : (i < bp1 ? 2 + u : rem1);
+    for (int j = used; j < 4; ++j) {
+      bins[(size_t)i * 8 + 2 * j] = 0;
+      bins[(size_t)i * 8 + 2 * j + 1] = -1;
+    }
+  }
+  if (tid == 0) *nbins = nb;
 }
 
 __global__ __launch_bounds__(256) void l2norm_rows_kernel(float* x, int H) {
@@ -453,7 +517,17 @@
 extern "C" int ufnd_text_pack(const int32_t* mask, int B, int L, int32_t* cu_seqlens, int32_t* row_src, void* stream_) {
   UFND_REQUIRE(mask && cu_seqlens && row_src, "text_pack: null argument");
   UFND_REQUIRE(B >= 1 && B <= PACK_MAX_B && L >= 1 && (long long)B * L < (1ll << 31), "text_pack: B=%d L=%d (B <= %d)", B, L, PACK_MAX_B);
-  hipLaunchKernelGGL(text_pack_kernel, dim3(1), dim3(PACK_THREADS), 0, (hipStream_t)stream_, mask, B, L, cu_seqlens, row_src);
+  hipLaunchKernelGGL(text_pack_kernel, dim3(1), dim3(PACK_THREADS), 0, (hipStream_t)stream_, mask, B, L, cu_seqlens, row_src,
+                     (int32_t*)nullptr, (int32_t*)nullptr);
+  UFND_CHECK_LAUNCH();
+  return UFND_OK;
+}
+
+extern "C" int ufnd_text_pack_bins(const int32_t* mask, int B, int L, int32_t* cu_seqlens, int32_t* row_src, int32_t* bins,
+                                   int32_t* nbins, void* stream_) {
+  UFND_REQUIRE(mask && cu_seqlens && row_src && bins && nbins, "text_pack_bins: null argument");
+  UFND_REQUIRE(B >= 1 && B <= PACK_MAX_B && L >= 1 && L <= 128, "text_pack_bins: B=%d L=%d (B <= %d, L <= 128)", B, L, PACK_MAX_B);
+  hipLaunchKernelGGL(text_pack_kernel, dim3(1), dim3(PACK_THREADS), 0, (hipStream_t)stream_, mask, B, L, cu_seqlens, row_src, bins, nbins);
   UFND_CHECK_LAUNCH();
   return UFND_OK;
 }
diff --git a/ultrafnd_git_amd/csrc/gemm_bf16.hip b/ultrafnd_git_amd/csrc/gemm_bf16.hip
--- a/ultrafnd_git_amd/csrc/gemm_bf16.hip
+++ b/ultrafnd_git_amd/csrc/gemm_bf16.hip
@@ -143,10 +143,20 @@
   return ufnd_qkv_attention_bf16_packed(X, Wqkv, bqkv, key_mask, nullptr, ctx, B, L, heads, ldx, ldw, ln, stream_);
 }
 
+extern "C" int ufnd_qkv_attention_bf16_bins(const void* X, const void* Wqkv, const float* bqkv, const int32_t* key_mask,
+                                            const int32_t* cu_seqlens, const int32_t* bins, const int32_t* nbins, void* ctx, int B,
+                                            int L, int heads, int ldx, int ldw, const ufnd_gemm_ln* ln, void* stream_);
 extern "C" int ufnd_qkv_attention_bf16_packed(const void* X, const void* Wqkv, const float* bqkv, const int32_t* key_mask,
                                               const int32_t* cu_seqlens, void* ctx, int B, int L, int heads, int ldx, int ldw,
                                               const ufnd_gemm_ln* ln, void* stream_) {
+  return ufnd_qkv_attention_bf16_bins(X, Wqkv, bqkv, key_mask, cu_seqlens, nullptr, nullptr, ctx, B, L, heads, ldx, ldw, ln, stream_);
+}
+
+extern "C" int ufnd_qkv_attention_bf16_bins(const void* X, const void* Wqkv, const float* bqkv, const int32_t* key_mask,
+                                            const int32_t* cu_seqlens, const int32_t* bins, const int32_t* nbins, void* ctx, int B,
+                                            int L, int heads, int ldx, int ldw, const ufnd_gemm_ln* ln, void* stream_) {
   UFND_REQUIRE(X && Wqkv && ctx, "qkv_attention: null operand");
+  UFND_REQUIRE(!bins == !nbins && (!bins || cu_seqlens), "qkv_attention: slot bins need cu_seqlens, bins and nbins");
   UFND_REQUIRE(L == 128 && heads >= 2 && heads % 2 == 0 && heads <= 64 && B >= 1 && B <= 16384,
                "qkv_attention: B=%d L=%d heads=%d (this kernel is built for 128-token samples and an even head count; "
                "use ufnd_gemm_bf16[_ln] + ufnd_attention_bf16 otherwise)", B, L, heads);
@@ -164,6 +174,8 @@
   }
   a.att_mask = key_mask;
   a.att_cu = cu_seqlens;
+  a.att_bins = bins;
+  a.att_nbins = nbins;
   a.m_live = cu_seqlens ? cu_seqlens + B : nullptr;
   a.att_ctx = (__bf16*)ctx;
   a.att_h = H;
diff --git a/ultrafnd_git_amd/csrc/gemm_bf16_kernel.hpp b/ultrafnd_git_amd/csrc/gemm_bf16_kernel.hpp
--- a/ultrafnd_git_amd/csrc/gemm_bf16_kernel.hpp
+++ b/ultrafnd_git_amd/csrc/gemm_bf16_kernel.hpp
@@ -51,6 +51,8 @@
   int pp_rows;
   const int* m_live;
   const int32_t* att_cu;
+  const int32_t* att_bins;
+  const int* att_nbins;
 };
 
 __device__ __forceinline__ void dma16(const void* gsrc, void* lds_dst) {
@@ -105,7 +107,7 @@
   constexpr int CBYTES = NW * MI * CP * 4;
   constexpr int RING = STA * ASLOT + STB * BSLOT;
   constexpr int ATT_OFF = (CBYTES + 1023) & ~1023;
-  constexpr int ATT_END = ATT ? ATT_OFF + 6 * 16384 + 512 : 0;
+  constexpr int ATT_END = ATT ? ATT_OFF + 6 * 16384 + 2048 : 0;
   constexpr int STAT_OFF0 = (RING > CBYTES) ? RING : CBYTES;
   constexpr int STAT_OFF = STAT_OFF0 > ATT_END ? STAT_OFF0 : ATT_END;
   constexpr int SMEM = STAT_OFF + (LNX ? BM * 8 + 64 : 0);
@@ -127,6 +129,13 @@
       const int v = __builtin_amdgcn_readfirstlane(*a.m_live);
       mlive = v < a.M ? (v > 0 ? v : 0) : a.M;
       m_tiles = (mlive + BM - 1) / BM;
+      if ((int)blockIdx.x >= m_tiles * a.n_tiles) return;
+    }
+  }
+  if constexpr (ATT) {
+    if (a.att_bins) {
+      const int v = __builtin_amdgcn_readfirstlane(*a.att_nbins);
+      m_tiles = v < a.m_tiles ? (v > 0 ? v : 0) : a.m_tiles;
       if ((int)blockIdx.x >= m_tiles * a.n_tiles) return;
     }
   }
@@ -150,8 +159,21 @@
   }
   const int m0 = tm * BM, n0 = tn * BN;
   int arow0 = m0, alen = BM;
+  int srow[4] = {0, 0, 0, 0}, scnt[4] = {0, 0, 0, 0}, smeta[4] = {-1, -1, -1, -1};
+  const bool slots = ATT && a.att_bins != nullptr;
   if constexpr (ATT) {
-    if (a.att_cu) {
+    if (slots) {
+      const int32_t* bd = a.att_bins + (size_t)tm * 8;
+#pragma unroll
+      for (int j = 0; j < 4; ++j) {
+        srow[j] = __builtin_amdgcn_readfirstlane(bd[2 * j]);
+        smeta[j] = __builtin_amdgcn_readfirstlane(bd[2 * j + 1]);
+        const int n = smeta[j] & 255, rest = n - 32 * ((smeta[j] >> 8) & 3);
+        scnt[j] = smeta[j] < 0 ? 0 : (rest < 32 ? rest : 32);
+      }
+#pragma unroll
+      for (int j = 1; j < 4; ++j) srow[j] = scnt[j] > 0 ? srow[j] : srow[0];
+    } else if (a.att_cu) {
       mlive = __builtin_amdgcn_readfirstlane(*a.m_live);
       arow0 = __builtin_amdgcn_readfirstlane(a.att_cu[tm]);
       alen = __builtin_amdgcn_readfirstlane(a.att_cu[tm + 1]) - arow0;
@@ -160,6 +182,23 @@
   } else {
     alen = mlive - m0;
   }
+  auto tile_row = [&](int tr) {
+    if (slots) {
+      const int j = tr >> 5, q = tr & 31;
+      const int r0 = j == 0 ? srow[0] : j == 1 ? srow[1] : j == 2 ? srow[2] : srow[3];
+      const int c = j == 0 ? scnt[0] : j == 1 ? scnt[1] : j == 2 ? scnt[2] : scnt[3];
+      return r0 + (q < c ? q : (c > 0 ? c - 1 : 0));
+    }
+    const int gr = arow0 + tr;
+    return gr < mlive ? gr : mlive - 1;
+  };
+  auto tile_row_live = [&](int tr) {
+    if (slots) {
+      const int j = tr >> 5;
+      return (tr & 31) < (j == 0 ? scnt[0] : j == 1 ? scnt[1] : j == 2 ? scnt[2] : scnt[3]);
+    }
+    return tr < alen;
+  };
   const int wave = __builtin_amdgcn_readfirstlane(threadIdx.x >> 6), lane = threadIdx.x & 63;
   const int wm = wave / WN, wn = wave % WN, fr = lane & (MI - 1), g = lane / MI;
 
@@ -180,9 +219,14 @@
     }
   }
   const int prow = lane >> 3, ppos = lane & 7;
-  auto issueA = [&](int t) {
+  int arow_att[ATT ? PWA : 1];
+  if constexpr (ATT) {
+#pragma unroll
+    for (int ii = 0; ii < PWA; ++ii) arow_att[ii] = tile_row(8 * (wave + NW * ii) + prow);
+  }
+  auto issueA = [&](int t, int kt) {
     char* buf = smem + (t % STA) * ASLOT;
-    const int k0 = kbase + t * BK;
+    const int k0 = kbase + kt * BK;
 #pragma unroll
     for (int ii = 0; ii < PWA; ++ii) {
       const int p = wave + NW * ii;
@@ -190,12 +234,13 @@
       const int c = ppos ^ ((r >> 1) & 7);
       int gr = arow0 + r;
       gr = gr < mlive ? gr : mlive - 1;
+      if constexpr (ATT) gr = arow_att[ii];
       dma16(a.A + (size_t)gr * a.lda + k0 + c * 8, buf + p * 1024);
     }
   };
-  auto issueB = [&](int t) {
+  auto issueB = [&](int t, int kt) {
     char* buf = smem + STA * ASLOT + (t % STB) * BSLOT;
-    const int k0 = kbase + t * BK;
+    const int k0 = kbase + kt * BK;
 #pragma unroll
     for (int ii = 0; ii < PWB; ++ii) {
       int p = wave + NW * ii;
@@ -220,6 +265,7 @@
       const int parts = a.a_stats ? a.a_parts : a.r_parts;
       int row = arow0 + (int)threadIdx.x / TPR;
       row = row < mlive ? row : mlive - 1;
+      if constexpr (ATT) row = tile_row((int)threadIdx.x / TPR);
       const f32x4* base = reinterpret_cast<const f32x4*>(sp + (size_t)row * parts * 2);
       const int nq = parts >> 1, sub = threadIdx.x % TPR;
 #pragma unroll
@@ -233,31 +279,31 @@
   }
   int att_mk = 1;
   if constexpr (ATT) {
-    if (a.att_mask && threadIdx.x < BM) att_mk = a.att_mask[m0 + threadIdx.x];
+    if (slots) {
+      const int j = (int)threadIdx.x >> 7, k = threadIdx.x & 127;
+      const int mt = j == 0 ? smeta[0] : j == 1 ? smeta[1] : j == 2 ? smeta[2] : smeta[3];
+      att_mk = mt >= 0 && k < (mt & 255);
+      if (att_mk && a.att_mask) att_mk = a.att_mask[(size_t)(mt >> 10) * BM + k];
+    } else if (a.att_mask && threadIdx.x < BM) {
+      att_mk = a.att_mask[m0 + threadIdx.x];
+    }
   }
 #pragma unroll
   for (int s = 0; s < STA; ++s) {
-    if (s < STB && s < nk) issueB(s);
-    if (s < nk) issueA(s);
+    const int ks = s < nk ? s : nk - 1;
+    if (s < STB && (LNX || s < nk)) issueB(s, ks);
+    if (LNX || s < nk) issueA(s, ks);
   }
 
   if constexpr (LNX) {
     if (sp) {
       constexpr int NPRO = STA * PWA + STB * PWB;
       static_assert(NPRO <= 63, "vmcnt range");
-      if (STA <= nk) {
-        if constexpr (GPT == 1)
-          asm volatile("s_waitcnt vmcnt(%3)" : "+v"(sv[0][0]), "+v"(sv[0][1]), "+v"(sv[0][2]) : "n"(NPRO) : "memory");
-        else
-          asm volatile("s_waitcnt vmcnt(%6)" : "+v"(sv[0][0]), "+v"(sv[0][1]), "+v"(sv[0][2]), "+v"(sv[GPT - 1][0]), "+v"(sv[GPT - 1][1]),
-                       "+v"(sv[GPT - 1][2]) : "n"(NPRO) : "memory");
-      } else {
-        if constexpr (GPT == 1)
-          asm volatile("s_waitcnt vmcnt(0)" : "+v"(sv[0][0]), "+v"(sv[0][1]), "+v"(sv[0][2]) : : "memory");
-        else
-          asm volatile("s_waitcnt vmcnt(0)" : "+v"(sv[0][0]), "+v"(sv[0][1]), "+v"(sv[0][2]), "+v"(sv[GPT - 1][0]), "+v"(sv[GPT - 1][1]),
-                       "+v"(sv[GPT - 1][2]) : : "memory");
-      }
+      if constexpr (GPT == 1)
+        asm volatile("s_waitcnt vmcnt(%3) ; STATRETIRE %0 %1 %2" : "+v"(sv[0][0]), "+v"(sv[0][1]), "+v"(sv[0][2]) : "n"(NPRO) : "memory");
+      else
+        asm volatile("s_waitcnt vmcnt(%6) ; STATRETIRE %0 %1 %2 %3 %4 %5" : "+v"(sv[0][0]), "+v"(sv[0][1]), "+v"(sv[0][2]), "+v"(sv[GPT - 1][0]),
+                     "+v"(sv[GPT - 1][1]), "+v"(sv[GPT - 1][2]) : "n"(NPRO) : "memory");
       const int nq_ = (a.a_stats ? a.a_parts : a.r_parts) >> 1, sub_ = threadIdx.x % TPR;
       float gs[GPT], gq[GPT];
 #pragma unroll
@@ -290,7 +336,7 @@
       if (a.guard && a.a_stats) {
         float ratio = __fmul_rn(fabsf(mean), rstd);
         ratio = ratio == ratio ? ratio : INFINITY;
-        const float worst = wave_max(threadIdx.x % TPR == 0 && (int)threadIdx.x / TPR < alen ? ratio : 0.0f);
+        const float worst = wave_max(threadIdx.x % TPR == 0 && tile_row_live((int)threadIdx.x / TPR) ? ratio : 0.0f);
         if (lane == 0) reinterpret_cast<float*>(smem + STAT_OFF + BM * 8)[wave] = worst;
       }
       asm volatile("s_waitcnt lgkmcnt(0)" ::: "memory");
@@ -352,8 +398,8 @@
       __builtin_amdgcn_sched_barrier(0);
       if constexpr (ABL != 1) read_half(t + 1, IntC<0>{}, af0, bf0);
       if constexpr (ABL != 2) {
-        if constexpr (IB) issueB(t + STB);
-        if constexpr (IA) issueA(t + STA);
+        if constexpr (IB) issueB(t + STB, t + STB);
+        if constexpr (IA) issueA(t + STA, t + STA);
       }
     }
     if constexpr (ABL != 1) {
@@ -613,9 +659,18 @@
   if constexpr (ATT) {
     constexpr float NEG_MASK = -3.0e38f;
     float* kbias = reinterpret_cast<float*>(smem + ATT_OFF + 6 * 16384);
-    if (threadIdx.x < BM) kbias[threadIdx.x] = att_mk != 0 ? 0.0f : NEG_MASK;
+    if (slots || threadIdx.x < BM) kbias[threadIdx.x] = att_mk != 0 ? 0.0f : NEG_MASK;
     __syncthreads();
     const int hh = wave >> 2, wq = wave & 3, g4 = lane >> 4, f16 = lane & 15;
+    int wrow0 = arow0 + 32 * wq, wcnt = alen - 32 * wq, koff = 0;
+    const float* wbias = kbias;
+    if (slots) {
+      const int mt = wq == 0 ? smeta[0] : wq == 1 ? smeta[1] : wq == 2 ? smeta[2] : smeta[3];
+      wrow0 = wq == 0 ? srow[0] : wq == 1 ? srow[1] : wq == 2 ? srow[2] : srow[3];
+      wcnt = wq == 0 ? scnt[0] : wq == 1 ? scnt[1] : wq == 2 ? scnt[2] : scnt[3];
+      koff = 32 * (wq - ((mt >> 8) & 3));
+      wbias = kbias + wq * BM;
+    }
     const char* qimg = smem + ATT_OFF + hh * 16384;
     const char* kimg = smem + ATT_OFF + (2 + hh) * 16384;
     const char* vimg = smem + ATT_OFF + (4 + hh) * 16384;
@@ -633,12 +688,11 @@
       for (int qt = 0; qt < 2; ++qt) o[dt][qt] = f32x4{0.f, 0.f, 0.f, 0.f};
     float m_run[2] = {-INFINITY, -INFINITY}, l_run[2] = {0.f, 0.f};
     constexpr int KB = 64, KT = KB / 16;
-    if (wq * 32 < alen) {
+    if (wcnt > 0) {
 #pragma unroll
     for (int kb0 = 0; kb0 < BM; kb0 += KB) {
-      const char* ks = kimg + kb0 * 128;
-      const char* vs = vimg + kb0 * 128;
-      if (masked_block_is_noop(kbias + kb0, lane, m_run)) continue;
+      const int kr0 = koff + kb0;
+      if (masked_block_is_noop(wbias + kb0, lane, m_run)) continue;
       f32x4 sc[KT][2];
 #pragma unroll
       for (int kt = 0; kt < KT; ++kt)
@@ -648,15 +702,15 @@
       for (int kk = 0; kk < 2; ++kk)
 #pragma unroll
         for (int kt = 0; kt < KT; ++kt) {
-          const bf16x8 kf = lds_frag(ks, kt * 16 + f16, g4 + 4 * kk);
+          const bf16x8 kf = lds_frag(kimg, (kr0 + kt * 16 + f16) & (BM - 1), g4 + 4 * kk);
 #pragma unroll
           for (int qt = 0; qt < 2; ++qt) sc[kt][qt] = __builtin_amdgcn_mfma_f32_16x16x32_bf16(kf, qf[qt][kk], sc[kt][qt], 0, 0, 0);
         }
-      const bool any_masked = __any(kbias[kb0 + lane] != 0.0f);
+      const bool any_masked = __any(wbias[kb0 + lane] != 0.0f);
       bf16x8 pf[KT / 2][2];
 #pragma unroll
       for (int qt = 0; qt < 2; ++qt) {
-        const float alpha = online_softmax_block<KT>(sc, qt, kbias + kb0, any_masked, g4, a.att_scale_log2e, m_run[qt], l_run[qt], pf);
+        const float alpha = online_softmax_block<KT>(sc, qt, wbias + kb0, any_masked, g4, a.att_scale_log2e, m_run[qt], l_run[qt], pf);
         if (!__all(alpha == 1.0f)) {
 #pragma unroll
           for (int dt = 0; dt < 4; ++dt) o[dt][qt] *= alpha;
@@ -667,13 +721,13 @@
 #pragma unroll
         for (int dt = 0; dt < 4; ++dt) {
           const int qq = f16 >> 2, pp = f16 & 3;
-          const int key0 = 32 * ksd + 4 * g4 + qq;
+          const int key0 = (kr0 + 32 * ksd + 4 * g4 + qq) & (BM - 1);
           const int ch = 2 * dt + (pp >> 1);
           const int off0 = key0 * 128 + ((ch ^ (((key0 >> 1) & 3) << 1)) << 4) + 8 * (pp & 1);
           const int key1 = key0 + 16;
           const int off1 = key1 * 128 + ((ch ^ (((key1 >> 1) & 3) << 1)) << 4) + 8 * (pp & 1);
-          const s16x4 t0 = __builtin_amdgcn_ds_read_tr16_b64_v4i16((s16x4 __attribute__((address_space(3)))*)(vs + off0));
-          const s16x4 t1 = __builtin_amdgcn_ds_read_tr16_b64_v4i16((s16x4 __attribute__((address_space(3)))*)(vs + off1));
+          const s16x4 t0 = __builtin_amdgcn_ds_read_tr16_b64_v4i16((s16x4 __attribute__((address_space(3)))*)(vimg + off0));
+          const s16x4 t1 = __builtin_amdgcn_ds_read_tr16_b64_v4i16((s16x4 __attribute__((address_space(3)))*)(vimg + off1));
           union { s16x4 s2[2]; bf16x8 v; } u;
           u.s2[0] = t0;
           u.s2[1] = t1;
@@ -689,9 +743,9 @@
       l += __shfl_xor(l, 16, 64);
       l += __shfl_xor(l, 32, 64);
       const float inv = 1.0f / l;
-      const int q = wq * 32 + qt * 16 + f16;
-      if (q >= alen) continue;
-      __bf16* dst = a.att_ctx + (size_t)(arow0 + q) * a.att_h + (tn * 2 + hh) * 64 + 4 * g4;
+      const int q = qt * 16 + f16;
+      if (q >= wcnt) continue;
+      __bf16* dst = a.att_ctx + (size_t)(wrow0 + q) * a.att_h + (tn * 2 + hh) * 64 + 4 * g4;
 #pragma unroll
       for (int dt = 0; dt < 4; ++dt) {
         bf16x4 ov = {(__bf16)(o[dt][qt][0] * inv), (__bf16)(o[dt][qt][1] * inv), (__bf16)(o[dt][qt][2] * inv), (__bf16)(o[dt][qt][3] * inv)};
diff --git a/ultrafnd_git_amd/encoders.py b/ultrafnd_git_amd/encoders.py
--- a/ultrafnd_git_amd/encoders.py
+++ b/ultrafnd_git_amd/encoders.py
@@ -23,6 +23,32 @@
     if not 0.0 <= p < 1.0:
         raise ValueError(f"{name}={p!r}: a dropout probability in [0, 1)")
     return p
+
+
+def text_slot_bins(n_rows) -> list:
+    cls = {c: [b for b, n in enumerate(n_rows) if (int(n) + 31) // 32 == c] for c in (1, 2, 3, 4)}
+    one, two, three = cls[1], cls[2], cls[3]
+    p = min(len(one), len(three))
+    ones = one[p:]
+    u = min(2, len(ones)) if len(two) % 2 else 0
+    slots = lambda *bs: [(b, s) for b in bs for s in range((int(n_rows[b]) + 31) // 32)]
+    full = [slots(b) for b in cls[4]] + [slots(three[k], one[k]) for k in range(p)]
+    full += [slots(two[k], two[k + 1]) for k in range(0, len(two) - 1, 2)]
+    odd = slots(two[-1], *ones[:u]) if len(two) % 2 else None
+    rest = ones[u:]
+    if odd is not None and u == 2:
+        full.append(odd)
+    full += [slots(*rest[k:k + 4]) for k in range(0, len(rest) - len(rest) % 4, 4)]
+    part = [slots(b) for b in three[p:]]
+    if odd is not None and u < 2:
+        part.append(odd)
+    if len(rest) % 4:
+        part.append(slots(*rest[len(rest) - len(rest) % 4:]))
+    return [x + [None] * (4 - len(x)) for x in full + part]
+
+
+def text_slot_bin_count(n_rows) -> int:
+    return len(text_slot_bins(n_rows))
 
 
 class _EncoderBase(nn.Module):
@@ -145,13 +171,19 @@
         L.check(L.lib().ufnd_layernorm(x.data_ptr(), ldx, gamma.data_ptr(), beta.data_ptr(), L.ptr(out_bf16),
                                        L.ptr(out_f32), M, H, eps, L.stream_ptr(x.device)), "ufnd_layernorm")
 
-    def _qkv_attn(self, A, W, bias, mask_i32, ctx, B, Lq, heads, a_stats=None, colsum=None, eps=1e-5, cu=None):
+    def _qkv_attn(self, A, W, bias, mask_i32, ctx, B, Lq, heads, a_stats=None, colsum=None, eps=1e-5, cu=None, bins=None):
         import ctypes
         ln = None
         if a_stats is not None:
             ln = L.GemmLn()
             ln.a_stats, ln.colsum, ln.a_parts, ln.a_eps, ln.r_eps, ln.width = a_stats.data_ptr(), colsum.data_ptr(), a_stats.shape[1], eps, eps, self.hidden
             ln.guard = self._guard_buf(A.device).data_ptr()
+        if bins is not None:
+            L.check(L.lib().ufnd_qkv_attention_bf16_bins(A.data_ptr(), W.data_ptr(), L.ptr(bias), L.ptr(mask_i32), cu.data_ptr(),
+                                                         bins[0].data_ptr(), bins[1].data_ptr(), ctx.data_ptr(), B, Lq, heads, A.stride(0),
+                                                         W.stride(0), ctypes.byref(ln) if ln is not None else None,
+                                                         L.stream_ptr(A.device)), "ufnd_qkv_attention_bf16_bins")
+            return
         L.check(L.lib().ufnd_qkv_attention_bf16_packed(A.data_ptr(), W.data_ptr(), L.ptr(bias), L.ptr(mask_i32), L.ptr(cu), ctx.data_ptr(),
                                                        B, Lq, heads, A.stride(0), W.stride(0), ctypes.byref(ln) if ln is not None else None,
                                                        L.stream_ptr(A.device)), "ufnd_qkv_attention_bf16_packed")
@@ -235,7 +267,8 @@
                                "x1b": torch.empty(M, H, **bf), "x1f": torch.empty(M, H, **f32),
                                "qkv": torch.empty(M, 3 * H, **bf), "ctx": torch.empty(M, H, **bf),
                                "h": torch.empty(M, self.inter, **bf), "feat": torch.empty(B, H, **f32),
-                               "cu": torch.zeros(B + 1, dtype=torch.int32, device=dev), "row_src": torch.zeros(M, dtype=torch.int32, device=dev)}
+                               "cu": torch.zeros(B + 1, dtype=torch.int32, device=dev), "row_src": torch.zeros(M, dtype=torch.int32, device=dev),
+                               "bins": torch.zeros(B, 8, dtype=torch.int32, device=dev), "nbins": torch.zeros(1, dtype=torch.int32, device=dev)}
             p1 = L.lib().ufnd_gemm_bf16_stat_parts(M, H, H)
             p2 = L.lib().ufnd_gemm_bf16_stat_parts(M, H, self.inter)
             if self.fold_ln and p1 > 0 and p1 == p2 and p1 % 2 == 0:
@@ -272,11 +305,12 @@
         H = self.hidden
         v = {k: (x[:M] if torch.is_tensor(x) and x.dim() >= 2 and x.shape[0] >= M and k not in ("feat", "st") else x) for k, x in b.items()}
         cu = fused[3] if fused is not None and len(fused) > 3 else None
+        bins = fused[4] if fused is not None and len(fused) > 4 else None
         if "st" in b:
             return self._layers_folded(p, v, M, attn, fused)
         for ly in p["layers"]:
             if fused is not None:
-                self._qkv_attn(v["xb"], ly["wqkv"], ly["bqkv"], fused[2], v["ctx"], fused[0], fused[1], self.heads, cu=cu)
+                self._qkv_attn(v["xb"], ly["wqkv"], ly["bqkv"], fused[2], v["ctx"], fused[0], fused[1], self.heads, cu=cu, bins=bins)
             else:
                 self._gemm(v["xb"], ly["wqkv"], ly["bqkv"], out_bf16=v["qkv"], which="qkv")
                 attn(v["qkv"], v["ctx"])
@@ -291,16 +325,17 @@
         y1, y2 = b["y"], b["y2"]
         st = b["st"]
         cu = fused[3] if fused is not None and len(fused) > 3 else None
+        bins = fused[4] if fused is not None and len(fused) > 4 else None
         prev = None
         for i, ly in enumerate(p["layers"]):
             st1, st2 = st[2 * i][:M], st[2 * i + 1][:M]
             stp = st[2 * i - 1][:M] if i > 0 else None
             if fused is not None:
                 if prev is None:
-                    self._qkv_attn(b["xb"], ly["wqkv"], ly["bqkv"], fused[2], b["ctx"], fused[0], fused[1], self.heads, cu=cu)
+                    self._qkv_attn(b["xb"], ly["wqkv"], ly["bqkv"], fused[2], b["ctx"], fused[0], fused[1], self.heads, cu=cu, bins=bins)
                 else:
                     self._qkv_attn(b["y2b"], ly["wqkvf"], ly["bqkvf"], fused[2], b["ctx"], fused[0], fused[1], self.heads,
-                                   a_stats=stp, colsum=ly["csqkv"], eps=eps, cu=cu)
+                                   a_stats=stp, colsum=ly["csqkv"], eps=eps, cu=cu, bins=bins)
             elif prev is None:
                 self._gemm(b["xb"], ly["wqkv"], ly["bqkv"], out_bf16=b["qkv"], which="qkv")
             else:
@@ -356,14 +391,19 @@
         M, H, s = B * Lq, self.hidden, L.stream_ptr(dev)
         cu, feat = b["cu"], b["feat"]
         live = cu.data_ptr() + 4 * B
-        L.check(L.lib().ufnd_text_pack(mask.data_ptr(), B, Lq, cu.data_ptr(), b["row_src"].data_ptr(), s), "ufnd_text_pack")
+        fuse = self.fuse_qkv_attention and Lq == 128 and self.heads % 2 == 0
+        if fuse:
+            L.check(L.lib().ufnd_text_pack_bins(mask.data_ptr(), B, Lq, cu.data_ptr(), b["row_src"].data_ptr(), b["bins"].data_ptr(),
+                                                b["nbins"].data_ptr(), s), "ufnd_text_pack_bins")
+        else:
+            L.check(L.lib().ufnd_text_pack(mask.data_ptr(), B, Lq, cu.data_ptr(), b["row_src"].data_ptr(), s), "ufnd_text_pack")
         L.check(L.lib().ufnd_bert_embed_live(ids.data_ptr(), b["row_src"].data_ptr(), live, w["embeddings.word_embeddings.weight"].data_ptr(),
                                              w["embeddings.position_embeddings.weight"].data_ptr(),
                                              w["embeddings.token_type_embeddings.weight"].data_ptr(),
                                              w["embeddings.LayerNorm.weight"].data_ptr(), w["embeddings.LayerNorm.bias"].data_ptr(),
                                              b["xb"].data_ptr(), None if ("st" in b and self.residual_dtype == "bf16") else b["xf"].data_ptr(),
                                              M, Lq, H, self.vocab, self.eps, s), "ufnd_bert_embed_live")
-        fused = (B, Lq, mask, cu) if (self.fuse_qkv_attention and Lq == 128 and self.heads % 2 == 0) else None
+        fused = (B, Lq, mask, cu, (b["bins"], b["nbins"])) if fuse else None
 
         def attn(qkv, ctx):
             L.check(L.lib().ufnd_attention_bf16_varlen_masked(qkv.data_ptr(), cu.data_ptr(), mask.data_ptr(), ctx.data_ptr(), B, Lq,
```

Result: faster. 28580 (median of 6 runs) (+3.3%).
